# deemoe404/rmcv

Measured on AMD Instinct MI355X. Metric: frames/sec (1280x1024 BGR) armour detect, higher is better.
Workload: dtype u8

## Files before the change

include/rmcv_abi.h:

```cpp
#ifndef RMCV_ABI_H
#define RMCV_ABI_H

#include <stdint.h>

#ifdef __cplusplus
extern "C" {
#endif

#define RMCV_ABI_VERSION 1

#define RMCV_OK 0
#define RMCV_ERR_BAD_ARG (-1)
#define RMCV_ERR_CAPACITY (-2)
#define RMCV_ERR_NOMEM (-3)
#define RMCV_ERR_HIP (-4)
#define RMCV_ERR_NO_DEVICE (-5)
#define RMCV_ERR_RCCL (-6)
#define RMCV_ERR_TIMEOUT (-7)

#define RMCV_CAMP_RED 0
#define RMCV_CAMP_BLUE 1
#define RMCV_CAMP_GUIDELIGHT 2
#define RMCV_CAMP_NEUTRAL (-1)

// ... 19 lines not shown
    int32_t blob_i, blob_j;
} rmcv_armour;

typedef struct {
    int32_t camp;
    int32_t lower_bound;
    int32_t morph;
    float   tilt_max;
    float   ratio_lo, ratio_hi;
    double  area_lo, area_hi;
    float   angle_diff_max;
    float   shear_max;
    float   length_ratio_max;
    int32_t _pad;
} rmcv_params;

typedef struct {
    int32_t max_frames;
    int32_t max_width;
    int32_t max_height;
    int32_t max_contours;
    int32_t max_points;
    int32_t max_blobs;
    int32_t max_armours;
    int32_t _pad;
} rmcv_limits;

#define RMCV_STAGE_BINARY 1
#define RMCV_STAGE_CONTOURS 2
#define RMCV_STAGE_BLOBS 4
#define RMCV_STAGE_ARMOURS 8
#define RMCV_STAGE_ALL 15
#define RMCV_STAGE_POSE 32
#define RMCV_STAGE_NO_IMAGE 64
#define RMCV_STAGE_IDENTITY 16

#define RMCV_FRAME_OVF_CONTOURS 1
#define RMCV_FRAME_OVF_POINTS 2
#define RMCV_FRAME_OVF_BLOBS 4
#define RMCV_FRAME_OVF_ARMOURS 8
#define RMCV_FRAME_SLOW_PATH 16
#define RMCV_FRAME_MID_PATH 64
#define RMCV_FRAME_HULL 32

typedef struct rmcv_ctx rmcv_ctx;

int  rmcv_abi_version(void);
void rmcv_default_params(rmcv_params* p);
void rmcv_default_limits(rmcv_limits* l);

int  rmcv_ctx_create(int device, const rmcv_limits* limits , rmcv_ctx** out);
void rmcv_ctx_destroy(rmcv_ctx* ctx);
const char* rmcv_last_error(const rmcv_ctx* ctx);
#define RMCV_OPT_SPARSE_WAVES 1
#define RMCV_OPT_PIXEL_GROUPS 2
#define RMCV_OPT_FRAME_UPLOAD 3
#define RMCV_OPT_RUN_AHEAD 4
#define RMCV_OPT_CONTOUR_TIER 5
#define RMCV_OPT_DENSE_DEFER 7
#define RMCV_OPT_PIXEL_HALO_NT 11
#define RMCV_OPT_OVERLOADS 13
#define RMCV_OPT_PIXEL_SHAPE 14
#define RMCV_OPT_WAIT_TIMEOUT_MS 15
#define RMCV_OPT_IMAGE_EXPORT 17
#define RMCV_OPT_TEST_SLOW_US 18
#define RMCV_OPT_TEST_DELAY_US 16
#define RMCV_OPT_INPUT_FORMAT 19
#define RMCV_INPUT_BGR 0
#define RMCV_BAYER_RG 1
#define RMCV_BAYER_GB 2
#define RMCV_BAYER_GR 3
#define RMCV_BAYER_BG 4
#define RMCV_OPT_INPUT_SAMPLE_BITS 20
#define RMCV_OPT_INPUT_VALID_BIT 21
#define RMCV_OPT_INPUT_ORIENT 22
#define RMCV_ORIENT_MIRROR 1
#define RMCV_ORIENT_FLIP 2
#define RMCV_OPT_ENHANCE 23
int  rmcv_ctx_set_option(rmcv_ctx* ctx, int option, int value);
int  rmcv_ctx_set_enhance_gains(rmcv_ctx* ctx, float max_gain, float min_gain);
int  rmcv_ctx_get_enhance(const rmcv_ctx* ctx, int32_t* on, float* max_gain, float* min_gain);
int64_t rmcv_pixel_ws_launches(void);
int64_t rmcv_pixel_image_delta_launches(void);
int  rmcv_ctx_check_guards(rmcv_ctx* ctx, int32_t* n_damaged);
int  rmcv_ctx_frame_timing(const rmcv_ctx* ctx, double* us, int cap);
int  rmcv_ctx_forget_frame_buffer(rmcv_ctx* ctx, const void* frame);


int rmcv_extract_color(rmcv_ctx* ctx, const uint8_t* bgr, int w, int h, int stride, int camp, int lower_bound,
                       int morph, uint8_t* binary_out, rmcv_point* pts_out, int pts_cap, int32_t* offs_out,
                       int contours_cap, int32_t* n_contours, int32_t* n_points);

int rmcv_filter_lightblobs(rmcv_ctx* ctx, const rmcv_point* pts, const int32_t* offs, int n_contours,
                           float tilt_max, float ratio_lo, float ratio_hi, double area_lo, double area_hi,
                           int enemy, rmcv_lightblob* blobs_out, int blobs_cap, int32_t* n_blobs,
                           int32_t* blob_src, int32_t* neg_idx_out, int32_t* n_neg);

int rmcv_filter_armours(rmcv_ctx* ctx, const rmcv_lightblob* blobs, int n_blobs, float angle_diff_max,
                        float shear_max, float length_ratio_max, int enemy, rmcv_armour* armours_out,
                        int armours_cap, int32_t* n_armours);

int rmcv_fit_ellipse(rmcv_ctx* ctx, const rmcv_point* pts, int n, rmcv_rrect* out);

int rmcv_demosaic(rmcv_ctx* ctx, const uint8_t* raw, int w, int h, int stride, int pattern, uint8_t* bgr_out, int out_stride);
int rmcv_demosaic_raw(rmcv_ctx* ctx, const void* raw, int w, int h, int stride, int pattern, int sample_bits, int valid_bit, int orient,
                      uint8_t* bgr_out, int out_stride);

int rmcv_gamma_lut(float gamma, uint8_t lut[256]);
int rmcv_enhance_gamma(const uint64_t sums_bgr[3], int64_t n_pixels, float max_gain, float min_gain, float* gamma);
int rmcv_calc_gamma(rmcv_ctx* ctx, const uint8_t* src, int row_bytes, int rows, int src_stride, float gamma, uint8_t* dst, int dst_stride);
int rmcv_auto_enhance(rmcv_ctx* ctx, const uint8_t* bgr, int w, int h, int stride, float max_gain, float min_gain, uint8_t* out, int out_stride,
                      float* gamma_out);


int rmcv_batch_upload(rmcv_ctx* ctx, const uint8_t* frames, int n_frames, int w, int h, int stride,
                      int64_t frame_pitch);
int rmcv_batch_set_device_frames(rmcv_ctx* ctx, const void* d_frames, int n_frames, int w, int h, int stride,
                                 int64_t frame_pitch);
int rmcv_batch_run(rmcv_ctx* ctx, const rmcv_params* p, int stages, void* hip_stream);
int rmcv_batch_sync(rmcv_ctx* ctx);
int rmcv_batch_run_timed(rmcv_ctx* ctx, const rmcv_params* p, int stages, void* hip_stream, float stage_ms[5]);

int rmcv_batch_counts(rmcv_ctx* ctx, int32_t* n_contours, int32_t* n_points, int32_t* n_blobs,
                      int32_t* n_armours, int32_t* status);
int rmcv_batch_get_binary(rmcv_ctx* ctx, int frame, uint8_t* binary_out);
int rmcv_batch_get_contours(rmcv_ctx* ctx, int frame, rmcv_point* pts_out, int pts_cap, int32_t* offs_out,
                            int contours_cap, int32_t* n_contours, int32_t* n_points);
int rmcv_batch_get_blobs(rmcv_ctx* ctx, int frame, rmcv_lightblob* blobs_out, int cap, int32_t* n_blobs,
                         int32_t* blob_src);
int rmcv_batch_get_gammas(rmcv_ctx* ctx, float* gamma_out, int cap);
int rmcv_batch_get_armours(rmcv_ctx* ctx, rmcv_armour* armours_out, int cap, int32_t* frame_offs,
                           int32_t* n_total);
int rmcv_batch_device_views(rmcv_ctx* ctx, void** d_armours, void** d_counts, int32_t* per_frame_cap,
                            int32_t* n_frames);

int rmcv_batch_set_windows(rmcv_ctx* ctx, const rmcv_point* origins, int win_w, int win_h);
int rmcv_batch_set_device_windows(rmcv_ctx* ctx, const void* d_origins, int win_w, int win_h);
int rmcv_batch_get_windows(rmcv_ctx* ctx, rmcv_point* eff_out, int cap, int32_t* win_w, int32_t* win_h);
int rmcv_batch_device_windows(rmcv_ctx* ctx, void** d_eff, int32_t* win_w, int32_t* win_h);
int rmcv_get_roi(const float* points, int n, float scale_w, float scale_h, int frame_w, int frame_h, const int32_t previous[4], int32_t out[4]);
int rmcv_window_origin(const int32_t rect[4], int win_w, int win_h, int32_t out_xy[2]);
int rmcv_armours_to_frame(rmcv_armour* armours, int n, int x, int y);

int rmcv_frame_key(int32_t camp, int32_t lower_bound, int32_t out[4]);
int rmcv_batch_set_frame_camps(rmcv_ctx* ctx, const int32_t* camps, const int32_t* lower_bounds);
int rmcv_batch_set_device_frame_camps(rmcv_ctx* ctx, const void* d_camps, const void* d_lower_bounds);
int rmcv_batch_get_frame_keys(rmcv_ctx* ctx, int32_t* keys_out , int cap);

#define RMCV_SVM_FEATURES 1200
int rmcv_svm_load(rmcv_ctx* ctx, const float* weights , const double* rho,
                  const int32_t* labels, int n_class);
int rmcv_classify_armours(rmcv_ctx* ctx, const uint8_t* bgr, int w, int h, int stride, rmcv_armour* armours, int n,
                          int32_t* identity_out, uint8_t* icons_out);
int rmcv_batch_get_identities(rmcv_ctx* ctx, int32_t* identity_out, int cap, int32_t* n_total);
int rmcv_batch_get_icons(rmcv_ctx* ctx, int frame, uint8_t* icons_out, int cap_armours, int32_t* n_armours);

#define RMCV_SVM_MAX_GRID 16
#define RMCV_SVM_MAX_DF 28
#define RMCV_SVM_MAX_FOLDS 64
#define RMCV_SVM_MAX_SAMPLES 8192
#define RMCV_SVM_MAX_PAIR_SAMPLES 2048
typedef struct {
    double  eps;
    int32_t max_iter;
    int32_t k_fold;
    int32_t n_c;
// ... 457 lines not shown
```

rmcv_amd/abi.py:

```python
import ctypes as C
import os

import numpy as np

_HERE = os.path.dirname(os.path.abspath(__file__))
LIB_PATH = os.environ.get("RMCV_LIB_PATH") or os.path.join(_HERE, "lib", "librmcv_hip.so")

POINT = np.dtype([("x", "<i4"), ("y", "<i4")])
RRECT = np.dtype([("cx", "<f4"), ("cy", "<f4"), ("w", "<f4"), ("h", "<f4"), ("angle", "<f4")])
LIGHTBLOB = np.dtype([("angle", "<f4"), ("target", "<i4"), ("center", "<f4", (2,)),
                      ("vertices", "<f4", (4, 2)), ("size", "<f4", (2,))])
ARMOUR = np.dtype([("icon", "<f4", (4, 2)), ("vertices", "<f4", (4, 2)), ("bbox", "<f4", (4,)),
                   ("blob_i", "<i4"), ("blob_j", "<i4")])
TRACK_IDS = 32
TRACK = np.dtype([("armour", ARMOUR), ("timestamp", "<i8"), ("lost_count", "<i4"), ("identity", "<i4"), ("position", "<f8", (3,)),
                  ("initialized", "<i4"), ("n_ids", "<i4"), ("ids", "<i4", (TRACK_IDS,)), ("counts", "<i4", (TRACK_IDS,)),
                  ("measurement", "<f8", (6,)), ("state_pre", "<f8", (6,)), ("state_post", "<f8", (6,)),
                  ("transition", "<f8", (6, 6)), ("measurement_matrix", "<f8", (6, 6)), ("process_noise_cov", "<f8", (6, 6)),
                  ("measurement_noise_cov", "<f8", (6, 6)), ("error_cov_pre", "<f8", (6, 6)), ("error_cov_post", "<f8", (6, 6)),
                  ("gain", "<f8", (6, 6))])
assert POINT.itemsize == 8 and LIGHTBLOB.itemsize == 56 and ARMOUR.itemsize == 88 and TRACK.itemsize == 2552
AIM = np.dtype([("track", "<i4"), ("identity", "<i4"), ("lost_count", "<i4"), ("status", "<i4"), ("pitch", "<f8"), ("yaw", "<f8"),
                ("flight_time", "<f8"), ("distance", "<f8"), ("point", "<f8", (3,))])
AIM_INPUT = np.dtype([("world2camera", "<f8", (4, 4)), ("motor_angle", "<f8")])
assert AIM.itemsize == 72 and AIM_INPUT.itemsize == 136
ATTITUDE = np.dtype([("roll", "<f8"), ("pitch", "<f8"), ("yaw", "<f8")])
ATTITUDE_CONFIG = np.dtype([("gripper2camera", "<f8", (4, 4)), ("motor_angle_mode", "<i4"), ("reserved", "<i4")])
assert ATTITUDE.itemsize == 24 and ATTITUDE_CONFIG.itemsize == 136
SERIAL_PACKET_BYTES = 24
ATT_MOTOR_KEEP, ATT_MOTOR_PITCH = 0, 1

OK, ERR_BAD_ARG, ERR_CAPACITY, ERR_NOMEM, ERR_HIP, ERR_NO_DEVICE, ERR_RCCL, ERR_TIMEOUT = 0, -1, -2, -3, -4, -5, -6, -7
COMM_ID_BYTES = 128
CAMP_RED, CAMP_BLUE, CAMP_GUIDELIGHT, CAMP_NEUTRAL = 0, 1, 2, -1
MORPH_NONE, MORPH_DILATE, MORPH_CLOSE = 0, 1, 2
OPT_SPARSE_WAVES = 1
OPT_PIXEL_GROUPS = 2
OPT_FRAME_UPLOAD = 3
OPT_RUN_AHEAD = 4
OPT_CONTOUR_TIER = 5
OPT_DENSE_DEFER = 7
OPT_PIXEL_HALO_NT = 11
OPT_OVERLOADS = 13
OPT_PIXEL_SHAPE = 14
OPT_WAIT_TIMEOUT_MS = 15
OPT_TEST_DELAY_US = 16
OPT_IMAGE_EXPORT = 17
OPT_TEST_SLOW_US = 18
OPT_INPUT_FORMAT = 19
INPUT_BGR, BAYER_RG, BAYER_GB, BAYER_GR, BAYER_BG = 0, 1, 2, 3, 4
BAYER_PATTERNS = (BAYER_RG, BAYER_GB, BAYER_GR, BAYER_BG)
OPT_INPUT_SAMPLE_BITS = 20
OPT_INPUT_VALID_BIT = 21
OPT_INPUT_ORIENT = 22
ORIENT_MIRROR, ORIENT_FLIP = 1, 2
OPT_ENHANCE = 23
ENHANCE_MAX_GAIN, ENHANCE_MIN_GAIN = 100.0, 50.0
STAGE_BINARY, STAGE_CONTOURS, STAGE_BLOBS, STAGE_ARMOURS, STAGE_ALL, STAGE_IDENTITY, STAGE_POSE, STAGE_NO_IMAGE = 1, 2, 4, 8, 15, 16, 32, 64
SVM_FEATURES = 1200
COMPENSATE_NONE, COMPENSATE_CLASSIC, COMPENSATE_NI = 0, 1, 2
AIM_NO_TARGET, AIM_NO_SOLUTION = 1, 2
AIM_HEIGHT_FIXED, AIM_HEIGHT_DELTA = 0, 1
AIM_SRC_FILTER, AIM_SRC_MEASUREMENT = 0, 1
AIM_PICK_WINDOW, AIM_PICK_NEAREST = 0, 1
VIEW_BLOBS, VIEW_NEGATIVES, VIEW_ARMOURS, VIEW_ALL = 1, 2, 4, 7
FRAME_OVF_CONTOURS, FRAME_OVF_POINTS, FRAME_OVF_BLOBS, FRAME_OVF_ARMOURS, FRAME_SLOW_PATH, FRAME_MID_PATH = 1, 2, 4, 8, 16, 64
HARVEST_SKIP, HARVEST_MISSES = -2**31, 1
HARVEST_META = np.dtype([("tag", "<u8"), ("frame", "<i4"), ("armour", "<i4"), ("label", "<i4"), ("identity", "<i4"), ("win_x", "<i4"), ("win_y", "<i4"),
                         ("icon", "<f4", (4, 2))])

EXPORTS = [
    "rmcv_abi_version", "rmcv_default_params", "rmcv_default_limits", "rmcv_ctx_create", "rmcv_ctx_destroy",
    "rmcv_last_error", "rmcv_ctx_set_option", "rmcv_ctx_forget_frame_buffer", "rmcv_ctx_check_guards", "rmcv_ctx_frame_timing", "rmcv_extract_color", "rmcv_filter_lightblobs", "rmcv_filter_armours", "rmcv_fit_ellipse", "rmcv_demosaic", "rmcv_demosaic_raw",
    "rmcv_batch_upload", "rmcv_batch_set_device_frames", "rmcv_batch_run", "rmcv_batch_sync", "rmcv_batch_run_timed",
    "rmcv_batch_counts", "rmcv_batch_get_binary", "rmcv_batch_get_contours", "rmcv_batch_get_blobs",
    "rmcv_batch_get_armours", "rmcv_batch_device_views", "rmcv_batch_compact_armours", "rmcv_synth_frame", "rmcv_synth_checksum",
    "rmcv_svm_load", "rmcv_classify_armours", "rmcv_batch_get_identities", "rmcv_batch_get_icons",
    "rmcv_default_pnp_config", "rmcv_pnp_load", "rmcv_locate_armours", "rmcv_batch_set_base2gripper", "rmcv_batch_get_poses",
    "rmcv_max_iou", "rmcv_identity_max", "rmcv_comm_unique_id", "rmcv_comm_create", "rmcv_comm_destroy", "rmcv_comm_info", "rmcv_comm_last_error", "rmcv_gather",
    "rmcv_default_pipeline_config", "rmcv_pipeline_create", "rmcv_pipeline_destroy", "rmcv_pipeline_last_error", "rmcv_pipeline_get_info", "rmcv_pipeline_context", "rmcv_pipeline_context_of", "rmcv_pipeline_set_hot_contexts", "rmcv_pipeline_set_wait_timeout", "rmcv_pipeline_reset_stats", "rmcv_hw_queues_hint", "rmcv_pixel_ws_launches", "rmcv_pixel_image_delta_launches",
    "rmcv_pipeline_submit", "rmcv_pipeline_submit_legacy", "rmcv_pipeline_wait", "rmcv_pipeline_collect", "rmcv_pipeline_drain", "rmcv_pipeline_record",
    "rmcv_pipeline_set_hook", "rmcv_pipeline_set_gather", "rmcv_pipeline_gathered", "rmcv_device_alloc", "rmcv_device_free", "rmcv_device_upload", "rmcv_device_download",
    "rmcv_track_init", "rmcv_track_reset", "rmcv_track_update", "rmcv_track_predict", "rmcv_track_step", "rmcv_min_area_rect", "rmcv_match_lightblob", "rmcv_find_lightblobs", "rmcv_lightblob_overlap", "rmcv_batch_run_legacy",
    "rmcv_ctx_set_enhance_gains", "rmcv_ctx_get_enhance", "rmcv_gamma_lut", "rmcv_enhance_gamma", "rmcv_calc_gamma", "rmcv_auto_enhance", "rmcv_batch_get_gammas",
    "rmcv_batch_set_windows", "rmcv_batch_set_device_windows", "rmcv_batch_get_windows", "rmcv_batch_device_windows", "rmcv_pipeline_submit_windows",
    "rmcv_get_roi", "rmcv_window_origin", "rmcv_armours_to_frame",
    "rmcv_default_tracker_config", "rmcv_tracker_create", "rmcv_tracker_destroy", "rmcv_tracker_last_error", "rmcv_tracker_reset", "rmcv_tracker_set_origins",
    "rmcv_tracker_device_origins", "rmcv_batch_track", "rmcv_tracker_counts", "rmcv_tracker_get", "rmcv_tracker_step_host", "rmcv_pipeline_submit_tracked",
    "rmcv_projectile_angle", "rmcv_solve_gea", "rmcv_delta_height", "rmcv_distance", "rmcv_rigid_inverse", "rmcv_default_aim_config", "rmcv_tracker_set_aim",
    "rmcv_tracker_set_aim_inputs", "rmcv_tracker_device_aim_inputs", "rmcv_tracker_aim", "rmcv_tracker_get_aims", "rmcv_tracker_device_aims", "rmcv_tracker_put",
    "rmcv_aim_step_host",
    "rmcv_frame_key", "rmcv_batch_set_frame_camps", "rmcv_batch_set_device_frame_camps", "rmcv_batch_get_frame_keys", "rmcv_pipeline_submit_camps",
    "rmcv_tracker_set_camps", "rmcv_tracker_device_camps",
    "rmcv_euler_to_matrix", "rmcv_homogeneous", "rmcv_crc8", "rmcv_serial_decode", "rmcv_serial_encode", "rmcv_attitude_step_host", "rmcv_default_attitude_config",
    "rmcv_tracker_set_attitude", "rmcv_tracker_set_attitudes", "rmcv_tracker_get_attitudes", "rmcv_tracker_device_attitudes", "rmcv_tracker_get_aim_inputs",
    "rmcv_batch_get_base2gripper", "rmcv_batch_attitude", "rmcv_pipeline_submit_tracked_serial",
    "rmcv_frame_camera", "rmcv_pnp_load_cameras", "rmcv_batch_set_frame_cameras", "rmcv_batch_set_device_frame_cameras", "rmcv_batch_get_frame_cameras",
    "rmcv_pipeline_set_frame_cameras", "rmcv_tracker_set_stream_cameras", "rmcv_tracker_set_aim_configs",
    "rmcv_batch_debug_views", "rmcv_batch_get_debug_view", "rmcv_debug_view", "rmcv_debug_view_host", "rmcv_pipeline_set_views", "rmcv_pipeline_views",
    "rmcv_pack_bound", "rmcv_pack_host", "rmcv_unpack_host", "rmcv_pack_frames", "rmcv_unpack_frames",
    "rmcv_default_recorder_config", "rmcv_recorder_create", "rmcv_recorder_destroy", "rmcv_recorder_last_error", "rmcv_recorder_set_user", "rmcv_recorder_record",
    "rmcv_recorder_freeze", "rmcv_recorder_resume", "rmcv_recorder_count", "rmcv_recorder_entry", "rmcv_recorder_frame", "rmcv_recorder_device_frame",
    "rmcv_recorder_save", "rmcv_session_append", "rmcv_session_open", "rmcv_session_count", "rmcv_session_entry", "rmcv_session_frame", "rmcv_session_close",
    "rmcv_pipeline_set_recorder",
    "rmcv_loop_bound", "rmcv_loop_trigger_host", "rmcv_recorder_set_trigger", "rmcv_recorder_trigger", "rmcv_recorder_loop", "rmcv_session_loop", "rmcv_session_append_loop",
    "rmcv_tracker_restore", "rmcv_tracker_config_from_loop", "rmcv_tracker_aim_config_from_loop", "rmcv_tracker_attitude_config_from_loop",
    "rmcv_svm_train_defaults", "rmcv_svm_train", "rmcv_svm_train_host", "rmcv_svm_gram", "rmcv_svm_gram_host", "rmcv_svm_predict", "rmcv_svm_predict_host",
    "rmcv_dataset_create", "rmcv_dataset_destroy", "rmcv_dataset_clear", "rmcv_dataset_last_error", "rmcv_dataset_count", "rmcv_dataset_get", "rmcv_dataset_device",
    "rmcv_batch_harvest", "rmcv_batch_harvest_device", "rmcv_harvest_plan_host", "rmcv_pipeline_set_harvest", "rmcv_svm_train_dataset", "rmcv_svm_predict_dataset",
]


class Params(C.Structure):
    _fields_ = [("camp", C.c_int32), ("lower_bound", C.c_int32), ("morph", C.c_int32), ("tilt_max", C.c_float),
                ("ratio_lo", C.c_float), ("ratio_hi", C.c_float), ("area_lo", C.c_double), ("area_hi", C.c_double),
                ("angle_diff_max", C.c_float), ("shear_max", C.c_float), ("length_ratio_max", C.c_float),
                ("_pad", C.c_int32)]


class LegacyParams(C.Structure):
    _fields_ = [("min_ratio", C.c_float), ("max_ratio", C.c_float), ("tilt_angle", C.c_float), ("min_area", C.c_float),
                ("max_area", C.c_float), ("fit_ellipse", C.c_int32)]


class PnpConfig(C.Structure):
    _fields_ = [("camera_matrix", C.c_double * 9), ("dist", C.c_double * 5), ("gripper2camera", C.c_double * 16),
                ("square_w", C.c_float), ("square_h", C.c_float)]


class Limits(C.Structure):
    _fields_ = [("max_frames", C.c_int32), ("max_width", C.c_int32), ("max_height", C.c_int32),
                ("max_contours", C.c_int32), ("max_points", C.c_int32), ("max_blobs", C.c_int32),
                ("max_armours", C.c_int32), ("_pad", C.c_int32)]


class PipelineConfig(C.Structure):
    _fields_ = [("depth", C.c_int32), ("pixel_streams", C.c_int32), ("sparse_streams", C.c_int32), ("armour_cap", C.c_int32),
                ("sparse_waves", C.c_int32), ("pixel_groups", C.c_int32), ("host_results", C.c_int32), ("dense_streams", C.c_int32),
                ("hot_contexts", C.c_int32), ("_reserved", C.c_int32)]


class PipelineInfo(C.Structure):
    _fields_ = [("depth", C.c_int32), ("pixel_streams", C.c_int32), ("sparse_streams", C.c_int32), ("armour_cap", C.c_int32),
                ("sparse_waves", C.c_int32), ("pixel_groups", C.c_int32), ("host_results", C.c_int32), ("dense_streams", C.c_int32),
                ("max_frames", C.c_int32), ("hw_queues_env", C.c_int32), ("hw_queues_wanted", C.c_int32), ("_pad", C.c_int32),
                ("record_bytes", C.c_int64), ("armours_offset", C.c_int64), ("submitted", C.c_uint64), ("collected", C.c_uint64),
                ("dense_split", C.c_uint64), ("hot_batches", C.c_uint64), ("hot_contexts", C.c_int32), ("_pad2", C.c_int32), ("latency_batches", C.c_uint64),
                ("host_blocking_calls", C.c_uint64), ("wait_timeout_ms", C.c_int32), ("_pad3", C.c_int32), ("max_submit_us", C.c_double), ("heavy_batches", C.c_uint64), ("held_back", C.c_uint64)]


SVM_MAX_GRID, SVM_MAX_DF, SVM_MAX_FOLDS, SVM_MAX_SAMPLES, SVM_MAX_PAIR_SAMPLES = 16, 28, 64, 8192, 2048


class SvmTrainParams(C.Structure):
    _fields_ = [("eps", C.c_double), ("max_iter", C.c_int32), ("k_fold", C.c_int32), ("n_c", C.c_int32), ("reserved", C.c_int32),
                ("c_grid", C.c_double * SVM_MAX_GRID)]


class SvmTrainReport(C.Structure):
    _fields_ = [("best_c", C.c_double), ("best_index", C.c_int32), ("n_df", C.c_int32), ("cv_errors", C.c_int32 * SVM_MAX_GRID),
                ("iterations", C.c_int32 * SVM_MAX_DF), ("converged", C.c_int32 * SVM_MAX_DF), ("objective", C.c_double * SVM_MAX_DF),
                ("phase_ms", C.c_double * 6), ("alpha_out", C.c_void_p), ("message", C.c_char * 128)]

# ... 35 lines not shown
    _fields_ = [("world2camera", C.c_double * 16), ("motor_angle", C.c_double)]


class _Attitude(C.Structure):
    _fields_ = [("roll", C.c_double), ("pitch", C.c_double), ("yaw", C.c_double)]


class _TrackerConfig(C.Structure):
    _fields_ = [("n_streams", C.c_int32), ("track_cap", C.c_int32), ("process_noise", C.c_double), ("measurement_noise", C.c_double),
                ("error", C.c_double), ("tick_frequency", C.c_double), ("roi_scale_w", C.c_float), ("roi_scale_h", C.c_float),
                ("frame_w", C.c_int32), ("frame_h", C.c_int32), ("win_w", C.c_int32), ("win_h", C.c_int32)]


class _AimConfig(C.Structure):
    _fields_ = [("g", C.c_double), ("v0", C.c_double), ("height", C.c_double), ("offset_x", C.c_float), ("offset_y", C.c_float),
                ("angle_offset", C.c_double), ("latency_s", C.c_double), ("mode", C.c_int32), ("height_mode", C.c_int32), ("source", C.c_int32),
                ("pick", C.c_int32), ("lead_iterations", C.c_int32), ("max_lost", C.c_int32), ("overloads", C.c_int32), ("identity_mask", C.c_uint32)]


class _AttitudeConfig(C.Structure):
    _fields_ = [("gripper2camera", C.c_double * 16), ("motor_angle_mode", C.c_int32), ("reserved", C.c_int32)]


class LoopState(C.Structure):
    _fields_ = [("stream", C.c_int32), ("n_tracking", C.c_int32), ("status", C.c_int32), ("n_armours", C.c_int32),
                ("origin_next", C.c_int32 * 2), ("origin_eff", C.c_int32 * 2), ("frame_status", C.c_int32), ("has_camps", C.c_int32),
                ("camp", C.c_int32), ("lower_bound", C.c_int32), ("has_key", C.c_int32), ("key", C.c_int32 * 4), ("has_cameras", C.c_int32),
                ("cam_eff", C.c_int32), ("has_aim", C.c_int32), ("has_attitude", C.c_int32), ("has_packet", C.c_int32), ("packet_errors", C.c_int32),
                ("n_tracks", C.c_int32), ("flags", C.c_int32), ("fired", C.c_uint32), ("has_prev", C.c_int32), ("trig_frame_status_mask", C.c_int32),
                ("trig_aim_jump_deg", C.c_double), ("timestamp", C.c_int64), ("sequence", C.c_uint64), ("aim", _Aim), ("aim_input", _AimInput), ("attitude", _Attitude),
                ("packet", C.c_uint8 * 24), ("tracker_config", _TrackerConfig), ("aim_config", _AimConfig), ("attitude_config", _AttitudeConfig),
                ("gripper2camera", C.c_double * 16)]


class TriggerConfig(C.Structure):
    _fields_ = [("mask", C.c_uint32), ("post_batches", C.c_int32), ("frame_status_mask", C.c_int32), ("reserved", C.c_int32), ("aim_jump_deg", C.c_double)]


class TriggerInfo(C.Structure):
    _fields_ = [("fired", C.c_int32), ("mask", C.c_uint32), ("sequence", C.c_uint64), ("k", C.c_int32), ("stream", C.c_int32), ("noticed", C.c_int32),
                ("batches_since", C.c_int32)]


LOOP_SIDE_BYTES = 32
assert C.sizeof(TriggerConfig) == 24 and C.sizeof(TriggerInfo) == 32 and C.sizeof(LoopState) % 8 == 0


PIPELINE_HOOK = C.CFUNCTYPE(C.c_int, C.c_void_p, C.c_uint64, C.c_void_p, C.c_int64, C.c_void_p, C.POINTER(C.c_void_p))


class RmcvError(RuntimeError):
    def __init__(self, code, msg=""):
        super().__init__("rmcv error %d: %s" % (code, msg))
        self.code = code


_lib = None


def load(path):
    if not os.path.exists(path):
        raise ImportError("%s is missing: run `make -C rmcv_amd/csrc` (or __graft_entry__.build())" % path)
    L = C.CDLL(path)
    L.rmcv_last_error.restype = C.c_char_p
    L.rmcv_last_error.argtypes = [C.c_void_p]
    L.rmcv_synth_checksum.restype = C.c_uint64
    L.rmcv_ctx_destroy.restype = None
    L.rmcv_ctx_destroy.argtypes = [C.c_void_p]
    L.rmcv_pipeline_last_error.restype = C.c_char_p
    L.rmcv_pipeline_last_error.argtypes = [C.c_void_p]
    L.rmcv_pipeline_destroy.restype = None
    L.rmcv_pipeline_destroy.argtypes = [C.c_void_p]
    L.rmcv_pipeline_context.restype = C.c_void_p
    L.rmcv_pipeline_context.argtypes = [C.c_void_p, C.c_int]
    L.rmcv_pipeline_set_hot_contexts.restype = C.c_int
    L.rmcv_pipeline_set_hot_contexts.argtypes = [C.c_void_p, C.c_int]
    L.rmcv_pipeline_set_wait_timeout.restype = C.c_int
    L.rmcv_pipeline_set_wait_timeout.argtypes = [C.c_void_p, C.c_int]
    L.rmcv_pixel_ws_launches.restype = C.c_int64
    L.rmcv_pixel_ws_launches.argtypes = []
    if hasattr(L, "rmcv_pixel_image_delta_launches"):
        L.rmcv_pixel_image_delta_launches.restype = C.c_int64
        L.rmcv_pixel_image_delta_launches.argtypes = []
    L.rmcv_pipeline_context_of.restype = C.c_void_p
    L.rmcv_pipeline_context_of.argtypes = [C.c_void_p, C.c_uint64]
    L.rmcv_pipeline_submit.argtypes = [C.c_void_p, C.c_void_p, C.c_int, C.c_int, C.c_int, C.c_int, C.c_int64, C.c_void_p, C.c_int, C.c_void_p]
    L.rmcv_pipeline_submit_legacy.argtypes = [C.c_void_p, C.c_void_p, C.c_int, C.c_int, C.c_int, C.c_int, C.c_int64, C.c_void_p, C.c_void_p, C.c_int, C.c_void_p]
    L.rmcv_pipeline_wait.argtypes = [C.c_void_p, C.c_uint64]
    L.rmcv_pipeline_collect.argtypes = [C.c_void_p, C.c_uint64, C.c_void_p, C.c_int, C.c_void_p, C.c_void_p]
    L.rmcv_pipeline_record.argtypes = [C.c_void_p, C.c_uint64, C.c_void_p, C.c_void_p]
    L.rmcv_pipeline_gathered.argtypes = [C.c_void_p, C.c_uint64, C.c_void_p, C.c_void_p]
    L.rmcv_pipeline_set_gather.argtypes = [C.c_void_p, C.c_void_p, C.c_int]
    if hasattr(L, "rmcv_demosaic"):
        L.rmcv_demosaic.restype = C.c_int
        L.rmcv_demosaic.argtypes = [C.c_void_p, C.c_void_p, C.c_int, C.c_int, C.c_int, C.c_int, C.c_void_p, C.c_int]
    if hasattr(L, "rmcv_demosaic_raw"):
        L.rmcv_demosaic_raw.restype = C.c_int
        L.rmcv_demosaic_raw.argtypes = [C.c_void_p, C.c_void_p, C.c_int, C.c_int, C.c_int, C.c_int, C.c_int, C.c_int, C.c_int, C.c_void_p, C.c_int]
    if hasattr(L, "rmcv_auto_enhance"):
        L.rmcv_ctx_set_enhance_gains.argtypes = [C.c_void_p, C.c_float, C.c_float]
        L.rmcv_ctx_get_enhance.argtypes = [C.c_void_p, C.c_void_p, C.c_void_p, C.c_void_p]
        L.rmcv_gamma_lut.argtypes = [C.c_float, C.c_void_p]
        L.rmcv_enhance_gamma.argtypes = [C.c_void_p, C.c_int64, C.c_float, C.c_float, C.c_void_p]
        L.rmcv_calc_gamma.argtypes = [C.c_void_p, C.c_void_p, C.c_int, C.c_int, C.c_int, C.c_float, C.c_void_p, C.c_int]
        L.rmcv_auto_enhance.argtypes = [C.c_void_p, C.c_void_p, C.c_int, C.c_int, C.c_int, C.c_float, C.c_float, C.c_void_p, C.c_int, C.c_void_p]
        L.rmcv_batch_get_gammas.argtypes = [C.c_void_p, C.c_void_p, C.c_int]
    if hasattr(L, "rmcv_get_roi"):
        L.rmcv_batch_set_windows.argtypes = [C.c_void_p, C.c_void_p, C.c_int, C.c_int]
        L.rmcv_batch_set_device_windows.argtypes = [C.c_void_p, C.c_void_p, C.c_int, C.c_int]
        L.rmcv_batch_get_windows.argtypes = [C.c_void_p, C.c_void_p, C.c_int, C.c_void_p, C.c_void_p]
        L.rmcv_batch_device_windows.argtypes = [C.c_void_p, C.c_void_p, C.c_void_p, C.c_void_p]
        L.rmcv_pipeline_submit_windows.argtypes = [C.c_void_p, C.c_void_p, C.c_int, C.c_int, C.c_int, C.c_int, C.c_int64, C.c_void_p, C.c_int, C.c_int,
                                                   C.c_void_p, C.c_int, C.c_void_p]
        L.rmcv_get_roi.argtypes = [C.c_void_p, C.c_int, C.c_float, C.c_float, C.c_int, C.c_int, C.c_void_p, C.c_void_p]
        L.rmcv_window_origin.argtypes = [C.c_void_p, C.c_int, C.c_int, C.c_void_p]
        L.rmcv_armours_to_frame.argtypes = [C.c_void_p, C.c_int, C.c_int, C.c_int]
    if hasattr(L, "rmcv_tracker_create"):
        L.rmcv_default_tracker_config.restype = None
        L.rmcv_default_tracker_config.argtypes = [C.c_void_p]
        L.rmcv_tracker_create.argtypes = [C.c_int, C.c_void_p, C.c_void_p]
        L.rmcv_tracker_destroy.restype = None
        L.rmcv_tracker_destroy.argtypes = [C.c_void_p]
        L.rmcv_tracker_last_error.restype = C.c_char_p
        L.rmcv_tracker_last_error.argtypes = [C.c_void_p]
        L.rmcv_tracker_reset.argtypes = [C.c_void_p]
        L.rmcv_tracker_set_origins.argtypes = [C.c_void_p, C.c_void_p]
        L.rmcv_tracker_device_origins.argtypes = [C.c_void_p, C.c_void_p]
        L.rmcv_batch_track.argtypes = [C.c_void_p, C.c_void_p, C.c_int64, C.c_void_p]
        L.rmcv_tracker_counts.argtypes = [C.c_void_p, C.c_void_p, C.c_void_p, C.c_int]
        L.rmcv_tracker_get.argtypes = [C.c_void_p, C.c_int, C.c_void_p, C.c_int, C.c_void_p, C.c_void_p, C.c_void_p]
        L.rmcv_tracker_step_host.argtypes = [C.c_void_p, C.c_void_p, C.c_void_p, C.c_void_p, C.c_void_p, C.c_void_p, C.c_void_p, C.c_int, C.c_void_p, C.c_void_p,
                                             C.c_int, C.c_int, C.c_int64]
        L.rmcv_pipeline_submit_tracked.argtypes = [C.c_void_p, C.c_void_p, C.c_void_p, C.c_int, C.c_int, C.c_int, C.c_int, C.c_int64, C.c_void_p, C.c_int, C.c_int64, C.c_void_p]
    if hasattr(L, "rmcv_aim_step_host"):
        L.rmcv_projectile_angle.restype = C.c_double
        L.rmcv_projectile_angle.argtypes = [C.c_double, C.c_double, C.c_double, C.c_double]
        L.rmcv_solve_gea.restype = C.c_double
        L.rmcv_solve_gea.argtypes = [C.c_void_p, C.c_double, C.c_double, C.c_double, C.c_float, C.c_float, C.c_double, C.c_int, C.c_void_p]
        L.rmcv_delta_height.restype = C.c_double
        L.rmcv_delta_height.argtypes = [C.c_void_p, C.c_double, C.c_float, C.c_double]
        L.rmcv_distance.restype = C.c_double
        L.rmcv_distance.argtypes = [C.c_void_p]
        L.rmcv_rigid_inverse.argtypes = [C.c_void_p, C.c_void_p]
        L.rmcv_default_aim_config.restype = None
        L.rmcv_default_aim_config.argtypes = [C.c_void_p]
        L.rmcv_tracker_set_aim.argtypes = [C.c_void_p, C.c_void_p]
        L.rmcv_tracker_set_aim_inputs.argtypes = [C.c_void_p, C.c_void_p]
        L.rmcv_tracker_device_aim_inputs.argtypes = [C.c_void_p, C.c_void_p]
        L.rmcv_tracker_aim.argtypes = [C.c_void_p, C.c_int64, C.c_void_p]
        L.rmcv_tracker_get_aims.argtypes = [C.c_void_p, C.c_void_p, C.c_int]
        L.rmcv_tracker_device_aims.argtypes = [C.c_void_p, C.c_void_p]
        L.rmcv_tracker_put.argtypes = [C.c_void_p, C.c_int, C.c_void_p, C.c_int, C.c_void_p]
        L.rmcv_aim_step_host.argtypes = [C.c_void_p, C.c_double, C.c_void_p, C.c_int, C.c_void_p, C.c_int64, C.c_void_p]
    if hasattr(L, "rmcv_frame_key"):
        L.rmcv_frame_key.argtypes = [C.c_int32, C.c_int32, C.c_void_p]
        L.rmcv_batch_set_frame_camps.argtypes = [C.c_void_p, C.c_void_p, C.c_void_p]
        L.rmcv_batch_set_device_frame_camps.argtypes = [C.c_void_p, C.c_void_p, C.c_void_p]
        L.rmcv_batch_get_frame_keys.argtypes = [C.c_void_p, C.c_void_p, C.c_int]
        L.rmcv_pipeline_submit_camps.argtypes = [C.c_void_p, C.c_void_p, C.c_int, C.c_int, C.c_int, C.c_int, C.c_int64, C.c_void_p, C.c_void_p, C.c_void_p,
                                                 C.c_int, C.c_int, C.c_void_p, C.c_int, C.c_void_p]
        L.rmcv_tracker_set_camps.argtypes = [C.c_void_p, C.c_void_p, C.c_void_p]
        L.rmcv_tracker_device_camps.argtypes = [C.c_void_p, C.c_void_p, C.c_void_p]
    if hasattr(L, "rmcv_attitude_step_host"):
        L.rmcv_euler_to_matrix.argtypes = [C.c_void_p, C.c_void_p]
        L.rmcv_homogeneous.argtypes = [C.c_void_p, C.c_void_p, C.c_void_p]
        L.rmcv_crc8.restype = C.c_uint8
# ... 315 lines not shown
```

rmcv_amd/csrc/image_plan.h:

```cpp
#pragma once

namespace rmcv {

enum ImageTrack { IMAGE_UNKNOWN = 0, IMAGE_TRACKED };
struct ImageState {
    ImageTrack track;
    int w, h;
    int frames;
};
constexpr ImageState IMAGE_STATE_UNKNOWN = {IMAGE_UNKNOWN, 0, 0, 0};

enum ImageKernel { IMAGE_KERNEL_WS = 0, IMAGE_KERNEL_OTHER };
struct ImageLaunch {
    ImageKernel kernel;
    bool image;
    int w, h, ww, frames;
};
enum ImageMode { IMAGE_FULL = 0, IMAGE_DELTA };
struct ImageStep { ImageMode mode; ImageState next; };

inline ImageStep image_step(const ImageState& st, const ImageLaunch& l, bool ok)
{
    ImageStep r = {IMAGE_FULL, st};
    if (!l.image) {
        if (!ok) r.next = IMAGE_STATE_UNKNOWN;
        return r;
    }
    const bool same = st.track == IMAGE_TRACKED && st.w == l.w && st.h == l.h;
    if (l.kernel == IMAGE_KERNEL_WS && same && l.frames <= st.frames && l.ww <= 32) r.mode = IMAGE_DELTA;
    if (!ok || l.kernel != IMAGE_KERNEL_WS) {
        r.next = IMAGE_STATE_UNKNOWN;
        return r;
    }
    r.next = {IMAGE_TRACKED, l.w, l.h, same && st.frames > l.frames ? st.frames : l.frames};
    return r;
}

}
```

rmcv_amd/csrc/k_binary.hip:

```cpp
#include <stdlib.h>

#include <algorithm>
#include <atomic>
#include <type_traits>

#include "k_binary_device.h"

namespace rmcv {

#define K1_ENH 0
#define K1_KERNEL k_binary
#define K1_THRESH(d) thresh16<CA, CB>(d, lb)
#define K1_PASS(a, b) ((a) - (b) >= lb)
#include "k_binary_kernel.inc"

#include "k_binary_ws.inc"

static std::atomic<int64_t> g_ws_launches{0};
int64_t pixel_ws_launches() { return g_ws_launches.load(std::memory_order_relaxed); }
static std::atomic<int64_t> g_image_delta_launches{0};
int64_t pixel_image_delta_launches() { return g_image_delta_launches.load(std::memory_order_relaxed); }
#define K1_LAUNCH_T launch_binary_t
#define K1_EXTRA
#include "k_binary_launch.inc"

hipError_t launch_binary(const Geom& g, const Bufs& b, int camp, int lower_bound, int morph, bool image, const RunPlan& plan, hipStream_t s,
                         ImageState* img)
{
    const PixelVariant v = pixel_variant(g.input_format, g.enhance, g.win, g.keys);
    if (v == PIXEL_BGR)
        return with_channel_pair(frame_key_eff(camp, lower_bound), [&](auto ca, auto cb) { return launch_binary_t<ca, cb>(g, b, lower_bound, morph, image, plan, s, img); });
    const ImageLaunch l = {IMAGE_KERNEL_OTHER, image, g.w, g.h, g.ww, g.n_frames};
    const ImageState before = img ? *img : IMAGE_STATE_UNKNOWN;
    if (img) *img = image_step(before, l, false).next;
    hipError_t e = hipSuccess;
    switch (v) {
    case PIXEL_BGR: break;
    case PIXEL_BAYER: e = launch_binary_bayer(g, b, camp, lower_bound, morph, image, s); break;
    case PIXEL_ENH: e = launch_binary_enh(g, b, camp, lower_bound, morph, image, plan, s); break;
    case PIXEL_WIN: e = launch_binary_win(g, b, camp, lower_bound, morph, image, plan, s); break;
    case PIXEL_CAMP: e = launch_binary_camp(g, b, morph, image, plan, s); break;
    case PIXEL_CAMP_WIN: e = launch_binary_camp_win(g, b, morph, image, plan, s); break;
    }
    if (img && e == hipSuccess) *img = image_step(before, l, true).next;
    return e;
}

__global__ void k_pack_bits(const uint8_t* __restrict__ binary, int w, int h, int ww, uint64_t* __restrict__ bits, int prow,
                            int64_t plane_pitch, uint32_t* __restrict__ rowmask)
{
    const int f = blockIdx.y;
    const int item = blockIdx.x * blockDim.x + threadIdx.x;
    if (item >= h * ww) return;
    const int y = item / ww, k = item % ww;
    const uint8_t* row = binary + (int64_t)f * w * h + (int64_t)y * w;
    uint64_t word = 0;
    for (int bqt = 0; bqt < 64; bqt++) {
        int x = k * 64 + bqt;
        if (x < w && row[x]) word |= 1ull << bqt;
    }
    bits[(int64_t)f * plane_pitch + (int64_t)(y + 1) * prow + 1 + k] = word;
    if (word && k < 32) atomicOr(&rowmask[(int64_t)f * h + y], 1u << k);
}

hipError_t launch_pack_bits(const Geom& g, const Bufs& b, hipStream_t s)
{
    const int items = g.h * g.ww;
    hipError_t e = hipMemsetAsync(b.rowmask, 0, (size_t)g.n_frames * g.h * sizeof(uint32_t), s);
    if (e != hipSuccess) return e;
    return launch(k_pack_bits, dim3((items + 255) / 256, g.n_frames), dim3(256), 0, s, b.binary, g.w, g.h, g.ww, b.bits,
                       g.prow, g.plane_pitch, b.rowmask);
}

}
```

rmcv_amd/csrc/k_binary_launch.inc:

```
#ifndef K1_WIN
#define K1_WIN 0
#endif
#ifndef K1_CAMP
#define K1_CAMP 0
#endif
#if K1_CAMP
#define K1_INST(F) K1_KERNEL<F>
#else
#define K1_INST(F) K1_KERNEL<CA, CB, F>
template <int CA, int CB>
#endif
static hipError_t K1_LAUNCH_T(const Geom& g, const Bufs& b, int lower_bound, int morph, bool image, const RunPlan& plan,
                                  hipStream_t s, ImageState* img = nullptr)
{
    constexpr PixelVariant variant = K1_CAMP ? (K1_WIN ? PIXEL_CAMP_WIN : PIXEL_CAMP) : K1_WIN ? PIXEL_WIN : K1_ENH ? PIXEL_ENH : PIXEL_BGR;
    const PixelShape ps = pixel_shape(pixel_batch(g, b, variant, lower_bound, plan));
    const int strips = ps.strips, lb = ps.lb, all_pass = ps.all_pass, mode = ps.mode;
    const size_t planes = ps.planes;
#if !K1_ENH && !K1_WIN && !K1_CAMP
    const ImageState img_before = img ? *img : IMAGE_STATE_UNKNOWN;
    const ImageLaunch img_launch = {IMAGE_KERNEL_WS, image, g.w, g.h, g.ww, g.n_frames};
    const ImageMode img_mode = image_step(img_before, img_launch, true).mode;
    bool all_ws = true;
    if (img) *img = image_step(img_before, img_launch, false).next;
#endif
    for (int f0 = 0; f0 < g.n_frames; f0 += ps.chunk) {
        const int nf = std::min(ps.chunk, g.n_frames - f0);
        const PixelChunk pc = pixel_chunk(ps, nf);
        const int n_blocks = pc.n_blocks, grid = pc.grid, taper_head = pc.taper_head, taper_tail = pc.taper_tail;
        const uint8_t* frames = b.frames + (int64_t)f0 * g.frame_pitch;
        uint8_t* binary = image ? b.binary + (int64_t)f0 * g.w * g.h : nullptr;
        uint64_t* bits = b.bits + (int64_t)f0 * g.plane_pitch;
        uint32_t* rowmask = b.rowmask + (int64_t)f0 * g.h;
        static size_t lds_set[MAX_DEVICES][3] = {};
        if (planes > 60 * 1024 && planes > lds_set[g.device][mode]) {
#if K1_WIN
            const void* fn = mode == 1 ? reinterpret_cast<const void*>(K1_INST(1)) : reinterpret_cast<const void*>(K1_INST(0));
#else
            const void* fn = mode == 2 ? reinterpret_cast<const void*>(K1_INST(2)) : mode == 1 ? reinterpret_cast<const void*>(K1_INST(1)) : reinterpret_cast<const void*>(K1_INST(0));
#endif
            const hipError_t ea = hipFuncSetAttribute(fn, hipFuncAttributeMaxDynamicSharedMemorySize, (int)planes);
            if (ea != hipSuccess) return ea;
            lds_set[g.device][mode] = planes;
        }
#if !K1_ENH && !K1_WIN && !K1_CAMP
        constexpr int WS_NL = 8, WS_NS = 8, WS_RING = 2, WS_AUX = 2 ;
        if (pc.ws) {
            K1Args ka;
            ka.frames = frames; ka.frame_pitch = g.frame_pitch; ka.stride = g.stride; ka.n_frames = nf; ka.w = g.w; ka.h = g.h; ka.ww = g.ww;
            ka.lb = lb; ka.morph = morph; ka.binary = binary; ka.bits = bits; ka.prow = g.prow; ka.plane_pitch = g.plane_pitch;
            ka.strips = strips; ka.n_blocks = n_blocks; ka.rowmask = rowmask; ka.strip_ctr = b.strip_ctr;
            ka.imgmask = b.imgmask + (int64_t)f0 * g.h; ka.delta = img_mode == IMAGE_DELTA;
            g_ws_launches.fetch_add(1, std::memory_order_relaxed);
            if (ka.delta && binary) g_image_delta_launches.fetch_add(1, std::memory_order_relaxed);
            const hipError_t e = launch(k_binary_ws<CA, CB, WS_NL, WS_NS, WS_RING, WS_AUX, 3, 3>, dim3(pc.grid_ws), dim3((WS_NL + WS_NS) * 64), ps.planes_ws, s, ka);
            if (e != hipSuccess) return e;
            continue;
        }
        all_ws = false;
#endif
#define RMCV_K1_LAUNCH(F)                                                                                                             \
    launch(K1_INST(F), dim3(grid), dim3(256), planes, s, frames, g.frame_pitch, g.stride, nf, g.w, g.h, g.ww, lb, all_pass, \
           morph, binary, bits, g.prow, g.plane_pitch, strips, n_blocks, rowmask, b.strip_ctr, taper_head, taper_tail,               \
           g.pixel_halo_nt K1_EXTRA)
#if K1_WIN
        const hipError_t e = mode == 1 ? RMCV_K1_LAUNCH(1) : RMCV_K1_LAUNCH(0);
#else
        const hipError_t e = mode == 2 ? RMCV_K1_LAUNCH(2) : mode == 1 ? RMCV_K1_LAUNCH(1) : RMCV_K1_LAUNCH(0);
#endif
#undef RMCV_K1_LAUNCH
        if (e != hipSuccess) return e;
    }
#if !K1_ENH && !K1_WIN && !K1_CAMP
    if (img) *img = image_step(img_before, {all_ws ? IMAGE_KERNEL_WS : IMAGE_KERNEL_OTHER, image, g.w, g.h, g.ww, g.n_frames}, true).next;
#endif
    return hipSuccess;
}
#undef K1_INST
```

rmcv_amd/csrc/k_binary_ws.inc:

```

struct K1Args {
    const uint8_t* frames;
    int64_t frame_pitch;
    int stride, n_frames, w, h, ww, lb, morph;
    uint8_t* binary;
    uint64_t* bits;
    int prow;
    int64_t plane_pitch;
    int strips, n_blocks;
    uint32_t* rowmask;
    int* strip_ctr;
    uint32_t* imgmask;
    int delta;
};

template <int NS>
__device__ __forceinline__ uint32_t ws_image_mask(const K1Args& a, const int L, const int sw, const int lane)
{
    constexpr int RPW = SR / NS;
    if (!(a.delta && a.binary && a.ww <= 32) || L < 0) return 0u;
    const int f = L / a.strips, y = (L - f * a.strips) * SR + sw * RPW + lane;
    return (lane < RPW && y < a.h) ? a.imgmask[(int64_t)f * a.h + y] : 0u;
}

template <int NS>
__device__ __forceinline__ uint32_t ws_store_strip(const K1Args& a, const int L, const uint64_t* __restrict__ T, uint64_t* __restrict__ Ew,
                                               const uint64_t* __restrict__ lut, const int sw, const int lane,
                                               const __amdgpu_buffer_rsrc_t r_bin, const __amdgpu_buffer_rsrc_t r_plane, const uint32_t m_old,
                                                   const int L_next)
{
    constexpr int RPW = SR / NS;
    static_assert(RPW >= 2 && RPW % 2 == 0, "a lane produces a pair of rows");
    const int halo = a.morph, ww = a.ww, w = a.w, h = a.h;
    const int f = L / a.strips, strip = L - f * a.strips;
    const int y0 = strip * SR;
    const int s0 = sw * RPW;
    if (y0 + s0 >= h) return ws_image_mask<NS>(a, L_next, sw, lane);
    const uint32_t plane_base = (uint32_t)((int64_t)f * a.plane_pitch);
    const int n_task = (RPW / 2) * ww;
    const uint32_t r_ww = (uint32_t)((0x100000000ull + ww - 1) / ww);
    const bool masked = a.binary && ww <= 32, delta = masked && a.delta;
    const bool my_row = lane < RPW && y0 + s0 + lane < h;
    uint32_t* const im = a.imgmask + ((int64_t)f * h + y0 + s0 + lane);
    uint32_t m_new = 0;
    for (int t0 = 0; t0 < n_task; t0 += 64) {
        const int t = t0 + lane;
        const bool on = t < n_task;
        const int p = on ? div_r(t, r_ww) : 0, k = on ? t - p * ww : 0;
        const int s = s0 + 2 * p;
        const uint64_t* base = T + __umul24(s, ww) + k;
        uint64_t e0, e1;
        if (halo == 0) {
            e0 = base[0];
            e1 = base[ww];
        } else {
            const int nr = 2 + 2 * halo;
            uint64_t ta[6], tb[6], tc[6];
#pragma unroll
            for (int i = 0; i < 6; i++) {
                if (i < nr) {
                    tb[i] = base[i * ww];
                    ta[i] = k > 0 ? base[i * ww - 1] : 0ull;
                    tc[i] = k < ww - 1 ? base[i * ww + 1] : 0ull;
                } else {
                    ta[i] = tb[i] = tc[i] = 0ull;
                }
            }
            uint64_t Db[4];
            uint32_t DL[4], DR[4];
#pragma unroll
            for (int i = 1; i <= 4; i++) {
                if (i <= nr - 2) {
                    const uint64_t ca = ta[i - 1] | ta[i] | ta[i + 1], cb = tb[i - 1] | tb[i] | tb[i + 1], cc = tc[i - 1] | tc[i] | tc[i + 1];
                    uint64_t d = cb | (cb << 1) | (cb >> 1) | (ca >> 63) | ((cc & 1ull) << 63);
                    uint32_t dl = (uint32_t)((ca >> 62) != 0) | (uint32_t)(cb & 1ull);
                    uint32_t dr = (uint32_t)((cc & 3ull) != 0) | (uint32_t)(cb >> 63);
                    const int y = y0 - halo + s + i;
                    if (y < 0 || y >= h) { d = ~0ull; dl = 1; dr = 1; }
                    if (k == 0) dl = 1;
                    if (k == ww - 1) dr = 1;
                    Db[i - 1] = d; DL[i - 1] = dl; DR[i - 1] = dr;
                } else {
                    Db[i - 1] = 0; DL[i - 1] = 0; DR[i - 1] = 0;
                }
            }
            if (halo == 1) {
                e0 = Db[0];
                e1 = Db[1];
            } else {
                uint64_t e[2];
#pragma unroll
                for (int j = 0; j < 2; j++) {
                    const uint64_t c = Db[j] & Db[j + 1] & Db[j + 2];
                    const uint64_t l = (uint64_t)(DL[j] & DL[j + 1] & DL[j + 2]), r = (uint64_t)(DR[j] & DR[j + 1] & DR[j + 2]);
                    e[j] = c & ((c << 1) | l) & ((c >> 1) | (r << 63));
                }
                e0 = e[0];
                e1 = e[1];
            }
        }
        const int y = y0 + s;
        if (on) {
            Ew[__umul24(2 * p, ww) + k] = e0;
            Ew[__umul24(2 * p + 1, ww) + k] = e1;
        }
#ifdef RMCV_K1_NOBITS
        const uint32_t po0 = OOB, po1 = OOB;
#else
        const uint32_t po0 = (on && y < h) ? (plane_base + __umul24(y + 1, a.prow) + 1u + (uint32_t)k) * 8u : OOB;
        const uint32_t po1 = (on && y + 1 < h) ? (plane_base + __umul24(y + 2, a.prow) + 1u + (uint32_t)k) * 8u : OOB;
#endif
        __builtin_amdgcn_raw_buffer_store_b64(__builtin_bit_cast(u32x2v, e0), r_plane, po0, 0, RMCV_K1_PLAIN_PLAUX);
        __builtin_amdgcn_raw_buffer_store_b64(__builtin_bit_cast(u32x2v, e1), r_plane, po1, 0, RMCV_K1_PLAIN_PLAUX);
        {
            const bool last = on && k == ww - 1;
            const u32x4v z = {0u, 0u, 0u, 0u};
            __builtin_amdgcn_raw_buffer_store_b128(z, r_plane, last && po0 != OOB ? po0 + 8u : OOB, 0, RMCV_K1_PLAIN_PLAUX);
            __builtin_amdgcn_raw_buffer_store_b128(z, r_plane, last && po1 != OOB ? po1 + 8u : OOB, 0, RMCV_K1_PLAIN_PLAUX);
        }
        if (ww <= 32 && n_task <= 64) {
            const uint64_t b0 = __builtin_amdgcn_ballot_w64(on && e0 != 0), b1 = __builtin_amdgcn_ballot_w64(on && e1 != 0);
            if (lane < RPW) {
                const int pr = lane >> 1;
                const uint64_t b = (lane & 1) ? b1 : b0;
                const uint32_t m = (uint32_t)(b >> __umul24(pr, ww)) & (ww == 32 ? 0xFFFFFFFFu : ((1u << ww) - 1u));
                m_new = m;
#ifndef RMCV_K1_NOROWMASK
                if (y0 + s0 + lane < h) a.rowmask[(int64_t)f * h + y0 + s0 + lane] = m;
#endif
            }
        }
    }
    __builtin_amdgcn_fence(__ATOMIC_RELEASE, "wavefront");
    __builtin_amdgcn_wave_barrier();
    __builtin_amdgcn_fence(__ATOMIC_ACQUIRE, "wavefront");
    if (ww <= 32 && n_task > 64) {
        if (lane < RPW && y0 + s0 + lane < h) {
            uint32_t m = 0;
            for (int k = 0; k < ww; k++) m |= (uint32_t)(Ew[__umul24(lane, ww) + k] != 0) << k;
            a.rowmask[(int64_t)f * h + y0 + s0 + lane] = m;
            m_new = m;
        }
    }
    const uint32_t m_ahead = ws_image_mask<NS>(a, L_next, sw, lane);
    if (a.binary) {
        const uint32_t keep = delta ? (m_old | m_new) : 0xFFFFFFFFu;
        if (masked && my_row && (!delta || m_new != m_old)) *im = m_new;
        if (delta && __builtin_amdgcn_ballot_w64(my_row && keep != 0) == 0) return m_ahead;
        const int n_valid = min(RPW, h - (y0 + s0)) * ww * 4;
        const uint16_t* R16 = reinterpret_cast<const uint16_t*>(Ew);
        const uint32_t out0 = (uint32_t)((int64_t)f * w * h) + (uint32_t)(y0 + s0) * (uint32_t)w;
        for (int b = 0; b < n_valid; b += 64) {
            const int it = b + lane;
            bool ok = it < n_valid;
            if (delta) {
                const int wd = ok ? it >> 2 : 0, r = div_r(wd, r_ww), k = wd - r * ww;
                const uint32_t kr = (uint32_t)__shfl((int)keep, r);
                ok = ok && ((kr >> k) & 1u);
                if (__builtin_amdgcn_ballot_w64(ok) == 0) continue;
            }
            const uint32_t m = R16[it < n_valid ? it : 0];
            const uint64_t lo = lut[m & 0xFF], hi = lut[m >> 8];
            const u32x4v o = {(uint32_t)lo, (uint32_t)(lo >> 32), (uint32_t)hi, (uint32_t)(hi >> 32)};
#ifdef RMCV_K1_NOSTORE
            const uint32_t off = OOB;
#else
            const uint32_t off = ok ? out0 + (uint32_t)it * 16u : OOB;
#endif
            __builtin_amdgcn_raw_buffer_store_b128(o, r_bin, off, 0, RMCV_K1_STAUX);
        }
    }
    return m_ahead;
}

template <int CA, int CB, int NL, int NS, int R, int AUX, int PRIO_L, int PRIO_S>
__global__ __launch_bounds__((NL + NS) * 64, 6) void k_binary_ws(const K1Args a)
{
    extern __shared__ uint64_t smem[];
    constexpr int RPW = SR / NS;
    const int tid = threadIdx.x;
    const int lane = tid & 63;
    const int wave = __builtin_amdgcn_readfirstlane(tid >> 6);
    const int ww = a.ww;
    const int PL = (SR + 4) * ww;
    uint64_t* const T0 = smem;
    uint64_t* const T1 = smem + PL;
    uint64_t* const Ew = smem + 2 * PL + (wave >= NL ? (wave - NL) * RPW * ww : 0);
    __shared__ uint64_t s_lut[256];
    __shared__ uint16_t s_spare[NL * 64];
    __shared__ int s_L[4];
    asm volatile("v_mov_b32 v71, 0" ::: "v71");
    if (tid < 256) s_lut[tid] = (uint64_t)expand4(tid) | ((uint64_t)expand4(tid >> 4) << 32);
    const int xcd = blockIdx.x & 7;
    const int per_xcd = (a.n_blocks + 7) >> 3;
    int* const head = a.strip_ctr + xcd * CTR_STRIDE;
    if (tid == 0) {
        const int j0 = atomicAdd(head, 2);
        s_L[0] = j0;
        s_L[1] = j0 + 1;
    }
    const __amdgpu_buffer_rsrc_t r_in = __builtin_amdgcn_make_buffer_rsrc(
        const_cast<uint8_t*>(a.frames), 0, (int)((int64_t)(a.n_frames - 1) * a.frame_pitch + (int64_t)(a.h - 1) * a.stride + 3 * a.w), RSRC3);
    const __amdgpu_buffer_rsrc_t r_bin = __builtin_amdgcn_make_buffer_rsrc(a.binary, 0, a.binary ? (int)((int64_t)a.n_frames * a.w * a.h) : 0, RSRC3);
    const __amdgpu_buffer_rsrc_t r_plane = __builtin_amdgcn_make_buffer_rsrc(a.bits, 0, (int)((int64_t)a.n_frames * a.plane_pitch * 8), RSRC3);
    __syncthreads();
    auto strip_of = [&](int j) -> int {
        const int L = xcd * per_xcd + j;
        return ((uint32_t)j < (uint32_t)per_xcd && L < a.n_blocks) ? L : -1;
    };

    if (wave < NL) {
        if (PRIO_L > 0) __builtin_amdgcn_s_setprio(PRIO_L);
        const int halo = a.morph, w = a.w, h = a.h;
        const int srh = SR + 2 * halo;
        const uint32_t lane_off = (uint32_t)lane * 12u;
        const uint32_t M1 = (lane & 1) ? 0xF0F0u : 0x0F0Fu, S1 = (lane & 1) ? 12u : 4u;
        const uint32_t P2 = (lane & 2) ? 0x0c0c0105u : 0x0c0c0400u;
        constexpr uint32_t OOB_S = 0xFFFFFC00u;
        const uint32_t px_total = (uint32_t)__umul24(srh, w);
        const int n_blk = (int)((px_total + 255u) >> 8);
        const int n_itl = (n_blk + 3) >> 2;
        const int nbw = (n_itl + NL - 1) / NL;
        const int nbp = ((nbw + R - 1) / R) * R;
// ... 96 lines not shown
```

rmcv_amd/csrc/rmcv_ctx.h:

```cpp
#pragma once
#include <stdio.h>
#include <time.h>

#include <vector>

#include "rmcv_internal.h"
#include "frame_plan.h"

struct FrameChain {
    int frame_upload = 3;
    int run_ahead = 1;
    struct Reg { const void* p; size_t bytes; };
    std::vector<Reg> registered;
    uint8_t* h_frame = nullptr;
    size_t h_frame_bytes = 0;
    int32_t* h_hdr = nullptr;
    int32_t *hd_hdr = nullptr, *hd_offs = nullptr, *hd_blob_src = nullptr, *hd_neg = nullptr;
    rmcv_point* hd_pts = nullptr;
    rmcv_lightblob* hd_blobs = nullptr;
    rmcv_armour* hd_armours = nullptr;
    rmcv_point* h_pts = nullptr;
    int32_t* h_offs = nullptr;
    rmcv_lightblob* h_blobs = nullptr;
    int32_t* h_blob_src = nullptr;
    int32_t* h_neg = nullptr;
    rmcv_armour* h_armours = nullptr;
    int32_t* d_hdr = nullptr;
    int res_nc = -1, res_total = 0;
    int res_nb = -1;
    rmcv::LbParams last_lb{};
    rmcv::ArParams last_ar{};
    bool last_lb_valid = false, last_ar_valid = false;
    bool ahead_lb = false, ahead_ar = false;
    hipStream_t side = nullptr;
    hipEvent_t ev_fork = nullptr;
    uint8_t *h_image = nullptr, *hd_image = nullptr;
    size_t h_image_bytes = 0;
    uint32_t *h_iflags = nullptr, *hd_iflags = nullptr;
    uint32_t img_seq = 0;
    int image_export = 2;
    int upload_now = 0, image_now = 0;
    rmcv::CopyPathState copy_up{}, copy_img{};
    int test_slow_us = 0;
    uint32_t* d_iarrived = nullptr;
    double marks[9] = {};

    hipError_t init();
    void release();
};

struct rmcv_ctx {
    int device = 0;
    rmcv::Limits lim{};
    rmcv::Geom geom{};
    rmcv::Bufs bufs{};
    hipStream_t stream = nullptr;
    hipEvent_t ev[6] = {};
    uint8_t* own_frames = nullptr;
    size_t own_frames_bytes = 0;
    rmcv_point* pack_pts = nullptr;
    int32_t* pack_offs = nullptr;
    hipStream_t last_stream = nullptr;
    int geom_w = -1, geom_h = -1;
    rmcv::ImageState image = rmcv::IMAGE_STATE_UNKNOWN;
    int order_n = -1, order_h = -1;
    hipEvent_t ev_order = nullptr;
    bool order_pending = false;
    bool external_order = false;
    hipEvent_t ext_done = nullptr;
    FrameChain chain;
    int mid_frames = 0;
    bool mid_failed = false;
    int sparse_waves = 8;
    int pixel_groups = 3;
    int pixel_shape = 1;
    int dense_defer = 0;
    rmcv::InputOptions input;
    int wait_timeout_ms = 5000;
    const char* last_what = "nothing";
    bool timed_out = false;
    int test_delay_us = 0;
    uint64_t blocking_calls = 0;
    int32_t* order_scratch = nullptr;
    int last_stages = 0;
    rmcv_point* win_own = nullptr;
    int32_t* key_own = nullptr;
    int32_t* cam_own = nullptr;
    int last_camp = RMCV_CAMP_BLUE, last_lower_bound = 80;
    uint64_t* view_overlay = nullptr;
    int view_cap = 0;
    int32_t* view_frames = nullptr;
    uint8_t* view_out = nullptr;
    char err[256] = {0};
    std::vector<void*> allocs;
    struct Guarded { uint8_t* base; size_t bytes; const char* name; size_t rear = 0; };
    std::vector<Guarded> guarded;
};

static int fail(rmcv_ctx* c, int code, const char* what, hipError_t e = hipSuccess)
{
    if (c) {
        if (e != hipSuccess) snprintf(c->err, sizeof(c->err), "%s: %s", what, hipGetErrorString(e));
        else snprintf(c->err, sizeof(c->err), "%s", what);
    }
    if (e != hipSuccess) (void)hipGetLastError();
    return code;
}

static int refuse(rmcv_ctx* c, const char* why) { return why ? fail(c, RMCV_ERR_BAD_ARG, why) : RMCV_OK; }
static int refuse(rmcv_ctx* c, const rmcv::Refusal& r) { return r ? fail(c, r.code, r.why) : RMCV_OK; }

#define HIPCHK(c, call, what)                                        \
    do {                                                                \
        (c)->last_what = what;                                          \
        hipError_t e__ = (call);                                        \
        if (e__ != hipSuccess) return fail((c), RMCV_ERR_HIP, what, e__); \
    } while (0)

namespace rmcv {
static inline double now_us()
{
    timespec ts;
    clock_gettime(CLOCK_MONOTONIC, &ts);
    return ts.tv_sec * 1e6 + ts.tv_nsec * 1e-3;
}
}

static int wait_failed(rmcv_ctx* c, int rcw, const char* what, hipError_t e)
{
    if (rcw < 0) return fail(c, RMCV_ERR_HIP, what, e);
    c->timed_out = true;
    snprintf(c->err, sizeof(c->err), "%s: not finished after %d ms (RMCV_OPT_WAIT_TIMEOUT_MS); enqueued last: %s", what, c->wait_timeout_ms, c->last_what);
    return RMCV_ERR_TIMEOUT;
}
static int wait_stream(rmcv_ctx* c, hipStream_t s, const char* what)
{
    hipError_t e = hipSuccess;
    const int rcw = rmcv::wait_stream_deadline(s, c->wait_timeout_ms, &e);
    if (rcw) return wait_failed(c, rcw, what, e);
    return RMCV_OK;
}
static int wait_event(rmcv_ctx* c, hipEvent_t ev, const char* what)
{
    hipError_t e = hipSuccess;
    const int rcw = rmcv::wait_event_deadline(ev, c->wait_timeout_ms, &e);
    if (rcw) return wait_failed(c, rcw, what, e);
    return RMCV_OK;
// ... 65 lines not shown
```

rmcv_amd/csrc/rmcv_frame.hip:

```cpp
#include <stdlib.h>
#include <string.h>

#include <algorithm>
#include <cmath>
#include <vector>

#include "rmcv_ctx.h"

using namespace rmcv;

hipError_t FrameChain::init()
{
    hipError_t e = hipEventCreateWithFlags(&ev_fork, hipEventDisableTiming);
    if (e == hipSuccess) e = hipStreamCreateWithPriority(&side, hipStreamNonBlocking, 0);
    if (e != hipSuccess) return e;
    if (getenv("RMCV_IMAGE_EXPORT")) image_export = atoi(getenv("RMCV_IMAGE_EXPORT"));
    if (getenv("RMCV_FRAME_UPLOAD")) frame_upload = atoi(getenv("RMCV_FRAME_UPLOAD"));
    return e;
}

void FrameChain::release()
{
    if (side) hipStreamDestroy(side);
    if (ev_fork) hipEventDestroy(ev_fork);
// ... 237 lines not shown
            hipHostGetDevicePointer((void**)&ch.hd_iflags, ch.h_iflags, 0) != hipSuccess) {
            (void)hipGetLastError();
            if (ch.h_iflags) hipHostFree(ch.h_iflags);
            ch.h_iflags = ch.hd_iflags = nullptr;
            return false;
        }
        memset(ch.h_iflags, 0, IMG_CHUNKS * sizeof(uint32_t));
        if (dalloc(c, &ch.d_iarrived, IMG_CHUNKS) != hipSuccess || hipMemset(ch.d_iarrived, 0, IMG_CHUNKS * sizeof(uint32_t)) != hipSuccess) {
            (void)hipGetLastError();
            hipHostFree(ch.h_iflags);
            ch.h_iflags = ch.hd_iflags = nullptr;
            return false;
        }
    }
    if (bytes > ch.h_image_bytes) {
        if (ch.h_image) hipHostFree(ch.h_image);
        ch.h_image = ch.hd_image = nullptr;
        ch.h_image_bytes = 0;
        size_t cap = (size_t)c->lim.max_width * c->lim.max_height;
        if (cap < bytes) cap = bytes;
        if (hipHostMalloc((void**)&ch.h_image, cap, hipHostMallocMapped) != hipSuccess || hipHostGetDevicePointer((void**)&ch.hd_image, ch.h_image, 0) != hipSuccess) {
            (void)hipGetLastError();
            if (ch.h_image) hipHostFree(ch.h_image);
            ch.h_image = ch.hd_image = nullptr;
            return false;
        }
        ch.h_image_bytes = cap;
    }
    return true;
}

static int extract_color_body(rmcv_ctx* c, const uint8_t* bgr, int w, int h, int stride, int camp, int lower_bound, int morph,
                              uint8_t* binary_out, rmcv_point* pts_out, int pts_cap, int32_t* offs_out, int contours_cap,
                              int32_t* n_contours, int32_t* n_points);

int rmcv_extract_color(rmcv_ctx* c, const uint8_t* bgr, int w, int h, int stride, int camp, int lower_bound, int morph,
                       uint8_t* binary_out, rmcv_point* pts_out, int pts_cap, int32_t* offs_out, int contours_cap,
                       int32_t* n_contours, int32_t* n_points)
{
    const int rc = extract_color_body(c, bgr, w, h, stride, camp, lower_bound, morph, binary_out, pts_out, pts_cap, offs_out,
                                      contours_cap, n_contours, n_points);
    if (rc != RMCV_OK && rc != RMCV_ERR_TIMEOUT && c) {
        hipError_t e = hipSuccess;
        (void)wait_stream_deadline(c->stream, c->wait_timeout_ms, &e);
        if (c->chain.side) (void)wait_stream_deadline(c->chain.side, c->wait_timeout_ms, &e);
    }
    return rc;
}

static int extract_color_body(rmcv_ctx* c, const uint8_t* bgr, int w, int h, int stride, int camp, int lower_bound, int morph,
                              uint8_t* binary_out, rmcv_point* pts_out, int pts_cap, int32_t* offs_out, int contours_cap,
                              int32_t* n_contours, int32_t* n_points)
{
    if (!c || !bgr) return RMCV_ERR_BAD_ARG;
    FrameChain& ch = c->chain;
    if (morph < RMCV_MORPH_NONE || morph > RMCV_MORPH_CLOSE) return fail(c, RMCV_ERR_BAD_ARG, "bad morph");
    hipSetDevice(c->device);
    ch.marks[0] = now_us();
    int rc = rmcv_batch_sync(c);
    if (rc) return rc;
    resident_none(c);
    if ((rc = ensure_staging(c))) return rc;
    if ((rc = check_layout(c)) || (rc = check_sample_ptr(c, bgr))) return rc;
    const int rowb = ctx_pixel_bytes(c) * w;
    const int dstride = (rowb + 15) & ~15;
    if ((rc = set_geom(c, 1, w, h, dstride, (int64_t)dstride * h))) return rc;
    reset_modes(c);
    if (stride < rowb) return fail(c, RMCV_ERR_BAD_ARG, "bad stride");
    if (c->geom.sample_bytes == 2 && (stride & 1)) return fail(c, RMCV_ERR_BAD_ARG, "16-bit samples (RMCV_OPT_INPUT_SAMPLE_BITS): stride is bytes and must be even");
    if ((rc = ensure_own_frames(c, (size_t)dstride * h))) return rc;
    if ((rc = upload_one(c, bgr, rowb, h, stride, dstride))) return rc;
    ch.marks[1] = now_us();
    c->bufs.frames = c->own_frames;
    const Geom& g = c->geom;
    const Bufs& b = c->bufs;
    hipStream_t s = c->stream;
    RunPlan plan = ctx_plan(c);
    plan.sparse_waves = 8;
    if (c->test_delay_us) {
        HIPCHK(c, launch_delay((unsigned long long)c->test_delay_us * 1000ull, s), "k_delay (RMCV_OPT_TEST_DELAY_US)");
        c->test_delay_us = 0;
    }
    if (g.enhance) HIPCHK(c, launch_enhance_tables(g, b, lower_bound, s), "k_frame_sums + k_enhance_table");
    HIPCHK(c, launch_binary(g, b, camp, lower_bound, morph, binary_out != nullptr, plan, s, &c->image), PIXEL_VARIANTS[geom_variant(g)].kernel);
    if (binary_out) HIPCHK(c, hipEventRecord(ch.ev_fork, s), "image download: mark");
    const bool fused_ahead = ch.run_ahead && ch.last_lb_valid && ch.last_ar_valid && ch.last_lb.enemy == ch.last_ar.enemy;
    if (fused_ahead) {
        const rmcv_params p = chain_run_params(&ch.last_lb, &ch.last_ar);
        HIPCHK(c, launch_sparse(g, b, c->lim, p, true, false, plan, s), "k_contours (fused)");
    } else {
        HIPCHK(c, launch_contours(g, b, c->lim, s), "k_contours");
    }
    static const bool use_export = !(getenv("RMCV_EXPORT") && atoi(getenv("RMCV_EXPORT")) == 0);
    const bool exporting = use_export && ch.hd_hdr != nullptr;
    const bool will_lb = ch.last_lb_valid && ch.run_ahead, will_ar = will_lb && ch.last_ar_valid;
    const FrameWindows W = result_windows(c);
    ExportArgs ex;
    memset(&ex, 0, sizeof(ex));
    if (exporting) {
        ex.hdr_dst = ch.hd_hdr;
        ex.hdr_src[0] = ch.d_hdr; ex.hdr_src[1] = ch.d_hdr + 1; ex.hdr_src[2] = ch.d_hdr + 2;
        ex.sec[ex.n_sec++] = {c->pack_offs, ch.hd_offs, ch.d_hdr, 1, 4, W.offs + 1};
        ex.sec[ex.n_sec++] = {c->pack_pts, ch.hd_pts, ch.d_hdr + 1, 0, (int)sizeof(rmcv_point), W.pts};
        if (will_lb) {
            ex.hdr_src[4] = b.n_blobs; ex.hdr_src[5] = b.n_neg; ex.hdr_src[6] = b.status;
            ex.sec[ex.n_sec++] = {b.blobs, ch.hd_blobs, b.n_blobs, 0, (int)sizeof(rmcv_lightblob), W.blobs};
            ex.sec[ex.n_sec++] = {b.blob_src, ch.hd_blob_src, b.n_blobs, 0, 4, W.blobs};
            ex.sec[ex.n_sec++] = {b.neg_idx, ch.hd_neg, b.n_neg, 0, 4, W.neg};
        }
        if (will_ar) {
            ex.hdr_src[8] = b.n_armours; ex.hdr_src[9] = b.status; ex.hdr_src[10] = b.status;
            ex.sec[ex.n_sec++] = {b.armours, ch.hd_armours, b.n_armours, 0, (int)sizeof(rmcv_armour), W.armours};
        }
    }
    const bool export_in_pack = exporting && fused_ahead;
    HIPCHK(c, launch_pack_contours(g, b, c->lim, c->pack_pts, c->pack_offs, ch.d_hdr, s, export_in_pack ? &ex : nullptr), "k_pack_contours");
    if (!exporting) {
        HIPCHK(c, hipMemcpyAsync(ch.h_hdr, ch.d_hdr, 3 * 4, hipMemcpyDeviceToHost, s), "D2H");
        HIPCHK(c, hipMemcpyAsync(ch.h_offs, c->pack_offs, (size_t)(W.offs + 1) * 4, hipMemcpyDeviceToHost, s), "D2H offs");
        HIPCHK(c, hipMemcpyAsync(ch.h_pts, c->pack_pts, (size_t)W.pts * sizeof(rmcv_point), hipMemcpyDeviceToHost, s), "D2H pts");
    }
    bool ahead_lb = false, ahead_ar = false;
    if (will_lb) {
        if ((rc = enqueue_blobs(c, ch.last_lb, !fused_ahead, !exporting))) return rc;
        ahead_lb = true;
        if (will_ar) {
            if ((rc = enqueue_armours(c, ch.last_ar, !fused_ahead, !exporting))) return rc;
            ahead_ar = true;
        }
    }
    if (exporting && !export_in_pack) HIPCHK(c, launch_export(ex, s), "k_export");
    ch.marks[2] = now_us();
    if (binary_out && image_ready(c, (size_t)w * h)) {
        const long long bytes = (long long)w * h;
        if (++ch.img_seq == 0) ch.img_seq = 1;
        HIPCHK(c, hipStreamWaitEvent(ch.side, ch.ev_fork, 0), "image download: fork");
        const int n_chunks = IMG_CHUNKS_DEFAULT;
        HIPCHK(c, launch(k_image_export, dim3(IMG_GROUPS), dim3(256), 0, ch.side, b.binary, ch.hd_image, bytes, ch.hd_iflags, ch.img_seq, ch.d_iarrived, n_chunks), "k_image_export");
        c->last_what = "k_binary, k_image_export";
        const volatile uint32_t* fl = ch.h_iflags;
        const double t0w = now_us();
        for (int gch = 0; gch < n_chunks; gch++) {
            for (unsigned spins = 0; fl[gch] != ch.img_seq; spins++) {
                __builtin_ia32_pause();
                if ((spins & 1023u) == 1023u) {
                    const double dtw = now_us() - t0w;
                    if (c->wait_timeout_ms > 0 && dtw > c->wait_timeout_ms * 1000.0) return wait_failed(c, 1, "rmcv_extract_color: waiting for the byte image", hipSuccess);
                    if (dtw > 20000.0) { timespec nap = {0, 200000}; nanosleep(&nap, nullptr); }
                }
            }
            __atomic_thread_fence(__ATOMIC_ACQUIRE);
            if (gch == 0) ch.marks[3] = now_us();
            const ImageChunk ck = image_chunk(bytes, n_chunks, gch);
            if (ck.hi > ck.lo) memcpy(binary_out + ck.lo, ch.h_image + ck.lo, (size_t)(ck.hi - ck.lo));
        }
        ch.marks[4] = now_us();
        ch.image_now = 1;
    } else if (binary_out) {
        ch.image_now = 0;
        c->last_what = "k_binary";
        WAITCHK(c, wait_event(c, ch.ev_fork, "rmcv_extract_color: waiting for the pixel kernel"));
        ch.marks[3] = now_us();
        HIPCHK(c, hipMemcpyAsync(binary_out, b.binary, (size_t)w * h, hipMemcpyDeviceToHost, ch.side), "D2H binary");
        ch.marks[4] = now_us();
        WAITCHK(c, wait_stream(c, ch.side, "rmcv_extract_color: waiting for the byte image's download"));
    } else ch.marks[3] = ch.marks[4] = ch.marks[2];
    ch.marks[5] = now_us();
// ... 162 lines not shown
```

rmcv_amd/csrc/rmcv_host.hip:

```cpp
#include <sched.h>
#include <time.h>
#include <stdio.h>
#include <stdlib.h>

#include <algorithm>
#include <vector>

#include "rmcv_ctx.h"
#include "device_pack.h"

using namespace rmcv;

namespace rmcv {
template <typename Q>
static int poll_deadline(Q query, int timeout_ms, hipError_t* err)
{
    const double t0 = now_us();
    int rc = 0;
    for (;;) {
        const hipError_t e = query();
        if (e == hipSuccess) break;
        if (e != hipErrorNotReady) { *err = e; rc = -1; break; }
        const double dt = now_us() - t0;
        if (timeout_ms > 0 && dt > timeout_ms * 1000.0) { rc = 1; break; }
        if (dt < 2000.0) __builtin_ia32_pause();
        else if (dt < 20000.0) sched_yield();
        else { timespec nap = {0, 200000}; nanosleep(&nap, nullptr); }
    }
    (void)hipGetLastError();
    return rc;
}
int wait_stream_deadline(hipStream_t s, int timeout_ms, hipError_t* err) { return poll_deadline([s] { return hipStreamQuery(s); }, timeout_ms, err); }
int wait_event_deadline(hipEvent_t ev, int timeout_ms, hipError_t* err) { return poll_deadline([ev] { return hipEventQuery(ev); }, timeout_ms, err); }
}

extern "C" {

int rmcv_abi_version(void) { return RMCV_ABI_VERSION; }
int64_t rmcv_pixel_ws_launches(void) { return pixel_ws_launches(); }
int64_t rmcv_pixel_image_delta_launches(void) { return pixel_image_delta_launches(); }

const char* rmcv_last_error(const rmcv_ctx* ctx) { return ctx ? ctx->err : "null context"; }

void rmcv_ctx_destroy(rmcv_ctx* c)
{
    if (!c) return;
    hipSetDevice(c->device);
    {
        hipError_t e = hipSuccess;
        const int t = c->wait_timeout_ms;
        bool stuck = false;
        if (c->external_order && c->ext_done && c->timed_out) stuck |= wait_event_deadline(c->ext_done, t, &e) != 0;
        if (c->order_pending) stuck |= wait_event_deadline(c->ev_order, t, &e) == 1;
        if (c->stream) stuck |= wait_stream_deadline(c->stream, t, &e) == 1;
        if (c->chain.side) stuck |= wait_stream_deadline(c->chain.side, t, &e) == 1;
        if (stuck) {
            fprintf(stderr, "rmcv_ctx_destroy: work of this context has not finished after %d ms (enqueued last: %s); its buffers are leaked\n", t, c->last_what);
            delete c;
            return;
        }
    }
    c->chain.release();
    for (void* p : c->allocs) hipFree(p);
    if (c->own_frames) hipFree(c->own_frames);
    for (auto& e : c->ev)
        if (e) hipEventDestroy(e);
    if (c->ev_order) hipEventDestroy(c->ev_order);
    if (c->stream) hipStreamDestroy(c->stream);
    delete c;
}

int rmcv_ctx_create(int device, const rmcv_limits* limits, rmcv_ctx** out)
{
    if (!out) return RMCV_ERR_BAD_ARG;
    *out = nullptr;
    int ndev = 0;
    if (hipGetDeviceCount(&ndev) != hipSuccess || ndev <= 0 || device < 0 || device >= ndev) return RMCV_ERR_NO_DEVICE;
    rmcv_limits d;
    rmcv_default_limits(&d);
    if (limits) {
        if (limits->max_frames > 0) d.max_frames = limits->max_frames;
        if (limits->max_width > 0) d.max_width = limits->max_width;
        if (limits->max_height > 0) d.max_height = limits->max_height;
        if (limits->max_contours > 0) d.max_contours = limits->max_contours;
        if (limits->max_points > 0) d.max_points = limits->max_points;
        if (limits->max_blobs > 0) d.max_blobs = limits->max_blobs;
        if (limits->max_armours > 0) d.max_armours = limits->max_armours;
    }
    rmcv_ctx* c = new (std::nothrow) rmcv_ctx();
    if (!c) return RMCV_ERR_NOMEM;
    c->device = device;
    c->lim = Limits{d.max_frames, d.max_width, d.max_height, d.max_contours, d.max_points, d.max_blobs, d.max_armours};
    hipError_t e = hipSetDevice(device);
    if (e == hipSuccess) e = hipStreamCreateWithFlags(&c->stream, hipStreamNonBlocking);
    for (int i = 0; i < 6 && e == hipSuccess; i++) e = hipEventCreate(&c->ev[i]);
    if (e == hipSuccess) e = hipEventCreateWithFlags(&c->ev_order, hipEventDisableTiming);
    if (e == hipSuccess) e = c->chain.init();
    if (e == hipSuccess) {
        hipDeviceProp_t prop;
        c->geom.device = device;
        c->geom.n_cu = (device < MAX_DEVICES && hipGetDeviceProperties(&prop, device) == hipSuccess) ? prop.multiProcessorCount : 0;
        if (device >= MAX_DEVICES) e = hipErrorInvalidDevice;
    }
    const size_t F = (size_t)d.max_frames;
    const size_t plane = (size_t)(d.max_height + 2) * ((d.max_width + 63) / 64 + 2);
    Bufs& b = c->bufs;
    if (e == hipSuccess) e = dalloc(c, &b.binary, F * d.max_width * d.max_height);
    if (e == hipSuccess) e = dalloc(c, &b.bits, F * plane);
    if (e == hipSuccess) e = dalloc(c, &b.rowmask, F * d.max_height);
    if (e == hipSuccess) e = dalloc(c, &b.strip_ctr, 9 * CTR_STRIDE);
    if (e == hipSuccess) e = dalloc(c, &b.lab, F * plane);
    if (e == hipSuccess) e = dalloc(c, &b.neg, F * plane);
    if (e == hipSuccess) e = dalloc(c, &b.points, F * d.max_points);
    if (e == hipSuccess) e = dalloc(c, &c->pack_pts, F * d.max_points);
    if (e == hipSuccess) e = dalloc(c, &c->pack_offs, F * (d.max_contours + 1));
    if (e == hipSuccess) e = dalloc(c, &b.cont_start, F * d.max_contours);
    if (e == hipSuccess) e = dalloc(c, &b.cont_len, F * d.max_contours);
    if (e == hipSuccess) e = dalloc(c, &b.n_contours, F);
    if (e == hipSuccess) e = dalloc(c, &b.n_points, F);
    if (e == hipSuccess) e = dalloc(c, &b.visit_xy, F * VISIT_CAP);
    {
        const int64_t words = (int64_t)((d.max_width + 63) / 64) * d.max_height;
        b.mid_slot_cap = (int)std::min<int64_t>(words, 65535);
        b.mid_stride = (int64_t)((mid_bytes(b.mid_slot_cap) + 255) & ~(size_t)255);
        b.mid = nullptr;
    }
    if (e == hipSuccess) e = dalloc(c, &b.blobs, F * d.max_blobs);
    if (e == hipSuccess) e = dalloc(c, &b.blob_src, F * d.max_blobs);
    if (e == hipSuccess) e = dalloc(c, &b.ellipses, F * d.max_blobs);
    if (e == hipSuccess) e = dalloc(c, &b.neg_idx, F * d.max_contours);
    if (e == hipSuccess) e = dalloc(c, &b.elig, F * d.max_contours);
    if (e == hipSuccess) e = dalloc(c, &b.n_elig, F);
    if (e == hipSuccess) e = dalloc(c, &b.slot_kind, F * d.max_contours);
    if (e == hipSuccess) e = dalloc(c, &b.slot_ell, F * d.max_contours);
    if (e == hipSuccess) e = dalloc(c, &b.n_blobs, F);
    if (e == hipSuccess) e = dalloc(c, &b.n_neg, F);
    if (e == hipSuccess) e = dalloc(c, &b.armours, F * d.max_armours);
    if (e == hipSuccess) e = dalloc(c, &b.n_armours, F);
    if (e == hipSuccess) e = dalloc(c, &b.status, F);
    if (e == hipSuccess) e = dalloc(c, &b.frame_order, F);
    if (e == hipSuccess) e = dalloc(c, &c->order_scratch, 2 * F);
    if (e == hipSuccess) e = dalloc(c, &b.enh_sums, 3 * F);
    if (e == hipSuccess) e = dalloc(c, &b.enh_gamma, F);
    if (e == hipSuccess) e = dalloc(c, &b.enh_lut, 256 * F);
    if (e == hipSuccess) e = dalloc(c, &b.enh_m, 256 * F);
    if (e == hipSuccess) e = dalloc(c, &b.win_eff, F);
    if (e == hipSuccess) e = dalloc(c, &c->win_own, F);
    if (e == hipSuccess) e = dalloc(c, &b.imgmask, F * d.max_height);
    if (e == hipSuccess) e = dalloc(c, &b.key_eff, F);
    if (e == hipSuccess) e = dalloc(c, &b.key_enemy, F);
    if (e == hipSuccess) e = dalloc(c, &c->key_own, 2 * F);
    if (e == hipSuccess) {
        hipMemset(b.strip_ctr, 0, 9 * CTR_STRIDE * sizeof(int));
        hipMemset(b.n_contours, 0, F * 4);
        hipMemset(b.n_points, 0, F * 4);
        hipMemset(b.n_blobs, 0, F * 4);
        hipMemset(b.n_neg, 0, F * 4);
        hipMemset(b.n_armours, 0, F * 4);
        e = hipMemset(b.status, 0, F * 4);
        if (e == hipSuccess) e = hipMemset(b.win_eff, 0, F * sizeof(rmcv_point));
        if (e == hipSuccess) e = hipMemset(c->win_own, 0, F * sizeof(rmcv_point));
        if (e == hipSuccess) e = hipMemset(b.key_eff, 0, F * sizeof(FrameKey));
        if (e == hipSuccess) e = hipMemset(b.key_enemy, 0, F * 4);
    }
    if (e == hipSuccess) {
        const std::vector<float> ones(F, 1.0f);
        e = hipMemcpy(b.enh_gamma, ones.data(), F * sizeof(float), hipMemcpyHostToDevice);
    }
    if (e != hipSuccess) {
        fprintf(stderr, "rmcv_ctx_create: %s\n", hipGetErrorString(e));
        rmcv_ctx_destroy(c);
        return e == hipErrorOutOfMemory ? RMCV_ERR_NOMEM : RMCV_ERR_HIP;
    }
    *out = c;
    return RMCV_OK;
}

}

namespace rmcv {
void ctx_external_order(rmcv_ctx* c, hipEvent_t done)
{
    c->external_order = true;
    c->ext_done = done;
}
const Limits& ctx_limits(const rmcv_ctx* c) { return c->lim; }
uint64_t ctx_blocking_calls(const rmcv_ctx* c) { return c->blocking_calls; }
int ctx_wait_timeout_ms(const rmcv_ctx* c) { return c->wait_timeout_ms; }
bool pixel_ws_full(const rmcv_ctx* c, int lower_bound, const RunPlan& plan)
{
    return pixel_shape(pixel_batch(c->geom, c->bufs, geom_variant(c->geom), lower_bound, plan)).ws_full;
}
RunPlan ctx_plan(const rmcv_ctx* c) { return {c->pixel_shape, c->pixel_groups, c->sparse_waves, c->dense_defer ? SPARSE_SPLIT_BOTH : SPARSE_STANDARD}; }
int ctx_enhance(const rmcv_ctx* c) { return c->input.enhance; }
int ctx_n_cameras(const rmcv_ctx* c) { return c->bufs.pnp_cams ? c->bufs.n_cameras : 0; }
void ctx_set_frame_cameras(rmcv_ctx* c, const void* d_idx) { c->bufs.cam_req = (const int32_t*)d_idx; }
PixelVariant ctx_pixel_variant(const rmcv_ctx* c) { return geom_variant(c->geom); }
int ctx_frame_pixel_bytes(const rmcv_ctx* c) { return ctx_pixel_bytes(c); }
void ctx_record_batch(const rmcv_ctx* c, RecordBatch* b)
{
    const Geom& g = c->geom;
    b->input_format = g.input_format, b->sample_bits = 8 * g.sample_bytes, b->valid_bit = g.valid_bit, b->orient = g.orient;
    b->w_bytes = g.frame_w * geom_pixel_bytes(g);
    b->lag = pack_lag(g.input_format, b->sample_bits);
    b->key_eff = g.keys ? c->bufs.key_eff : nullptr;
    b->key_enemy = g.keys ? c->bufs.key_enemy : nullptr;
    b->win_eff = g.win ? c->bufs.win_eff : nullptr;
}
int ctx_compact(rmcv_ctx* c, void* d_armours_out, int cap, void* d_frame_offs, void* d_status_or, hipStream_t s, void* hd_record, int host_head)
{
    HIPCHK(c, launch_compact_armours(c->geom, c->bufs, c->lim, (rmcv_armour*)d_armours_out, cap, (int32_t*)d_frame_offs, s, (int32_t*)d_status_or, (uint8_t*)hd_record, host_head), "k_compact_armours");
    return RMCV_OK;
}
}

int rmcv::ensure_own_frames(rmcv_ctx* c, size_t need)
{
    if (need <= c->own_frames_bytes) return RMCV_OK;
    if (c->own_frames) hipFree(c->own_frames);
    c->own_frames = nullptr;
    c->own_frames_bytes = 0;
    size_t cap = (size_t)((3 * c->lim.max_width + 15) & ~15) * c->lim.max_height * c->lim.max_frames;
    if (cap < need) cap = need;
    HIPCHK(c, hipMalloc((void**)&c->own_frames, cap), "hipMalloc frames");
    c->own_frames_bytes = cap;
    return RMCV_OK;
}

static int ensure_mid(rmcv_ctx* c, int n_frames)
{
    if (n_frames <= c->mid_frames || c->mid_failed) return RMCV_OK;
    const bool no_mid = getenv("RMCV_NO_MID") && atoi(getenv("RMCV_NO_MID"));
    c->blocking_calls++;
    if (c->bufs.mid) {
        const int rcs = rmcv_batch_sync(c);
        if (rcs) return rcs;
        uint8_t* raw = c->bufs.mid - GUARD;
        for (size_t i = 0; i < c->allocs.size(); i++)
            if (c->allocs[i] == raw) { c->allocs.erase(c->allocs.begin() + i); break; }
        for (size_t i = 0; i < c->guarded.size(); i++)
            if (c->guarded[i].base == raw) { c->guarded.erase(c->guarded.begin() + i); break; }
        (void)hipFree(raw);
        c->bufs.mid = nullptr;
        c->mid_frames = 0;
    }
    const int want = n_frames > 1 ? c->lim.max_frames : 1;
    uint8_t* m = nullptr;
    const hipError_t e = no_mid ? hipErrorOutOfMemory : dalloc_named(c, &m, (size_t)want * (size_t)c->bufs.mid_stride, "b.mid");
    if (e != hipSuccess) {
        (void)hipGetLastError();
        c->mid_failed = true;
        return RMCV_OK;
    }
    c->bufs.mid = m;
    c->mid_frames = want;
    return RMCV_OK;
}

namespace rmcv {
static constexpr int ORDER_LDS = 2048;
__global__ __launch_bounds__(256) void k_frame_order(int32_t* __restrict__ order, int32_t* __restrict__ scratch, int n, int strips)
{
    __shared__ int32_t s_o[ORDER_LDS], s_rest[ORDER_LDS], s_used[ORDER_LDS];
    __shared__ int s_lo[9];
    const bool in_lds = n <= ORDER_LDS;
    int32_t* o = in_lds ? s_o : order;
    int32_t* rest = in_lds ? s_rest : scratch;
    int32_t* used = in_lds ? s_used : scratch + n;
    const int tid = threadIdx.x;
    for (int i = tid; i < n; i += 256) { o[i] = -1; used[i] = 0; }
    __threadfence_block();
    __syncthreads();
    if (tid == 0) {
        const int per_xcd = (n * strips + 7) >> 3;
        int q = 0;
        s_lo[0] = 0;
        for (int f = 0; f < n; f++) {
            int qf = (f * strips + strips - 1) / per_xcd;
            if (qf > 7) qf = 7;
            while (q < qf) s_lo[++q] = f;
        }
        while (q < 8) s_lo[++q] = n;
        int longest = 0;
        for (q = 0; q < 8; q++) longest = max(longest, s_lo[q + 1] - s_lo[q]);
        int nrest = 0;
        for (int t = 0; t < longest; t++)
            for (q = 0; q < 8; q++)
                if (t < s_lo[q + 1] - s_lo[q]) {
                    const int b_ = t * 8 + q, v = s_lo[q] + t;
                    if (b_ < n) o[b_] = v;
                    else rest[nrest++] = v;
                }
        int r = 0;
        for (int b_ = 0; b_ < n; b_++)
            if (o[b_] < 0 && r < nrest) o[b_] = rest[r++];
        for (int b_ = 0; b_ < n; b_++)
            if (o[b_] >= 0) used[o[b_]] = 1;
        int nf = 0;
        for (int b_ = 0; b_ < n; b_++)
            if (o[b_] < 0) {
                while (used[nf]) nf++;
                o[b_] = nf;
                used[nf] = 1;
            }
    }
    __threadfence_block();
    __syncthreads();
    if (in_lds)
        for (int i = tid; i < n; i += 256) order[i] = s_o[i];
}
}

namespace rmcv {
__global__ void k_delay(unsigned long long ns)
{
    const unsigned long long t0 = wall_clock64();
    while ((wall_clock64() - t0) * 10ull < ns) __builtin_amdgcn_s_sleep(32);
}
hipError_t launch_delay(unsigned long long ns, hipStream_t s) { return launch(k_delay, dim3(1), dim3(64), 0, s, ns); }
}

int rmcv::check_layout(rmcv_ctx* c) { return refuse(c, layout_refusal(c->input)); }
int rmcv::check_sample_ptr(rmcv_ctx* c, const void* p)
{
    if (c->input.format && c->input.sample_bits == 16 && ((uintptr_t)p & 1))
        return fail(c, RMCV_ERR_BAD_ARG, "16-bit samples (RMCV_OPT_INPUT_SAMPLE_BITS): the frame pointer must be 2-byte aligned");
    return RMCV_OK;
}

static int check_frame_camps(rmcv_ctx* c, int fmt, int enh) { return refuse(c, pixel_refusal(fmt, enh, false, true, false)); }

static int extent_apply(rmcv_ctx* c, hipStream_t as)
{
    const Geom& g = c->geom;
    const ExtentChange change = extent_change(c->geom_w, c->geom_h, c->order_n, c->order_h, g.w, g.h, g.n_frames);
    if (!change.planes && !change.order) return RMCV_OK;
    hipStream_t s = as ? as : c->stream;
    if (!as) {
        c->blocking_calls++;
        const int rcs = rmcv_batch_sync(c);
        if (rcs) return rcs;
    }
    if (change.planes) {
        const size_t plane = (size_t)(c->lim.max_height + 2) * ((c->lim.max_width + 63) / 64 + 2);
        HIPCHK(c, hipMemsetAsync(c->bufs.bits, 0, (size_t)c->lim.max_frames * plane * 8, s), "memset planes");
        HIPCHK(c, hipMemsetAsync(c->bufs.lab, 0, (size_t)c->lim.max_frames * plane * 8, s), "memset planes");
        HIPCHK(c, hipMemsetAsync(c->bufs.neg, 0, (size_t)c->lim.max_frames * plane * 8, s), "memset planes");
        c->geom_w = g.w;
        c->geom_h = g.h;
        c->image = IMAGE_STATE_UNKNOWN;
    }
    if (change.order) {
        const int strips = (g.h + STRIP_ROWS - 1) / STRIP_ROWS;
        HIPCHK(c, launch(k_frame_order, dim3(1), dim3(256), 0, s, c->bufs.frame_order, c->order_scratch, g.n_frames, strips), "k_frame_order");
        c->order_n = g.n_frames;
        c->order_h = g.h;
    }
    if (!as) WAITCHK(c, wait_stream(c, s, "binding a geometry"));
    return RMCV_OK;
}

int rmcv::set_geom(rmcv_ctx* c, int n_frames, int w, int h, int stride, int64_t frame_pitch, hipStream_t as, int win_w, int win_h)
{
    int rc = refuse(c, binding_refusal(c->lim, c->input, n_frames, w, h, stride, frame_pitch, win_w, win_h));
    if (rc || (rc = ensure_mid(c, n_frames))) return rc;
    bind_geom(c->geom, c->input, n_frames, w, h, stride, frame_pitch, win_w, win_h);
    return extent_apply(c, as);
}

static int bound(rmcv_ctx* c, const void* frames)
{
    c->bufs.frames = (const uint8_t*)frames;
    reset_modes(c);
    c->bufs.pose_base2gripper = c->bufs.base2gripper;
    c->last_stages = 0;
    return RMCV_OK;
}


template <typename T>
static int set_request_table(rmcv_ctx* c, const T** req, T* own, const T* h_vals, const void* d_vals, bool sync, const char* what)
{
    if (h_vals) {
        if (sync) {
            if (const int rc = ctx_ready(c)) return rc;
        }
        HIPCHK(c, hipMemcpy(own, h_vals, (size_t)c->geom.n_frames * sizeof(T), hipMemcpyHostToDevice), what);
    }
    *req = h_vals ? own : (const T*)d_vals;
    return RMCV_OK;
}

template <typename T>
static int get_effective_table(rmcv_ctx* c, T* out, int cap, bool on, const T* d_eff, const T& off, const char* what)
{
    const int n = std::min(cap, c->geom.n_frames);
    if (n <= 0) return RMCV_OK;
    if (!on) std::fill_n(out, n, off);
    else HIPCHK(c, hipMemcpy(out, d_eff, (size_t)n * sizeof(T), hipMemcpyDeviceToHost), what);
    return RMCV_OK;
}

static int armour_counts(rmcv_ctx* c, std::vector<int32_t>& cnt, int64_t* total)
{
    cnt.resize(c->geom.n_frames);
    HIPCHK(c, hipMemcpy(cnt.data(), c->bufs.n_armours, cnt.size() * 4, hipMemcpyDeviceToHost), "D2H");
    *total = 0;
    for (const int32_t n : cnt) *total += n;
    return RMCV_OK;
}
template <typename T>
static int gather_rows(rmcv_ctx* c, const T* d_table, const std::vector<int32_t>& cnt, T* out, const char* what)
{
    const size_t row_cap = (size_t)c->lim.max_armours;
    std::vector<T> all(cnt.size() * row_cap);
    HIPCHK(c, hipMemcpy(all.data(), d_table, all.size() * sizeof(T), hipMemcpyDeviceToHost), what);
    for (size_t f = 0; f < cnt.size(); f++) out = std::copy_n(all.data() + f * row_cap, cnt[f], out);
    return RMCV_OK;
}

static int order_begin(rmcv_ctx* c, hipStream_t s)
{
    if (c->external_order) return RMCV_OK;
    if (c->order_pending && c->last_stream != s) HIPCHK(c, hipStreamWaitEvent(s, c->ev_order, 0), "order: wait for the previous stream");
    return RMCV_OK;
}
static int order_end(rmcv_ctx* c, hipStream_t s)
{
    c->last_stream = s;
    if (c->external_order) return RMCV_OK;
    HIPCHK(c, hipEventRecord(c->ev_order, s), "order: record");
    c->order_pending = true;
    return RMCV_OK;
}

static int run_stages(rmcv_ctx* c, const rmcv_params* p, int stages, hipStream_t s, bool timed, const RunPlan& plan,
                      const rmcv_legacy_params* lp = nullptr, bool* lean = nullptr)
{
    const Geom& g = c->geom;
    const Bufs& b = c->bufs;
    const Limits& lim = c->lim;
    const RunSteps st = run_steps(stages, timed, lp != nullptr, g.input_format, g.enhance, g.win, g.keys);
    int k = 0;
    resident_none(c);
    int rc;
    if ((rc = refuse(c, st.refusal)) || (rc = order_begin(c, s))) return rc;
    if (c->test_delay_us) {
        HIPCHK(c, launch_delay((unsigned long long)c->test_delay_us * 1000ull, s), "k_delay (RMCV_OPT_TEST_DELAY_US)");
        c->test_delay_us = 0;
    }
    if (timed) HIPCHK(c, hipEventRecord(c->ev[k++], s), "event");
    if (st.status_clear) HIPCHK(c, launch_status_clear(g, b, st.status_clear, s), "k_status_clear");
    if (lean) *lean = false;
    if (st.enhance_tables) HIPCHK(c, launch_enhance_tables(g, b, p->lower_bound, s), "k_frame_sums + k_enhance_table");
    if (st.window_origins) HIPCHK(c, launch_window_origins(g, b, s), "k_window_origins");
    if (st.frame_keys) HIPCHK(c, launch_frame_keys(g, b, p->lower_bound, s), "k_frame_keys");
    if (st.binary) {
        c->last_camp = p->camp;
        c->last_lower_bound = p->lower_bound;
        HIPCHK(c, launch_binary(g, b, p->camp, p->lower_bound, p->morph, st.image, plan, s, &c->image), PIXEL_VARIANTS[geom_variant(g)].kernel);
    }
    if (timed) HIPCHK(c, hipEventRecord(c->ev[k++], s), "event");
    if (st.sparse) HIPCHK(c, launch_sparse(g, b, lim, *p, st.sparse_pairs, st.sparse_identity, plan, s, lean), "k_contours (fused)");
    if (st.contours) HIPCHK(c, launch_contours(g, b, lim, s), "k_contours");
    if (timed) HIPCHK(c, hipEventRecord(c->ev[k++], s), "event");
    if (st.match) HIPCHK(c, launch_match(g, b, lim, *p, *lp, 0, b.frames != nullptr, st.match_pairs, s), "k_match");
    if (st.blobs_armours) HIPCHK(c, launch_blobs_armours(g, b, lim, *p, s), "k_fit");
    if (st.blobs) HIPCHK(c, launch_blobs(g, b, lim, *p, s), "k_fit");
    if (timed) HIPCHK(c, hipEventRecord(c->ev[k++], s), "event");
    if (st.armours) HIPCHK(c, launch_armours(g, b, lim, *p, s), "k_armours");
    if (st.classify) HIPCHK(c, launch_classify(g, b, lim, s), "k_classify");
    if (st.pnp) HIPCHK(c, launch_pnp(g, b, lim, s), "k_pnp");
    if (timed) HIPCHK(c, hipEventRecord(c->ev[k++], s), "event");
    c->last_stages = next_last_stages(c->last_stages, stages);
    return order_end(c, s);
}

int rmcv::ctx_check_stages(rmcv_ctx* c, const rmcv_params* p, int stages)
{
    if (!c) return RMCV_ERR_BAD_ARG;
    return refuse(c, stage_refusal(p, stages, c->bufs.svm_w != nullptr, c->bufs.pnp_cfg != nullptr));
}
static int check_bound(rmcv_ctx* c, const rmcv_params* p, int stages)
{
    if (const int rc = ctx_check_stages(c, p, stages)) return rc;
    if ((c->geom.n_frames <= 0 || !c->bufs.frames) && (stages & RMCV_STAGE_BINARY)) return fail(c, RMCV_ERR_BAD_ARG, "no frames bound");
    return RMCV_OK;
}

extern "C" {

int rmcv_batch_upload(rmcv_ctx* c, const uint8_t* frames, int n_frames, int w, int h, int stride, int64_t frame_pitch)
{
    if (!c || !frames) return RMCV_ERR_BAD_ARG;
    int rc = ctx_ready(c);
    if (rc) return rc;
    resident_none(c);
    if ((rc = check_layout(c)) || (rc = check_sample_ptr(c, frames))) return rc;
    const UploadLayout dev = upload_layout(ctx_pixel_bytes(c), w, h);
    if ((rc = refuse(c, dev.refusal(stride, frame_pitch))) || (rc = set_geom(c, n_frames, w, h, dev.stride, dev.pitch))) return rc;
    const size_t need = (size_t)dev.pitch * n_frames;
    rc = ensure_own_frames(c, need);
    if (rc) return rc;
    if (dev.same(stride, frame_pitch)) {
        HIPCHK(c, hipMemcpyAsync(c->own_frames, frames, need, hipMemcpyHostToDevice, c->stream), "H2D frames");
    } else {
        for (int f = 0; f < n_frames; f++)
            HIPCHK(c, hipMemcpy2DAsync(c->own_frames + (size_t)f * dev.pitch, dev.stride, frames + (size_t)f * frame_pitch, stride,
                                       (size_t)dev.row_bytes, h, hipMemcpyHostToDevice, c->stream),
                   "H2D frames 2D");
    }
    WAITCHK(c, wait_stream(c, c->stream, "H2D frames"));
    return bound(c, c->own_frames);
}

int rmcv_batch_set_device_frames(rmcv_ctx* c, const void* d_frames, int n_frames, int w, int h, int stride,
                                 int64_t frame_pitch)
{
    if (!c || !d_frames) return RMCV_ERR_BAD_ARG;
    hipSetDevice(c->device);
    resident_none(c);
    int rc = check_sample_ptr(c, d_frames);
    if (rc) return rc;
    rc = set_geom(c, n_frames, w, h, stride, frame_pitch);
    if (rc) return rc;
    return bound(c, d_frames);
}

}
namespace rmcv {
int ctx_bind_frames(rmcv_ctx* c, const void* d_frames, int n_frames, int w, int h, int stride, int64_t frame_pitch, hipStream_t s,
                    const void* d_origins, int win_w, int win_h, const void* d_camps, const void* d_lower_bounds)
{
    if (!c || !d_frames || !s) return RMCV_ERR_BAD_ARG;
    resident_none(c);
    int rc = check_sample_ptr(c, d_frames);
    if (rc) return rc;
    if (d_camps && (rc = check_frame_camps(c, c->input.format, c->input.enhance))) return rc;
    if (d_origins && win_w <= 0) return fail(c, RMCV_ERR_BAD_ARG, "window size out of range: win_w and win_h must be at least 1");
    rc = set_geom(c, n_frames, w, h, stride, frame_pitch, s, d_origins ? win_w : 0, win_h);
    if (rc || (rc = bound(c, d_frames))) return rc;
    c->bufs.win_req = (const rmcv_point*)d_origins;
    c->geom.keys = d_camps != nullptr;
    c->bufs.key_camps = (const int32_t*)d_camps;
    c->bufs.key_lbs = d_camps ? (const int32_t*)d_lower_bounds : nullptr;
    return RMCV_OK;
}
int ctx_check_modes(rmcv_ctx* c, bool keys, bool legacy) { return refuse(c, pixel_refusal(c->input.format, c->input.enhance, false, keys, legacy)); }
int ctx_prepare_ring(rmcv_ctx* c) { return ensure_mid(c, c->lim.max_frames); }
int ctx_run(rmcv_ctx* c, const rmcv_params* p, const rmcv_legacy_params* lp, int stages, hipStream_t s, const RunPlan& plan, bool* lean)
{
    const int rc = check_bound(c, p, stages);
    if (rc) return rc;
    return run_stages(c, p, stages, s, false, plan, lp, lean);
}
}
extern "C" {

int rmcv_batch_run(rmcv_ctx* c, const rmcv_params* p, int stages, void* hip_stream)
{
    int rc = check_bound(c, p, stages);
    if (rc) return rc;
    hipSetDevice(c->device);
    return run_stages(c, p, stages, hip_stream ? (hipStream_t)hip_stream : c->stream, false, ctx_plan(c));
}

int rmcv_batch_run_legacy(rmcv_ctx* c, const rmcv_params* p, const rmcv_legacy_params* lp, int stages, void* hip_stream)
{
    int rc = check_bound(c, p, stages);
    if (rc) return rc;
    if (!lp) return fail(c, RMCV_ERR_BAD_ARG, "null legacy params");
    if ((rc = refuse(c, pixel_refusal(c->input.format | c->geom.input_format, c->input.enhance | c->geom.enhance, false, false, true)))) return rc;
    hipSetDevice(c->device);
    return run_stages(c, p, stages, hip_stream ? (hipStream_t)hip_stream : c->stream, false, ctx_plan(c), lp);
}

int rmcv_ctx_set_option(rmcv_ctx* c, int option, int value)
{
    if (!c) return RMCV_ERR_BAD_ARG;
    const OptionRule* rule = option_rule(option);
    if (!rule || !rule->accepts(value)) return fail(c, RMCV_ERR_BAD_ARG, "unknown option or value");
    switch (option) {
    case RMCV_OPT_SPARSE_WAVES: c->sparse_waves = value; break;
    case RMCV_OPT_RUN_AHEAD: c->chain.run_ahead = value; break;
    case RMCV_OPT_FRAME_UPLOAD: c->chain.frame_upload = value, c->chain.copy_up = {}; break;
    case RMCV_OPT_TEST_SLOW_US: c->chain.test_slow_us = value; break;
    case RMCV_OPT_PIXEL_HALO_NT: c->geom.pixel_halo_nt = value; break;
    case OPT_PIXEL_ROWQUAD: c->geom.pixel_rowquad = value; break;
    case RMCV_OPT_PIXEL_SHAPE: c->pixel_shape = value; break;
    case RMCV_OPT_OVERLOADS: c->geom.overloads = value, resident_none(c); break;
    case RMCV_OPT_DENSE_DEFER: c->dense_defer = value; break;
    case RMCV_OPT_CONTOUR_TIER: c->geom.contour_tier = value; break;
    case RMCV_OPT_IMAGE_EXPORT: c->chain.image_export = value, c->chain.copy_img = {}; break;
    case RMCV_OPT_WAIT_TIMEOUT_MS: c->wait_timeout_ms = value; break;
    case RMCV_OPT_TEST_DELAY_US: c->test_delay_us = value; break;
    case RMCV_OPT_INPUT_FORMAT: c->input.format = value; break;
    case RMCV_OPT_INPUT_SAMPLE_BITS: c->input.sample_bits = value; break;
    case RMCV_OPT_INPUT_VALID_BIT: c->input.valid_bit = value; break;
    case RMCV_OPT_INPUT_ORIENT: c->input.orient = value; break;
    case RMCV_OPT_ENHANCE: c->input.enhance = value; break;
    case RMCV_OPT_PIXEL_GROUPS: c->pixel_groups = value; break;
    }
    return RMCV_OK;
}

int rmcv_ctx_check_guards(rmcv_ctx* c, int32_t* n_damaged)
{
    if (!c || !n_damaged) return RMCV_ERR_BAD_ARG;
    if (const int rc = ctx_ready(c)) return rc;
    std::vector<uint8_t> h;
    int bad = 0;
    c->err[0] = 0;
    for (const auto& g : c->guarded) {
        for (int side = 0; side < 2; side++) {
            const size_t n = side ? g.rear : GUARD;
            const uint8_t* src = side ? g.base + GUARD + g.bytes : g.base;
            h.resize(n);
            HIPCHK(c, hipMemcpy(h.data(), src, n, hipMemcpyDeviceToHost), "D2H guard zone");
            size_t first = n;
            for (size_t i = 0; i < n; i++)
                if (h[i] != GUARD_BYTE) { first = i; break; }
            if (first < n) {
                if (!bad) snprintf(c->err, sizeof(c->err), "guard zone %s %s damaged at byte %zu (buffer of %zu bytes)", side ? "behind" : "in front of", g.name, first, g.bytes);
                bad++;
            }
        }
    }
    *n_damaged = bad;
    return RMCV_OK;
}

int rmcv_batch_sync(rmcv_ctx* c)
// ... 630 lines not shown
```

rmcv_amd/csrc/rmcv_internal.h:

```cpp
#pragma once
#include <hip/hip_runtime.h>
#include <stdint.h>

#include <tuple>
#include <utility>
#include <vector>

#include "../../include/rmcv_abi.h"
#include "bind_plan.h"
#include "device_harvest.h"
#include "image_plan.h"
#include "pixel_plan.h"
#include "sparse_plan.h"
#include "svm_plan.h"
#include "tracker_plan.h"

namespace rmcv {

static constexpr int CTR_STRIDE = 32;
static constexpr int VISIT_CAP = 4096;
static constexpr int NN_MID = 1 << 17;
static constexpr int CAND_MID = 1 << 15;
inline size_t mid_bytes(int slot_cap)
{
// ... 25 lines not shown
    int32_t* n_elig;
    int32_t* slot_kind;
    rmcv_rrect* slot_ell;
    int32_t* neg_idx;
    int32_t* n_blobs;
    int32_t* n_neg;
    rmcv_armour* armours;
    int32_t* n_armours;
    int32_t* status;
    int32_t* frame_order;
    float* svm_w;
    double* svm_rho;
    int32_t* svm_labels;
    int svm_classes;
    int32_t* identity;
    uint8_t* icons;
    rmcv_pnp_config* pnp_cfg;
    rmcv_pnp_config* cam_table;
    const rmcv_pnp_config* pnp_cams;
    int n_cameras;
    const int32_t* cam_req;
    int32_t* cam_eff;
    double* base2gripper;
    double* att_base2gripper;
    const double* pose_base2gripper;
    double* poses;
    uint64_t* enh_sums;
    float* enh_gamma;
    uint8_t* enh_lut;
    uint16_t* enh_m;
    const rmcv_point* win_req;
    rmcv_point* win_eff;
    const int32_t* key_camps;
    const int32_t* key_lbs;
    FrameKey* key_eff;
    int32_t* key_enemy;
};
inline const int32_t* enemy_table(const Geom& g, const Bufs& b) { return g.keys ? b.key_enemy : nullptr; }

__host__ __device__ inline rmcv_point window_origin_eff(rmcv_point req, int frame_w, int frame_h, int win_w, int win_h)
{
    const int xm = frame_w - win_w, ym = frame_h - win_h;
    rmcv_point e;
    e.x = (req.x < 0 ? 0 : (req.x > xm ? xm : req.x)) & ~15;
    e.y = req.y < 0 ? 0 : (req.y > ym ? ym : req.y);
    return e;
}
__host__ __device__ inline int64_t frame_origin_offset(const rmcv_point* __restrict__ win_eff, int f, int stride)
{
    return win_eff ? (int64_t)win_eff[f].y * stride + 3 * (int64_t)win_eff[f].x : 0;
}

inline PixelBatch pixel_batch(const Geom& g, const Bufs& b, PixelVariant v, int lower_bound, const RunPlan& plan)
{
    return {v, g.n_frames, g.w, g.h, g.ww, g.stride, g.frame_pitch, g.plane_pitch, g.n_cu, g.pixel_rowquad, (uintptr_t)b.frames % 16 == 0,
            lower_bound, plan.pixel_ws, plan.pixel_groups};
}

#define RMCV_FRAME_DEFERRED_ (1 << 30)

struct SparseSched {
    const int32_t* order;
};

static constexpr int MAX_DEVICES = 64;

template <typename... P, size_t... I>
inline hipError_t launch_tuple(void (*kernel)(P...), dim3 grid, dim3 block, size_t lds, hipStream_t s, std::tuple<P...>& vals,
                               std::index_sequence<I...>)
{
    void* ptrs[] = {static_cast<void*>(const_cast<typename std::remove_const<P>::type*>(&std::get<I>(vals)))...};
    return hipLaunchKernel(reinterpret_cast<const void*>(kernel), grid, block, ptrs, lds, s);
}
template <typename... P, typename... A>
inline hipError_t launch(void (*kernel)(P...), dim3 grid, dim3 block, size_t lds, hipStream_t s, A&&... a)
{
    static_assert(sizeof...(P) == sizeof...(A), "argument count differs from the kernel's parameter list");
    std::tuple<P...> vals{static_cast<P>(a)...};
    return launch_tuple(kernel, grid, block, lds, s, vals, std::index_sequence_for<P...>{});
}

int64_t pixel_ws_launches();
int64_t pixel_image_delta_launches();
hipError_t launch_match(const Geom& g, const Bufs& b, const Limits& lim, const rmcv_params& p, const rmcv_legacy_params& lp,
                        int mode, bool with_frames, bool pairs, hipStream_t s);
hipError_t launch_sparse(const Geom& g, const Bufs& b, const Limits& lim, const rmcv_params& p, bool pairs, bool identity, const RunPlan& plan,
                         hipStream_t s, bool* lean = nullptr);
hipError_t launch_pnp(const Geom& g, const Bufs& b, const Limits& lim, hipStream_t s);
hipError_t launch_binary(const Geom& g, const Bufs& b, int camp, int lower_bound, int morph, bool image, const RunPlan& plan, hipStream_t s,
                         ImageState* img);
hipError_t launch_binary_bayer(const Geom& g, const Bufs& b, int camp, int lower_bound, int morph, bool image, hipStream_t s);
hipError_t launch_enhance_tables(const Geom& g, const Bufs& b, int lower_bound, hipStream_t s);
hipError_t launch_binary_enh(const Geom& g, const Bufs& b, int camp, int lower_bound, int morph, bool image, const RunPlan& plan, hipStream_t s);
hipError_t launch_window_origins(const Geom& g, const Bufs& b, hipStream_t s);
hipError_t launch_binary_win(const Geom& g, const Bufs& b, int camp, int lower_bound, int morph, bool image, const RunPlan& plan, hipStream_t s);
hipError_t launch_frame_keys(const Geom& g, const Bufs& b, int run_lower_bound, hipStream_t s);
hipError_t launch_binary_camp(const Geom& g, const Bufs& b, int morph, bool image, const RunPlan& plan, hipStream_t s);
hipError_t launch_binary_camp_win(const Geom& g, const Bufs& b, int morph, bool image, const RunPlan& plan, hipStream_t s);
hipError_t launch_bytemap(const uint8_t* d_src, uint8_t* d_dst, int64_t n16, const uint8_t* d_lut, int n_cu, hipStream_t s);
hipError_t launch_gamma_lut(float gamma, uint8_t* d_lut, hipStream_t s);
hipError_t launch_demosaic(const uint8_t* d_raw, int stride, int w, int h, int pattern, int lay, uint8_t* d_out, int out_stride, hipStream_t s);
inline int geom_pixel_bytes(const Geom& g) { return g.input_format ? g.sample_bytes : 3; }
hipError_t launch_contours(const Geom& g, const Bufs& b, const Limits& lim, hipStream_t s);
hipError_t launch_blobs(const Geom& g, const Bufs& b, const Limits& lim, const rmcv_params& p, hipStream_t s);
hipError_t launch_armours(const Geom& g, const Bufs& b, const Limits& lim, const rmcv_params& p, hipStream_t s);
hipError_t launch_blobs_armours(const Geom& g, const Bufs& b, const Limits& lim, const rmcv_params& p, hipStream_t s);
hipError_t launch_compact_armours(const Geom& g, const Bufs& b, const Limits& lim, rmcv_armour* d_out, int cap,
                                  int32_t* d_frame_offs, hipStream_t s, int32_t* d_status_or = nullptr, uint8_t* hd_record = nullptr, int host_head = 0);
hipError_t launch_status_clear(const Geom& g, const Bufs& b, int mask, hipStream_t s);
hipError_t launch_classify(const Geom& g, const Bufs& b, const Limits& lim, hipStream_t s);
hipError_t launch_pack_bits(const Geom& g, const Bufs& b, hipStream_t s);
struct ExportSec {
    const void* src;
    void* dst;
    const int32_t* count;
    int count_add, elem_bytes, max_elems;
};
struct ExportArgs {
    ExportSec sec[8];
    int n_sec;
    const int32_t* hdr_src[12];
    int32_t* hdr_dst;
};
hipError_t launch_export(const ExportArgs& a, hipStream_t s);
hipError_t launch_pack_contours(const Geom& g, const Bufs& b, const Limits& lim, rmcv_point* d_pts_out, int32_t* d_offs_out,
                                int32_t* d_hdr , hipStream_t s, const ExportArgs* ex = nullptr);
hipError_t launch_gather3(const int32_t* a, const int32_t* b, const int32_t* c, int32_t* d_out, hipStream_t s);

struct ViewLists {
    const rmcv_lightblob* blobs;
    const int32_t* n_blobs;
    const rmcv_armour* armours;
    const int32_t* n_armours;
    const rmcv_point* points;
    const int32_t* cont_start;
    const int32_t* cont_len;
    const int32_t* n_contours;
    const int32_t* neg_idx;
    const int32_t* n_neg;
    const int32_t* neg_offs;
    int max_blobs, max_armours, max_points, max_contours, csr;
};
struct ViewJob {
    int w, h, prow;
    int64_t plane_pitch;
    const uint64_t* bits;
    uint64_t* overlay;
    const int32_t* frames;
    int n, vw, vh, flags;
    uint8_t* out;
    int out_stride;
    int64_t out_pitch;
    ViewLists lists;
};
hipError_t launch_view(const ViewJob& j, hipStream_t s);
inline int view_stages_needed(int flags)
{
    return RMCV_STAGE_BINARY | ((flags & (RMCV_VIEW_BLOBS | RMCV_VIEW_NEGATIVES)) ? RMCV_STAGE_CONTOURS | RMCV_STAGE_BLOBS : 0) |
           ((flags & RMCV_VIEW_ARMOURS) ? RMCV_STAGE_CONTOURS | RMCV_STAGE_BLOBS | RMCV_STAGE_ARMOURS : 0);
}
int ctx_view_prepare(rmcv_ctx* c, int n);
int ctx_view_check(rmcv_ctx* c, const int32_t* frames, int n, int n_frames, int stages, int vw, int vh, int flags, int out_stride, int64_t out_pitch);
int ctx_view_enqueue(rmcv_ctx* c, const int32_t* d_frames, int n, int vw, int vh, int flags, void* d_out, int out_stride, int64_t out_pitch, hipStream_t s);

void ctx_external_order(rmcv_ctx* c, hipEvent_t done);
int ctx_compact(rmcv_ctx* c, void* d_armours_out, int cap, void* d_frame_offs, void* d_status_or, hipStream_t s, void* hd_record = nullptr, int host_head = 0);
const Limits& ctx_limits(const rmcv_ctx* c);
RunPlan ctx_plan(const rmcv_ctx* c);
int ctx_run(rmcv_ctx* c, const rmcv_params* p, const rmcv_legacy_params* lp, int stages, hipStream_t s, const RunPlan& plan, bool* lean = nullptr);
int ctx_bind_frames(rmcv_ctx* c, const void* d_frames, int n_frames, int w, int h, int stride, int64_t frame_pitch, hipStream_t s,
                    const void* d_origins = nullptr, int win_w = 0, int win_h = 0, const void* d_camps = nullptr, const void* d_lower_bounds = nullptr);
int ctx_check_modes(rmcv_ctx* c, bool keys, bool legacy);
int ctx_prepare_ring(rmcv_ctx* c);
uint64_t ctx_blocking_calls(const rmcv_ctx* c);
int ctx_wait_timeout_ms(const rmcv_ctx* c);
bool pixel_ws_full(const rmcv_ctx* c, int lower_bound, const RunPlan& plan);
int wait_stream_deadline(hipStream_t s, int timeout_ms, hipError_t* err);
int wait_event_deadline(hipEvent_t ev, int timeout_ms, hipError_t* err);
hipError_t launch_delay(unsigned long long ns, hipStream_t s);
int ctx_check_stages(rmcv_ctx* c, const rmcv_params* p, int stages);
int ctx_enhance(const rmcv_ctx* c);
int ctx_n_cameras(const rmcv_ctx* c);
void ctx_set_frame_cameras(rmcv_ctx* c, const void* d_idx);
PixelVariant ctx_pixel_variant(const rmcv_ctx* c);


hipError_t launch_track(const rmcv_tracker_config& cfg, const TrackerBufs& tb, const Bufs& b, const Limits& lim, bool identity, bool pose,
                        const rmcv_point* win_eff, int64_t timestamp, hipStream_t s);
struct LoopTicket;
int ctx_track(rmcv_ctx* c, rmcv_tracker* trk, int64_t timestamp, int stages, hipStream_t s, const LoopTicket* loop = nullptr);
const TrackerView& tracker_view(const rmcv_tracker* t);
hipError_t tracker_order_begin(rmcv_tracker* t, hipStream_t s);
hipError_t tracker_order_end(rmcv_tracker* t, hipStream_t s);

hipError_t launch_aim(const TrackerView& v, int64_t now, hipStream_t s);

hipError_t launch_attitude(const TrackerView& v, const void* d_packets, double* d_base2gripper, hipStream_t s);
int ctx_attitude(rmcv_ctx* c, rmcv_tracker* trk, const void* d_packets, hipStream_t s);

static constexpr int PACK_MAX_FRAMES = 64;
struct PackIdx { int32_t f[PACK_MAX_FRAMES]; };
struct PackJob {
    const uint8_t* frames;
    int64_t pitch;
    int stride, w_bytes, h, lag, n;
    uint8_t* out;
    int64_t out_pitch;
    int64_t* sizes;
    int use_idx;
    PackIdx idx;
    const FrameKey* key_eff;
    int32_t* keys_out;
    const int32_t* key_enemy;
    int32_t* camps_out;
    const rmcv_point* win_eff;
    rmcv_point* origins_out;
};
hipError_t launch_pack(const PackJob& j, hipStream_t s);
hipError_t launch_unpack(const uint8_t* packed, int64_t in_pitch, int n, int w_bytes, int h, int lag, uint8_t* frames, int stride, int64_t pitch, hipStream_t s);
const char* pack_job_refusal(const void* frames, int n, int w_bytes, int h, int stride, int64_t pitch, int lag, const void* packed, int64_t packed_pitch);

struct RecordBatch {
    const void* d_frames;
    int w, h, stride;
    int w_bytes, lag;
    int64_t pitch;
    int batch_frames;
    int input_format, sample_bits, valid_bit, orient;
    int stages, win_w, win_h;
    rmcv_params params;
    int64_t timestamp;
    uint64_t ticket;
    const FrameKey* key_eff;
    const int32_t* key_enemy;
    const rmcv_point* win_eff;
    const rmcv_tracker* trk;
};
const char* recorder_refusal(const rmcv_recorder* r, int device, int n, int w_bytes, int h);
int recorder_enqueue(rmcv_recorder* r, const RecordBatch& b, const int32_t* frames, int n, hipStream_t s, LoopTicket* loop = nullptr);
void ctx_record_batch(const rmcv_ctx* c, RecordBatch* b);
int ctx_frame_pixel_bytes(const rmcv_ctx* c);

struct LoopLatch {
    uint32_t fired;
    int32_t k, stream;
    int32_t set;
    uint64_t sequence;
};
struct LoopTicket {
    rmcv_recorder* rec = nullptr;
    int slot = 0;
    uint64_t sequence = 0;
    const void* d_packets = nullptr;
};
struct LoopArgs {
    int n, rec_cap, n_streams, trk_cap;
// ... 61 lines not shown
```

rmcv_amd/csrc/rmcv_pipeline.hip:

```cpp
#include <stdio.h>
#include <stdlib.h>
#include <string.h>
#include <time.h>

#include <new>
#include <vector>

#include "batch_plan.h"
#include "rmcv_internal.h"

using namespace rmcv;

struct Slot {
    hipEvent_t ev_bin = nullptr;
    hipEvent_t ev_done = nullptr;
    hipEvent_t ev_host = nullptr;
    hipEvent_t ev_sp = nullptr;
    hipEvent_t ev_free = nullptr;
    hipEvent_t ev_chg = nullptr;
    void* ev_hook = nullptr;
    uint8_t *d_rec = nullptr, *h_rec = nullptr, *hd_rec = nullptr, *d_recv = nullptr;
    uint64_t ticket = 0;
    hipStream_t stream = nullptr;
    int frames = 0, ctx = 0;
    bool lean = false;
    uint8_t* d_views = nullptr;
    int view_n = 0, view_w = 0, view_h = 0;
};

struct BatchRequest {
    const void* d_frames;
    int n_frames, w, h, stride;
    int64_t frame_pitch;
    const rmcv_params* p;
    int stages;
    const rmcv_legacy_params* lp = nullptr;
    const void* d_origins = nullptr;
    int win_w = 0, win_h = 0;
    const void *d_camps = nullptr, *d_lower_bounds = nullptr;
    rmcv_tracker* trk = nullptr;
    int64_t timestamp = 0;
    const void* d_packets = nullptr;
};

struct rmcv_pipeline {
    int device = 0;
    rmcv_pipeline_config cfg{};
    Limits lim{};
    RecordLayout rec{};
    std::vector<rmcv_ctx*> ring;
    std::vector<int> ctx_last;
    std::vector<Slot> slots;
    std::vector<hipStream_t> pix, sp, dn;
    uint64_t next_ticket = 0, collected = 0;
    int hot = 0;
    int hot_cfg = 0;
    Mood mood{};
    bool split_now = false;
    bool was_cold = false;
    uint64_t hot_seq = 0, hot_batches = 0, heavy_batches = 0, split_batches = 0, latency_batches = 0;
    struct Pending {
        bool valid = false;
        uint64_t t = 0;
        BatchRequest req{};
        rmcv_params p{};
        rmcv_legacy_params lp{};
        size_t k = 0;
        rmcv_ctx* c = nullptr;
        bool used = false;
        RunPlan plan{};
        int sparse = 0;
        hipStream_t B = nullptr;
        bool views = false;
        LoopTicket loop{};
        bool harvest = false;
    } pend;
    rmcv_pipeline_hook hook = nullptr;
    void* hook_user = nullptr;
    rmcv_comm* comm = nullptr;
    int root = 0, n_ranks = 0, rank = 0;
    hipEvent_t ev_gather = nullptr;
    bool gather_pending = false;
    uint64_t own_blocking = 0, held_back = 0;
    int wait_timeout_ms = 5000;
    const char* last_what = "nothing";
    const void* cam_idx = nullptr;
    int cam_frames = 0;
    double max_submit_us = 0;
    struct Views {
        int n = 0, vw = 0, vh = 0, flags = 0, max_index = 0, need = 0;
        int32_t* d_frames = nullptr;
    } views;
    struct Recording {
        rmcv_recorder* rec = nullptr;
        int n = 0, max_index = 0;
        int32_t frames[RMCV_RECORDER_MAX_FRAMES] = {};
    } recd;
    struct Harvest {
        rmcv_dataset* ds = nullptr;
        int32_t* d_labels = nullptr;
        int n_labels = 0, flags = 0;
    } harv;
    char err[256] = {0};
};

static int finish_back(rmcv_pipeline* pl, bool latency);

static int pfail(rmcv_pipeline* pl, int code, const char* what, hipError_t e = hipSuccess)
{
    if (pl) {
        if (e != hipSuccess) snprintf(pl->err, sizeof(pl->err), "%s: %s", what, hipGetErrorString(e));
        else snprintf(pl->err, sizeof(pl->err), "%s", what);
    }
    if (e != hipSuccess) (void)hipGetLastError();
    return code;
}
#define PCHK(pl, call, what)                                               \
    do {                                                                   \
        (pl)->last_what = what;                                            \
        hipError_t e__ = (call);                                           \
        if (e__ != hipSuccess) return pfail((pl), RMCV_ERR_HIP, what, e__); \
    } while (0)
static int cfail(rmcv_pipeline* pl, rmcv_ctx* c, int rc)
{
    snprintf(pl->err, sizeof(pl->err), "%s", rmcv_last_error(c));
    return rc;
}

template <class Wait, class What> static int pwait(rmcv_pipeline* pl, Wait wait, What on, const char* what)
{
    hipError_t e = hipSuccess;
    const int rcw = wait(on, pl->wait_timeout_ms, &e);
    if (rcw < 0) return pfail(pl, RMCV_ERR_HIP, what, e);
    if (rcw == 0) return RMCV_OK;
    snprintf(pl->err, sizeof(pl->err), "%s: not finished after %d ms (rmcv_pipeline_set_wait_timeout); enqueued last: %s", what, pl->wait_timeout_ms, pl->last_what);
    return RMCV_ERR_TIMEOUT;
}
static int pwait_event(rmcv_pipeline* pl, hipEvent_t ev, const char* what) { return pwait(pl, wait_event_deadline, ev, what); }
static int pwait_stream(rmcv_pipeline* pl, hipStream_t st, const char* what) { return pwait(pl, wait_stream_deadline, st, what); }
static uint64_t ring_blocking(const rmcv_pipeline* pl)
{
    uint64_t n = 0;
    for (auto c : pl->ring) n += ctx_blocking_calls(c);
    return n;
}

static hipError_t slot_create(Slot& s, size_t record_bytes, bool host_mirror)
{
    hipError_t e = hipSuccess;
    for (hipEvent_t* ev : {&s.ev_sp, &s.ev_free, &s.ev_chg, &s.ev_bin, &s.ev_done, &s.ev_host})
        if (e == hipSuccess) e = hipEventCreateWithFlags(ev, hipEventDisableTiming);
    if (e == hipSuccess) e = hipMalloc((void**)&s.d_rec, record_bytes);
    if (e == hipSuccess) e = hipMemset(s.d_rec, 0, record_bytes);
    if (e == hipSuccess && host_mirror) {
        e = hipHostMalloc((void**)&s.h_rec, record_bytes, hipHostMallocMapped);
        if (e == hipSuccess) memset(s.h_rec, 0, record_bytes);
        if (e == hipSuccess) e = hipHostGetDevicePointer((void**)&s.hd_rec, s.h_rec, 0);
    }
    return e;
}
static void slot_destroy(Slot& s)
{
    for (hipEvent_t ev : {s.ev_bin, s.ev_done, s.ev_host, s.ev_sp, s.ev_free, s.ev_chg}) if (ev) hipEventDestroy(ev);
    if (s.d_rec) hipFree(s.d_rec);
    if (s.d_recv) hipFree(s.d_recv);
    if (s.h_rec) hipHostFree(s.h_rec);
    if (s.d_views) hipFree(s.d_views);
}
static RecordReport slot_report(const rmcv_pipeline* pl, const Slot& s) { return record_report(reinterpret_cast<const uint32_t*>(s.h_rec)[pl->rec.report_word]); }
static Slot* live_slot(rmcv_pipeline* pl, uint64_t ticket)
{
    Slot* s = ticket < pl->next_ticket ? &pl->slots[ticket_place(ticket, pl->cfg).slot] : nullptr;
    if (s && s->ticket == ticket + 1) return s;
    pfail(pl, RMCV_ERR_BAD_ARG, "no such ticket in flight (never issued, or its slot has been reused)");
    return nullptr;
}
static constexpr uint64_t NO_TICKET = ~0ull;
static int finish_newest(rmcv_pipeline* pl, uint64_t ticket)
{
    if (!pl->pend.valid) return RMCV_OK;
    hipSetDevice(pl->device);
    return finish_back(pl, pl->pend.t == ticket);
}

extern "C" {

void rmcv_default_pipeline_config(rmcv_pipeline_config* c) { if (c) *c = default_batch_config(); }

void rmcv_pipeline_destroy(rmcv_pipeline* pl)
{
    if (!pl) return;
    hipSetDevice(pl->device);
    if (!pl->ring.empty()) (void)finish_back(pl, true);
    {
        bool stuck = false;
        for (auto streams : {&pl->pix, &pl->sp, &pl->dn})
            for (auto s : *streams) if (s) stuck |= pwait_stream(pl, s, "destroy") == RMCV_ERR_TIMEOUT;
        if (stuck) {
            fprintf(stderr, "rmcv_pipeline_destroy: %s; the pipeline's buffers are leaked\n", pl->err);
            return;
        }
    }
    for (auto c : pl->ring) rmcv_ctx_destroy(c);
    for (auto& s : pl->slots) slot_destroy(s);
    if (pl->views.d_frames) hipFree(pl->views.d_frames);
    if (pl->harv.d_labels) hipFree(pl->harv.d_labels);
    if (pl->ev_gather) hipEventDestroy(pl->ev_gather);
    for (auto streams : {&pl->pix, &pl->sp, &pl->dn})
        for (auto s : *streams) if (s) hipStreamDestroy(s);
    delete pl;
}

int rmcv_pipeline_create(int device, const rmcv_limits* limits, const rmcv_pipeline_config* cfg, rmcv_pipeline** out)
{
    if (!out) return RMCV_ERR_BAD_ARG;
    *out = nullptr;
    const BatchConfig bc = resolve_config(cfg);
    if (bc.rc != RMCV_OK) return bc.rc;
    const rmcv_pipeline_config& d = bc.cfg;
    rmcv_pipeline* pl = new (std::nothrow) rmcv_pipeline();
    if (!pl) return RMCV_ERR_NOMEM;
    pl->device = device;
    pl->cfg = d, pl->hot_cfg = bc.hot_cfg;
    int rc = RMCV_OK;
    for (int k = 0; k < d.depth && rc == RMCV_OK; k++) {
        rmcv_ctx* c = nullptr;
        rc = rmcv_ctx_create(device, limits, &c);
        if (rc == RMCV_OK) {
            pl->ring.push_back(c);
            rc = rmcv_ctx_set_option(c, RMCV_OPT_SPARSE_WAVES, d.sparse_waves);
            if (rc == RMCV_OK) rc = rmcv_ctx_set_option(c, RMCV_OPT_PIXEL_GROUPS, d.pixel_groups);
            if (rc == RMCV_OK) rc = ctx_prepare_ring(c);
        }
    }
    if (rc != RMCV_OK) {
        rmcv_pipeline_destroy(pl);
        return rc;
    }
    pl->lim = ctx_limits(pl->ring[0]);
    pl->rec = record_layout(pl->lim.max_frames, pl->cfg.armour_cap);
    pl->cfg.armour_cap = pl->rec.armour_cap;
    hipError_t e = hipSetDevice(device);
    int lo = 0, hi = 0;
    if (e == hipSuccess) e = hipDeviceGetStreamPriorityRange(&lo, &hi);
    const auto streams = [&e](std::vector<hipStream_t>& v, int n, int priority) {
        for (int i = 0; i < n && e == hipSuccess; i++) {
            v.push_back(nullptr);
            e = hipStreamCreateWithPriority(&v.back(), hipStreamNonBlocking, priority);
        }
    };
    streams(pl->pix, d.pixel_streams, 0);
    streams(pl->sp, d.sparse_streams, hi);
    streams(pl->dn, d.dense_streams, 0);
    for (int k = 0; k < d.depth && e == hipSuccess; k++) {
        pl->slots.emplace_back();
        e = slot_create(pl->slots.back(), (size_t)pl->rec.record_bytes, d.host_results == 1);
        if (e == hipSuccess) ctx_external_order(pl->ring[(size_t)k], pl->slots.back().ev_done);
    }
    if (e == hipSuccess) e = hipEventCreateWithFlags(&pl->ev_gather, hipEventDisableTiming);
    pl->ctx_last.assign((size_t)d.depth, -1);
    pl->hot = hot_for(pl->hot_cfg, d.depth, pl->lim.max_frames, pl->lim.max_width, pl->lim.max_height);
    pl->wait_timeout_ms = ctx_wait_timeout_ms(pl->ring[0]);
    if (e != hipSuccess) {
        fprintf(stderr, "rmcv_pipeline_create: %s\n", hipGetErrorString(e));
        (void)hipGetLastError();
        rmcv_pipeline_destroy(pl);
        return e == hipErrorOutOfMemory ? RMCV_ERR_NOMEM : RMCV_ERR_HIP;
    }
    *out = pl;
    return RMCV_OK;
}

int rmcv_hw_queues_hint(void)
{
    setenv("GPU_MAX_HW_QUEUES", "12", 0);
    const char* q = getenv("GPU_MAX_HW_QUEUES");
    return q ? atoi(q) : 0;
}

const char* rmcv_pipeline_last_error(const rmcv_pipeline* pl) { return pl ? pl->err : "null pipeline"; }

int rmcv_pipeline_get_info(const rmcv_pipeline* pl, rmcv_pipeline_info* o)
{
    if (!pl || !o) return RMCV_ERR_BAD_ARG;
    memset(o, 0, sizeof(*o));
    const rmcv_pipeline_config& c = pl->cfg;
    o->depth = c.depth, o->pixel_streams = c.pixel_streams, o->sparse_streams = c.sparse_streams, o->armour_cap = c.armour_cap;
    o->sparse_waves = c.sparse_waves, o->pixel_groups = c.pixel_groups, o->host_results = c.host_results, o->dense_streams = c.dense_streams;
    const char* q = getenv("GPU_MAX_HW_QUEUES");
    o->hw_queues_env = q ? atoi(q) : 0;
    o->hw_queues_wanted = 1 + pl->cfg.pixel_streams + pl->cfg.sparse_streams + pl->cfg.dense_streams + (pl->comm ? 1 : 0);
    o->record_bytes = pl->rec.record_bytes, o->armours_offset = pl->rec.head_bytes;
    o->submitted = pl->next_ticket, o->collected = pl->collected;
    o->dense_split = pl->split_batches, o->hot_batches = pl->hot_batches, o->latency_batches = pl->latency_batches;
    o->hot_contexts = pl->hot, o->max_frames = pl->lim.max_frames;
    o->host_blocking_calls = pl->own_blocking, o->max_submit_us = pl->max_submit_us, o->wait_timeout_ms = pl->wait_timeout_ms;
    o->held_back = pl->held_back, o->heavy_batches = pl->heavy_batches;
    return RMCV_OK;
}

rmcv_ctx* rmcv_pipeline_context(rmcv_pipeline* pl, int slot)
{
    if (!pl || slot < 0 || slot >= pl->cfg.depth) return nullptr;
    return pl->ring[(size_t)slot];
}

int rmcv_pipeline_set_hot_contexts(rmcv_pipeline* pl, int n)
{
    if (!pl) return RMCV_ERR_BAD_ARG;
    if (n <= 0) { pl->hot = 0; pl->hot_cfg = -1; return RMCV_OK; }
    if (const char* no = hot_contexts_refusal(n, pl->cfg)) return pfail(pl, RMCV_ERR_BAD_ARG, no);
    pl->hot = pl->hot_cfg = n;
    return RMCV_OK;
}

int rmcv_pipeline_set_wait_timeout(rmcv_pipeline* pl, int ms)
{
    if (!pl || ms < 0) return RMCV_ERR_BAD_ARG;
    pl->wait_timeout_ms = ms;
    for (auto c : pl->ring) rmcv_ctx_set_option(c, RMCV_OPT_WAIT_TIMEOUT_MS, ms);
    return RMCV_OK;
}

rmcv_ctx* rmcv_pipeline_context_of(rmcv_pipeline* pl, uint64_t ticket)
{
    if (!pl || finish_newest(pl, ticket)) return nullptr;
    const Slot* s = live_slot(pl, ticket);
    if (!s) return nullptr;
    if (pl->ctx_last[(size_t)s->ctx] != (int)(s - pl->slots.data())) { pfail(pl, RMCV_ERR_BAD_ARG, "the ticket's context has been reused by a later batch (its record is still there: rmcv_pipeline_collect)"); return nullptr; }
    return pl->ring[(size_t)s->ctx];
}

int rmcv_pipeline_set_hook(rmcv_pipeline* pl, rmcv_pipeline_hook fn, void* user)
{
    if (!pl) return RMCV_ERR_BAD_ARG;
    if (const int rcb = finish_newest(pl, NO_TICKET)) return rcb;
    if (pl->comm && fn) return pfail(pl, RMCV_ERR_BAD_ARG, "the pipeline already gathers with rmcv_gather (rmcv_pipeline_set_gather): one hook at a time");
    pl->hook = fn, pl->hook_user = user;
    return RMCV_OK;
}

int rmcv_pipeline_set_gather(rmcv_pipeline* pl, rmcv_comm* comm, int root)
{
    if (!pl) return RMCV_ERR_BAD_ARG;
    if (const int rcb = finish_newest(pl, NO_TICKET)) return rcb;
    if (pl->hook && comm) return pfail(pl, RMCV_ERR_BAD_ARG, "the pipeline already has a hook (rmcv_pipeline_set_hook): one at a time");
    int rc = rmcv_pipeline_drain(pl);
    if (rc) return rc;
    hipSetDevice(pl->device);
    for (auto& s : pl->slots) if (s.d_recv) { hipFree(s.d_recv); s.d_recv = nullptr; }
    pl->comm = nullptr, pl->gather_pending = false;
    if (!comm) return RMCV_OK;
    int32_t n = 0, r = 0;
    if ((rc = rmcv_comm_info(comm, &n, &r))) return pfail(pl, rc, "rmcv_comm_info");
    if (root < 0 || root >= n) return pfail(pl, RMCV_ERR_BAD_ARG, "root out of range");
    if (r == root)
        for (auto& s : pl->slots) PCHK(pl, hipMalloc((void**)&s.d_recv, (size_t)pl->rec.record_bytes * (size_t)n), "hipMalloc (gather receive buffer)");
    pl->comm = comm;
    pl->root = root, pl->n_ranks = n, pl->rank = r;
    return RMCV_OK;
}

static int finish_back(rmcv_pipeline* pl, bool latency)
{
    if (!pl->pend.valid) return RMCV_OK;
    pl->pend.valid = false;
    const rmcv_pipeline::Pending& P = pl->pend;
    const BatchRequest& q = P.req;
    Slot& S = pl->slots[P.k];
    hipStream_t B = P.B;
    int rc = RMCV_OK;
    if (P.used && !pl->dn.empty() && hipEventQuery(S.ev_done) == hipSuccess) pl->split_now = split_rule(slot_report(pl, S), S.frames);
    (void)hipGetLastError();
    const BackPlan bp = back_plan(latency, pl->cfg, q.lp != nullptr, P.plan, pl->split_now, (int)pl->dn.size(), P.sparse, P.k);
    RunPlan plan = {P.plan.pixel_ws, P.plan.pixel_groups, bp.sparse_waves, bp.first};
    if (bp.w8) pl->latency_batches++;
    if (bp.split) pl->split_batches++;
    hipStream_t T = bp.dense_stream >= 0 ? pl->dn[(size_t)bp.dense_stream] : B;
    if (P.used && S.stream && S.stream != T) {
        PCHK(pl, hipEventRecord(S.ev_chg, S.stream), "pipeline: change of the slot's stream (mark)");
        PCHK(pl, hipStreamWaitEvent(T, S.ev_chg, 0), "pipeline: change of the slot's stream (wait)");
    }
    bool lean = false;
    if (P.sparse) {
        if (bp.split) {
            rc = ctx_run(P.c, q.p, nullptr, P.sparse & ~RMCV_STAGE_POSE, B, plan);
            if (rc == RMCV_OK) {
                PCHK(pl, hipEventRecord(S.ev_sp, B), "pipeline: mark the first sparse launch");
                PCHK(pl, hipStreamWaitEvent(T, S.ev_sp, 0), "pipeline: chain the dense frames");
                plan.form = bp.second;
                rc = ctx_run(P.c, q.p, nullptr, P.sparse, T, plan);
            }
        } else {
            rc = ctx_run(P.c, q.p, q.lp, P.sparse, B, plan, &lean);
        }
        if (rc) return cfail(pl, P.c, rc);
    }
    S.view_n = 0;
    if (P.views) {
        const rmcv_pipeline::Views& V = pl->views;
        rc = ctx_view_enqueue(P.c, V.d_frames, V.n, V.vw, V.vh, V.flags, S.d_views, 3 * V.vw, (int64_t)3 * V.vw * V.vh, T);
        if (rc) return cfail(pl, P.c, rc);
        pl->last_what = "k_view_resize";
        S.view_n = V.n, S.view_w = V.vw, S.view_h = V.vh;
    }
    if (P.harvest) {
        const rmcv_pipeline::Harvest& Hv = pl->harv;
        rc = ctx_harvest(P.c, Hv.ds, nullptr, Hv.d_labels, Hv.n_labels, Hv.flags, P.t, q.stages, T);
        if (rc) return cfail(pl, P.c, rc);
        pl->last_what = "k_harvest_rows";
    }
    PCHK(pl, hipEventRecord(S.ev_free, T), "pipeline: mark the pixel outputs' last reader");
    if (S.ev_hook) {
        PCHK(pl, hipStreamWaitEvent(T, (hipEvent_t)S.ev_hook, 0), "pipeline: wait for the record's reader");
        S.ev_hook = nullptr;
    }
    int32_t* offs = reinterpret_cast<int32_t*>(S.d_rec);
    rc = ctx_compact(P.c, S.d_rec + pl->rec.head_bytes, pl->cfg.armour_cap, offs, offs + pl->rec.status_word, T, S.hd_rec, (int)pl->rec.head_bytes);
    if (rc) return cfail(pl, P.c, rc);
    if (q.trk) {
        rc = ctx_track(P.c, q.trk, q.timestamp, q.stages, T, &P.loop);
        if (rc) return cfail(pl, P.c, rc);
        pl->last_what = P.loop.rec ? "k_loop_record" : "k_track";
    }
    PCHK(pl, hipEventRecord(S.ev_done, T), "pipeline: mark the slot");
    S.ticket = P.t + 1;
    S.frames = q.n_frames;
    S.lean = lean;
    S.stream = T;
    if (pl->comm) {
        if (pl->gather_pending) PCHK(pl, hipStreamWaitEvent(T, pl->ev_gather, 0), "pipeline: order the gathers");
        rc = rmcv_gather(pl->comm, S.d_rec, pl->rec.record_bytes, pl->rank == pl->root ? S.d_recv : nullptr, pl->root, T);
        if (rc) return pfail(pl, rc, rmcv_comm_last_error(pl->comm));
        PCHK(pl, hipEventRecord(pl->ev_gather, T), "pipeline: mark the gather");
        pl->gather_pending = true;
        PCHK(pl, hipEventRecord(S.ev_host, T), "pipeline: mark the gather");
    } else if (pl->hook) {
        void* done = nullptr;
        rc = pl->hook(pl->hook_user, P.t, S.d_rec, pl->rec.record_bytes, T, &done);
        if (rc) return pfail(pl, rc, "the pipeline hook failed");
        S.ev_hook = done;
    }
    return RMCV_OK;
}

static int submit(rmcv_pipeline* pl, const BatchRequest& q, uint64_t* ticket)
{
    if (!pl || !q.d_frames || !q.p) return RMCV_ERR_BAD_ARG;
    const rmcv_legacy_params* lp = q.lp;
    const int stages = q.stages;
    if (!(stages & RMCV_STAGE_BINARY)) return pfail(pl, RMCV_ERR_BAD_ARG, "a pipelined batch starts at RMCV_STAGE_BINARY");
    bool attitude = false;
    if (q.trk) {
        const TrackerView& v = tracker_view(q.trk);
        attitude = v.att_on;
        if (const char* no = tracked_refusal(v.device, pl->device, v.cfg, q.n_frames, q.w, q.h, stages, q.d_packets != nullptr, attitude))
            return pfail(pl, RMCV_ERR_BAD_ARG, no);
    }
    if (pl->views.n) {
        if (q.n_frames <= pl->views.max_index) return pfail(pl, RMCV_ERR_BAD_ARG, "the batch has fewer frames than the debug views name (rmcv_pipeline_set_views)");
        if ((stages & pl->views.need) != pl->views.need) return pfail(pl, RMCV_ERR_BAD_ARG, "the batch's stages lack what the debug views' flags need (rmcv_pipeline_set_views)");
    }
    if (pl->recd.n) {
        if (q.n_frames <= pl->recd.max_index) return pfail(pl, RMCV_ERR_BAD_ARG, "the batch has fewer frames than the recorder's frame list names (rmcv_pipeline_set_recorder)");
        if (const char* no = recorder_refusal(pl->recd.rec, pl->device, pl->recd.n, q.w * ctx_frame_pixel_bytes(pl->ring[0]), q.h)) return pfail(pl, RMCV_ERR_BAD_ARG, no);
        if (const char* no = recorder_trigger_refusal(pl->recd.rec, pl->cfg.depth)) return pfail(pl, RMCV_ERR_BAD_ARG, no);
    }
    if (pl->harv.ds)
        if (const char* no = ctx_harvest_refusal(pl->device, q.n_frames, true, pl->harv.ds, pl->harv.n_labels, pl->harv.flags, stages)) return pfail(pl, RMCV_ERR_BAD_ARG, no);
    hipSetDevice(pl->device);
    int rc = finish_back(pl, false);
    if (rc) return rc;
    const uint64_t t = pl->next_ticket;
    const TicketPlace at = ticket_place(t, pl->cfg);
    const size_t k = at.slot;
    Slot& S = pl->slots[k];
    const bool used = S.ticket != 0;
    pl->hot = hot_for(pl->hot_cfg, pl->cfg.depth, q.n_frames, q.d_origins ? q.win_w : q.w, q.d_origins ? q.win_h : q.h);
    if (pl->cfg.host_results == 1) {
        for (uint64_t d = 1; d <= (uint64_t)pl->cfg.depth && d <= t; d++) {
            const Slot& s = pl->slots[ticket_place(t - d, pl->cfg).slot];
            if (s.ticket != t - d + 1 || !s.h_rec) break;
            if (hipEventQuery(s.ev_done) != hipSuccess) continue;
            pl->mood = stream_mood(slot_report(pl, s), s.lean, s.frames);
            break;
        }
        (void)hipGetLastError();
    }
    const bool ws_variant = PIXEL_VARIANTS[pixel_variant(RMCV_INPUT_BGR, ctx_enhance(pl->ring[k]), q.d_origins != nullptr, q.d_camps != nullptr)].ws;
    const FrontPlan fp = front_plan(pl->hot, pl->mood.calm, pl->mood.heavy, pl->cfg, stages, lp != nullptr, ws_variant, q.trk != nullptr, pl->hot_seq, k);
    rmcv_ctx* c = pl->ring[fp.j];
    for (size_t i = 1; i < pl->ring.size(); i++)
        if (ctx_enhance(pl->ring[i]) != ctx_enhance(pl->ring[0]))
            return pfail(pl, RMCV_ERR_BAD_ARG, "RMCV_OPT_ENHANCE differs between the pipeline's contexts: set it on EVERY slot (rmcv_pipeline_context)");
    const bool cameras = pl->cam_idx && (stages & RMCV_STAGE_POSE);
    if (cameras) {
        bool agree = true;
        char msg[200];
        for (size_t i = 1; i < pl->ring.size(); i++) agree &= ctx_n_cameras(pl->ring[i]) == ctx_n_cameras(pl->ring[0]);
        if (const char* no = cameras_refusal(q.n_frames, pl->cam_frames, agree, msg)) return pfail(pl, RMCV_ERR_BAD_ARG, no);
    }
    if ((lp || q.d_camps) && (rc = ctx_check_modes(c, q.d_camps != nullptr, lp != nullptr))) return cfail(pl, c, rc);
    if ((rc = ctx_check_stages(c, q.p, stages))) return cfail(pl, c, rc);
    const RunPlan plan = fp.plan(ctx_plan(c));
    hipStream_t A = pl->pix[at.pixel], B = pl->sp[at.sparse];
    if (used) PCHK(pl, hipStreamWaitEvent(A, S.ev_done, 0), "pipeline: wait for the slot");
    if (pl->ctx_last[fp.j] >= 0 && pl->ctx_last[fp.j] != (int)k) {
        const Slot& last = pl->slots[(size_t)pl->ctx_last[fp.j]];
        PCHK(pl, hipStreamWaitEvent(A, waits_for_free(last.stream, B) ? last.ev_free : last.ev_done, 0), "pipeline: wait for the context");
    }
    rc = ctx_bind_frames(c, q.d_frames, q.n_frames, q.w, q.h, q.stride, q.frame_pitch, A, q.d_origins, q.win_w, q.win_h, q.d_camps, q.d_lower_bounds);
    if (rc) return cfail(pl, c, rc);
    if (cameras) ctx_set_frame_cameras(c, pl->cam_idx);
    const int pixel = stages & (RMCV_STAGE_BINARY | RMCV_STAGE_NO_IMAGE), sparse = stages & ~(RMCV_STAGE_BINARY | RMCV_STAGE_NO_IMAGE);
    ctx_external_order(c, S.ev_done);
    bool prev_live = false, prev_done = false;
    if (fp.fast && t > 0) {
        const Slot& prev = pl->slots[ticket_place(t - 1, pl->cfg).slot];
        prev_live = prev.ticket == t;
        prev_done = prev_live && hipEventQuery(prev.ev_done) == hipSuccess;
        (void)hipGetLastError();
    }
    const bool ws_full = prev_live && !prev_done && pl->was_cold && pixel_ws_full(c, q.p->lower_bound, plan);
    const HoldBack hb = hold_back(fp.fast, t, pl->was_cold, prev_live, prev_done, ws_full, q.n_frames, q.w, q.h);
    if (hb.hold_us > 0) {
        PCHK(pl, launch_delay((unsigned long long)hb.hold_us * 1000ull, A), "pipeline: k_delay");
        pl->held_back++;
    }
    if (q.trk && q.d_origins && !attitude) PCHK(pl, tracker_order_begin(q.trk, A), "pipeline: wait for the tracker's last step");
    if (attitude) {
        rc = ctx_attitude(c, q.trk, q.d_packets, A);
        if (rc) return cfail(pl, c, rc);
    }
    rc = ctx_run(c, q.p, nullptr, pixel, A, plan);
    if (rc) return cfail(pl, c, rc);
    pl->last_what = PIXEL_VARIANTS[ctx_pixel_variant(c)].step;
    pl->was_cold = hb.cold;
    if (fp.fast) { pl->hot_seq++; pl->hot_batches++; }
    if (fp.heavy) pl->heavy_batches++;
    pl->ctx_last[fp.j] = (int)k;
    S.ctx = (int)fp.j;
    PCHK(pl, hipEventRecord(S.ev_bin, A), "pipeline: mark the pixel kernel");
    PCHK(pl, hipStreamWaitEvent(B, S.ev_bin, 0), "pipeline: chain the sparse stages");
    LoopTicket loop{};
    if (pl->recd.n) {
        RecordBatch rb{};
        rb.d_frames = q.d_frames, rb.w = q.w, rb.h = q.h, rb.stride = q.stride, rb.pitch = q.frame_pitch, rb.batch_frames = q.n_frames;
        rb.stages = stages, rb.win_w = q.d_origins ? q.win_w : 0, rb.win_h = q.d_origins ? q.win_h : 0;
        rb.params = *q.p, rb.timestamp = q.timestamp, rb.ticket = t;
        ctx_record_batch(c, &rb);
        rb.trk = q.trk;
        if ((rc = recorder_enqueue(pl->recd.rec, rb, pl->recd.frames, pl->recd.n, B, &loop))) return pfail(pl, rc, rmcv_recorder_last_error(pl->recd.rec));
        loop.d_packets = q.d_packets;
        pl->last_what = "k_pack_emit";
    }
    pl->next_ticket = t + 1;
    if (ticket) *ticket = t;
    pl->pend = {true, t, q, *q.p, lp ? *lp : rmcv_legacy_params{}, k, c, used, plan, sparse, B, pl->views.n > 0, loop, pl->harv.ds != nullptr};
    pl->pend.req.p = &pl->pend.p;
    pl->pend.req.lp = lp ? &pl->pend.lp : nullptr;
    if (pl->hook || pl->comm) return finish_back(pl, false);
    return RMCV_OK;
}

static int submit_counted(rmcv_pipeline* pl, const BatchRequest& q, uint64_t* ticket)
{
    if (!pl) return RMCV_ERR_BAD_ARG;
    timespec t0, t1;
    clock_gettime(CLOCK_MONOTONIC, &t0);
    const uint64_t b0 = ring_blocking(pl);
    const int rc = submit(pl, q, ticket);
    pl->own_blocking += ring_blocking(pl) - b0;
    clock_gettime(CLOCK_MONOTONIC, &t1);
    const double us = (t1.tv_sec - t0.tv_sec) * 1e6 + (t1.tv_nsec - t0.tv_nsec) * 1e-3;
    if (us > pl->max_submit_us) pl->max_submit_us = us;
    return rc;
}

int rmcv_pipeline_set_frame_cameras(rmcv_pipeline* pl, const void* d_idx, int n_frames)
{
    if (!pl) return RMCV_ERR_BAD_ARG;
    if (d_idx && (n_frames < 1 || n_frames > pl->lim.max_frames)) return pfail(pl, RMCV_ERR_BAD_ARG, "rmcv_pipeline_set_frame_cameras: n_frames out of range");
    pl->cam_idx = d_idx;
    pl->cam_frames = d_idx ? n_frames : 0;
    return RMCV_OK;
}

int rmcv_pipeline_reset_stats(rmcv_pipeline* pl)
{
    if (!pl) return RMCV_ERR_BAD_ARG;
    pl->max_submit_us = 0;
    return RMCV_OK;
}

int rmcv_pipeline_submit(rmcv_pipeline* pl, const void* d_frames, int n_frames, int w, int h, int stride, int64_t frame_pitch,
                         const rmcv_params* p, int stages, uint64_t* ticket)
{
    return submit_counted(pl, {d_frames, n_frames, w, h, stride, frame_pitch, p, stages}, ticket);
}

int rmcv_pipeline_submit_legacy(rmcv_pipeline* pl, const void* d_frames, int n_frames, int w, int h, int stride, int64_t frame_pitch,
                                const rmcv_params* p, const rmcv_legacy_params* lp, int stages, uint64_t* ticket)
{
    if (!lp) return RMCV_ERR_BAD_ARG;
    BatchRequest q{d_frames, n_frames, w, h, stride, frame_pitch, p, stages};
    q.lp = lp;
    return submit_counted(pl, q, ticket);
}

int rmcv_pipeline_submit_windows(rmcv_pipeline* pl, const void* d_frames, int n_frames, int frame_w, int frame_h, int stride, int64_t frame_pitch,
                                 const void* d_origins, int win_w, int win_h, const rmcv_params* p, int stages, uint64_t* ticket)
{
    if (!pl) return RMCV_ERR_BAD_ARG;
    if (!d_origins) return pfail(pl, RMCV_ERR_BAD_ARG, "rmcv_pipeline_submit_windows: null origins (device memory: one rmcv_point per frame)");
    if (win_w < 1 || win_h < 1) return pfail(pl, RMCV_ERR_BAD_ARG, "rmcv_pipeline_submit_windows: window size out of range");
    BatchRequest q{d_frames, n_frames, frame_w, frame_h, stride, frame_pitch, p, stages};
    q.d_origins = d_origins, q.win_w = win_w, q.win_h = win_h;
    return submit_counted(pl, q, ticket);
}

int rmcv_pipeline_submit_tracked(rmcv_pipeline* pl, rmcv_tracker* trk, const void* d_frames, int n_frames, int frame_w, int frame_h, int stride,
                                 int64_t frame_pitch, const rmcv_params* p, int stages, int64_t timestamp, uint64_t* ticket)
{
    return rmcv_pipeline_submit_tracked_serial(pl, trk, d_frames, n_frames, frame_w, frame_h, stride, frame_pitch, nullptr, p, stages, timestamp, ticket);
// ... 239 lines not shown
```

Measured before the change: 1.230 million.

## Double-buffer pixel outputs per hot context and skip unchanged plane writes

Adds a second set of pixel-output buffers (binary, bit planes, row and image masks) to each hot context and alternates between them. The next batch's pixel kernel then waits only on the earlier use of the same set, not on the whole previous batch, so it can overlap the sparse stages still reading the other set. It also adds a plane-delta mode to the workspace binary kernel, which skips bit-plane stores, padding clears and rowmask writes for words that were empty before and are still empty. This costs extra device memory, more events and stream waits, and a more intricate state machine that must keep planes consistent across set swaps.

New measurement: 1.305 million, median of 6. 1.06x the previous value.

```diff
diff --git a/include/rmcv_abi.h b/include/rmcv_abi.h
--- a/include/rmcv_abi.h
+++ b/include/rmcv_abi.h
@@ -125,6 +125,7 @@
 int  rmcv_ctx_get_enhance(const rmcv_ctx* ctx, int32_t* on, float* max_gain, float* min_gain);
 int64_t rmcv_pixel_ws_launches(void);
 int64_t rmcv_pixel_image_delta_launches(void);
+int64_t rmcv_pixel_plane_delta_launches(void);
 int  rmcv_ctx_check_guards(rmcv_ctx* ctx, int32_t* n_damaged);
 int  rmcv_ctx_frame_timing(const rmcv_ctx* ctx, double* us, int cap);
 int  rmcv_ctx_forget_frame_buffer(rmcv_ctx* ctx, const void* frame);
diff --git a/rmcv_amd/abi.py b/rmcv_amd/abi.py
--- a/rmcv_amd/abi.py
+++ b/rmcv_amd/abi.py
@@ -78,7 +78,7 @@
     "rmcv_svm_load", "rmcv_classify_armours", "rmcv_batch_get_identities", "rmcv_batch_get_icons",
     "rmcv_default_pnp_config", "rmcv_pnp_load", "rmcv_locate_armours", "rmcv_batch_set_base2gripper", "rmcv_batch_get_poses",
     "rmcv_max_iou", "rmcv_identity_max", "rmcv_comm_unique_id", "rmcv_comm_create", "rmcv_comm_destroy", "rmcv_comm_info", "rmcv_comm_last_error", "rmcv_gather",
-    "rmcv_default_pipeline_config", "rmcv_pipeline_create", "rmcv_pipeline_destroy", "rmcv_pipeline_last_error", "rmcv_pipeline_get_info", "rmcv_pipeline_context", "rmcv_pipeline_context_of", "rmcv_pipeline_set_hot_contexts", "rmcv_pipeline_set_wait_timeout", "rmcv_pipeline_reset_stats", "rmcv_hw_queues_hint", "rmcv_pixel_ws_launches", "rmcv_pixel_image_delta_launches",
+    "rmcv_default_pipeline_config", "rmcv_pipeline_create", "rmcv_pipeline_destroy", "rmcv_pipeline_last_error", "rmcv_pipeline_get_info", "rmcv_pipeline_context", "rmcv_pipeline_context_of", "rmcv_pipeline_set_hot_contexts", "rmcv_pipeline_set_wait_timeout", "rmcv_pipeline_reset_stats", "rmcv_hw_queues_hint", "rmcv_pixel_ws_launches", "rmcv_pixel_image_delta_launches", "rmcv_pixel_plane_delta_launches",
     "rmcv_pipeline_submit", "rmcv_pipeline_submit_legacy", "rmcv_pipeline_wait", "rmcv_pipeline_collect", "rmcv_pipeline_drain", "rmcv_pipeline_record",
     "rmcv_pipeline_set_hook", "rmcv_pipeline_set_gather", "rmcv_pipeline_gathered", "rmcv_device_alloc", "rmcv_device_free", "rmcv_device_upload", "rmcv_device_download",
     "rmcv_track_init", "rmcv_track_reset", "rmcv_track_update", "rmcv_track_predict", "rmcv_track_step", "rmcv_min_area_rect", "rmcv_match_lightblob", "rmcv_find_lightblobs", "rmcv_lightblob_overlap", "rmcv_batch_run_legacy",
@@ -280,6 +280,9 @@
     if hasattr(L, "rmcv_pixel_image_delta_launches"):
         L.rmcv_pixel_image_delta_launches.restype = C.c_int64
         L.rmcv_pixel_image_delta_launches.argtypes = []
+    if hasattr(L, "rmcv_pixel_plane_delta_launches"):
+        L.rmcv_pixel_plane_delta_launches.restype = C.c_int64
+        L.rmcv_pixel_plane_delta_launches.argtypes = []
     L.rmcv_pipeline_context_of.restype = C.c_void_p
     L.rmcv_pipeline_context_of.argtypes = [C.c_void_p, C.c_uint64]
     L.rmcv_pipeline_submit.argtypes = [C.c_void_p, C.c_void_p, C.c_int, C.c_int, C.c_int, C.c_int, C.c_int64, C.c_void_p, C.c_int, C.c_void_p]
diff --git a/rmcv_amd/csrc/image_plan.h b/rmcv_amd/csrc/image_plan.h
--- a/rmcv_amd/csrc/image_plan.h
+++ b/rmcv_amd/csrc/image_plan.h
@@ -36,4 +36,14 @@
     return r;
 }
 
+struct PlaneStep { bool delta; int next; };
+inline PlaneStep plane_step(int sync, ImageMode mode, const ImageLaunch& l, bool ok)
+{
+    PlaneStep r = {false, 0};
+    if (!l.image || l.kernel != IMAGE_KERNEL_WS) return r;
+    r.delta = mode == IMAGE_DELTA && l.frames <= sync;
+    if (ok) r.next = r.delta ? sync : l.frames;
+    return r;
 }
+
+}
diff --git a/rmcv_amd/csrc/k_binary.hip b/rmcv_amd/csrc/k_binary.hip
--- a/rmcv_amd/csrc/k_binary.hip
+++ b/rmcv_amd/csrc/k_binary.hip
@@ -20,19 +20,22 @@
 int64_t pixel_ws_launches() { return g_ws_launches.load(std::memory_order_relaxed); }
 static std::atomic<int64_t> g_image_delta_launches{0};
 int64_t pixel_image_delta_launches() { return g_image_delta_launches.load(std::memory_order_relaxed); }
+static std::atomic<int64_t> g_plane_delta_launches{0};
+int64_t pixel_plane_delta_launches() { return g_plane_delta_launches.load(std::memory_order_relaxed); }
 #define K1_LAUNCH_T launch_binary_t
 #define K1_EXTRA
 #include "k_binary_launch.inc"
 
 hipError_t launch_binary(const Geom& g, const Bufs& b, int camp, int lower_bound, int morph, bool image, const RunPlan& plan, hipStream_t s,
-                         ImageState* img)
+                         ImageState* img, int* plane)
 {
     const PixelVariant v = pixel_variant(g.input_format, g.enhance, g.win, g.keys);
     if (v == PIXEL_BGR)
-        return with_channel_pair(frame_key_eff(camp, lower_bound), [&](auto ca, auto cb) { return launch_binary_t<ca, cb>(g, b, lower_bound, morph, image, plan, s, img); });
+        return with_channel_pair(frame_key_eff(camp, lower_bound), [&](auto ca, auto cb) { return launch_binary_t<ca, cb>(g, b, lower_bound, morph, image, plan, s, img, plane); });
     const ImageLaunch l = {IMAGE_KERNEL_OTHER, image, g.w, g.h, g.ww, g.n_frames};
     const ImageState before = img ? *img : IMAGE_STATE_UNKNOWN;
     if (img) *img = image_step(before, l, false).next;
+    if (plane) *plane = 0;
     hipError_t e = hipSuccess;
     switch (v) {
     case PIXEL_BGR: break;
diff --git a/rmcv_amd/csrc/k_binary_launch.inc b/rmcv_amd/csrc/k_binary_launch.inc
--- a/rmcv_amd/csrc/k_binary_launch.inc
+++ b/rmcv_amd/csrc/k_binary_launch.inc
@@ -11,7 +11,7 @@
 template <int CA, int CB>
 #endif
 static hipError_t K1_LAUNCH_T(const Geom& g, const Bufs& b, int lower_bound, int morph, bool image, const RunPlan& plan,
-                                  hipStream_t s, ImageState* img = nullptr)
+                                  hipStream_t s, ImageState* img = nullptr, int* plane = nullptr)
 {
     constexpr PixelVariant variant = K1_CAMP ? (K1_WIN ? PIXEL_CAMP_WIN : PIXEL_CAMP) : K1_WIN ? PIXEL_WIN : K1_ENH ? PIXEL_ENH : PIXEL_BGR;
     const PixelShape ps = pixel_shape(pixel_batch(g, b, variant, lower_bound, plan));
@@ -21,8 +21,11 @@
     const ImageState img_before = img ? *img : IMAGE_STATE_UNKNOWN;
     const ImageLaunch img_launch = {IMAGE_KERNEL_WS, image, g.w, g.h, g.ww, g.n_frames};
     const ImageMode img_mode = image_step(img_before, img_launch, true).mode;
+    const int plane_before = plane ? *plane : 0;
+    const bool plane_delta = plane_step(plane_before, img_mode, img_launch, true).delta;
     bool all_ws = true;
     if (img) *img = image_step(img_before, img_launch, false).next;
+    if (plane) *plane = plane_step(plane_before, img_mode, img_launch, false).next;
 #endif
     for (int f0 = 0; f0 < g.n_frames; f0 += ps.chunk) {
         const int nf = std::min(ps.chunk, g.n_frames - f0);
@@ -51,8 +54,10 @@
             ka.lb = lb; ka.morph = morph; ka.binary = binary; ka.bits = bits; ka.prow = g.prow; ka.plane_pitch = g.plane_pitch;
             ka.strips = strips; ka.n_blocks = n_blocks; ka.rowmask = rowmask; ka.strip_ctr = b.strip_ctr;
             ka.imgmask = b.imgmask + (int64_t)f0 * g.h; ka.delta = img_mode == IMAGE_DELTA;
+            ka.plane_delta = plane_delta;
             g_ws_launches.fetch_add(1, std::memory_order_relaxed);
             if (ka.delta && binary) g_image_delta_launches.fetch_add(1, std::memory_order_relaxed);
+            if (ka.delta && binary && plane_delta) g_plane_delta_launches.fetch_add(1, std::memory_order_relaxed);
             const hipError_t e = launch(k_binary_ws<CA, CB, WS_NL, WS_NS, WS_RING, WS_AUX, 3, 3>, dim3(pc.grid_ws), dim3((WS_NL + WS_NS) * 64), ps.planes_ws, s, ka);
             if (e != hipSuccess) return e;
             continue;
@@ -72,7 +77,9 @@
         if (e != hipSuccess) return e;
     }
 #if !K1_ENH && !K1_WIN && !K1_CAMP
-    if (img) *img = image_step(img_before, {all_ws ? IMAGE_KERNEL_WS : IMAGE_KERNEL_OTHER, image, g.w, g.h, g.ww, g.n_frames}, true).next;
+    const ImageLaunch img_ran = {all_ws ? IMAGE_KERNEL_WS : IMAGE_KERNEL_OTHER, image, g.w, g.h, g.ww, g.n_frames};
+    if (img) *img = image_step(img_before, img_ran, true).next;
+    if (plane) *plane = plane_step(plane_before, img_mode, img_ran, true).next;
 #endif
     return hipSuccess;
 }
diff --git a/rmcv_amd/csrc/k_binary_ws.inc b/rmcv_amd/csrc/k_binary_ws.inc
--- a/rmcv_amd/csrc/k_binary_ws.inc
+++ b/rmcv_amd/csrc/k_binary_ws.inc
@@ -12,6 +12,7 @@
     int* strip_ctr;
     uint32_t* imgmask;
     int delta;
+    int plane_delta;
 };
 
 template <int NS>
@@ -39,7 +40,7 @@
     const uint32_t plane_base = (uint32_t)((int64_t)f * a.plane_pitch);
     const int n_task = (RPW / 2) * ww;
     const uint32_t r_ww = (uint32_t)((0x100000000ull + ww - 1) / ww);
-    const bool masked = a.binary && ww <= 32, delta = masked && a.delta;
+    const bool masked = a.binary && ww <= 32, delta = masked && a.delta, pdelta = delta && a.plane_delta;
     const bool my_row = lane < RPW && y0 + s0 + lane < h;
     uint32_t* const im = a.imgmask + ((int64_t)f * h + y0 + s0 + lane);
     uint32_t m_new = 0;
@@ -100,6 +101,19 @@
             }
         }
         const int y = y0 + s;
+        bool k0 = true, k1 = true;
+        if (pdelta) {
+            static_assert(RPW / 2 * 32 <= 64, "a delta launch's tasks fit one pass");
+            uint64_t mo0 = 0, mo1 = 0;
+#pragma unroll
+            for (int i = 0; i < RPW / 2; i++) {
+                mo0 |= (uint64_t)(uint32_t)__builtin_amdgcn_readlane((int)m_old, 2 * i) << (i * ww);
+                mo1 |= (uint64_t)(uint32_t)__builtin_amdgcn_readlane((int)m_old, 2 * i + 1) << (i * ww);
+            }
+            const uint64_t kb0 = mo0 | __builtin_amdgcn_ballot_w64(on && e0 != 0), kb1 = mo1 | __builtin_amdgcn_ballot_w64(on && e1 != 0);
+            k0 = (kb0 >> lane) & 1ull;
+            k1 = (kb1 >> lane) & 1ull;
+        }
         if (on) {
             Ew[__umul24(2 * p, ww) + k] = e0;
             Ew[__umul24(2 * p + 1, ww) + k] = e1;
@@ -107,13 +121,13 @@
 #ifdef RMCV_K1_NOBITS
         const uint32_t po0 = OOB, po1 = OOB;
 #else
-        const uint32_t po0 = (on && y < h) ? (plane_base + __umul24(y + 1, a.prow) + 1u + (uint32_t)k) * 8u : OOB;
-        const uint32_t po1 = (on && y + 1 < h) ? (plane_base + __umul24(y + 2, a.prow) + 1u + (uint32_t)k) * 8u : OOB;
+        const uint32_t po0 = (on && y < h && k0) ? (plane_base + __umul24(y + 1, a.prow) + 1u + (uint32_t)k) * 8u : OOB;
+        const uint32_t po1 = (on && y + 1 < h && k1) ? (plane_base + __umul24(y + 2, a.prow) + 1u + (uint32_t)k) * 8u : OOB;
 #endif
         __builtin_amdgcn_raw_buffer_store_b64(__builtin_bit_cast(u32x2v, e0), r_plane, po0, 0, RMCV_K1_PLAIN_PLAUX);
         __builtin_amdgcn_raw_buffer_store_b64(__builtin_bit_cast(u32x2v, e1), r_plane, po1, 0, RMCV_K1_PLAIN_PLAUX);
         {
-            const bool last = on && k == ww - 1;
+            const bool last = on && k == ww - 1 && !pdelta;
             const u32x4v z = {0u, 0u, 0u, 0u};
             __builtin_amdgcn_raw_buffer_store_b128(z, r_plane, last && po0 != OOB ? po0 + 8u : OOB, 0, RMCV_K1_PLAIN_PLAUX);
             __builtin_amdgcn_raw_buffer_store_b128(z, r_plane, last && po1 != OOB ? po1 + 8u : OOB, 0, RMCV_K1_PLAIN_PLAUX);
@@ -126,7 +140,7 @@
                 const uint32_t m = (uint32_t)(b >> __umul24(pr, ww)) & (ww == 32 ? 0xFFFFFFFFu : ((1u << ww) - 1u));
                 m_new = m;
 #ifndef RMCV_K1_NOROWMASK
-                if (y0 + s0 + lane < h) a.rowmask[(int64_t)f * h + y0 + s0 + lane] = m;
+                if (y0 + s0 + lane < h && (!pdelta || m != m_old)) a.rowmask[(int64_t)f * h + y0 + s0 + lane] = m;
 #endif
             }
         }
@@ -138,7 +152,7 @@
         if (lane < RPW && y0 + s0 + lane < h) {
             uint32_t m = 0;
             for (int k = 0; k < ww; k++) m |= (uint32_t)(Ew[__umul24(lane, ww) + k] != 0) << k;
-            a.rowmask[(int64_t)f * h + y0 + s0 + lane] = m;
+            if (!pdelta || m != m_old) a.rowmask[(int64_t)f * h + y0 + s0 + lane] = m;
             m_new = m;
         }
     }
diff --git a/rmcv_amd/csrc/pixel_sets_plan.h b/rmcv_amd/csrc/pixel_sets_plan.h
--- /dev/null
+++ b/rmcv_amd/csrc/pixel_sets_plan.h
@@ -0,0 +1,19 @@
+#pragma once
+
+#include <stdint.h>
+
+namespace rmcv {
+
+inline int pixel_set_for(bool fast, uint64_t hot_seq, int hot, int sets)
+{
+    return fast && hot > 0 && sets > 1 ? (int)((hot_seq / (uint64_t)hot) & 1u) : 0;
+}
+
+struct SetWaits { bool pixel_ctx_last, pixel_set_last, pixel_ctx_bin, sparse_ctx_last; };
+inline SetWaits pixel_set_waits(bool fast, int sets, bool bind_enqueues)
+{
+    const bool old = !fast || sets < 2 || bind_enqueues;
+    return {old, !old, !old, true};
+}
+
+}
diff --git a/rmcv_amd/csrc/rmcv_ctx.h b/rmcv_amd/csrc/rmcv_ctx.h
--- a/rmcv_amd/csrc/rmcv_ctx.h
+++ b/rmcv_amd/csrc/rmcv_ctx.h
@@ -63,6 +63,15 @@
     hipStream_t last_stream = nullptr;
     int geom_w = -1, geom_h = -1;
     rmcv::ImageState image = rmcv::IMAGE_STATE_UNKNOWN;
+    int plane_sync = 0;
+    struct PixelSet {
+        uint8_t* binary = nullptr;
+        uint64_t* bits = nullptr;
+        uint32_t *rowmask = nullptr, *imgmask = nullptr;
+        rmcv::ImageState image = rmcv::IMAGE_STATE_UNKNOWN;
+        int plane_sync = 0;
+    } parked;
+    int n_sets = 1, cur_set = 0;
     int order_n = -1, order_h = -1;
     hipEvent_t ev_order = nullptr;
     bool order_pending = false;
diff --git a/rmcv_amd/csrc/rmcv_frame.hip b/rmcv_amd/csrc/rmcv_frame.hip
--- a/rmcv_amd/csrc/rmcv_frame.hip
+++ b/rmcv_amd/csrc/rmcv_frame.hip
@@ -343,7 +343,7 @@
         c->test_delay_us = 0;
     }
     if (g.enhance) HIPCHK(c, launch_enhance_tables(g, b, lower_bound, s), "k_frame_sums + k_enhance_table");
-    HIPCHK(c, launch_binary(g, b, camp, lower_bound, morph, binary_out != nullptr, plan, s, &c->image), PIXEL_VARIANTS[geom_variant(g)].kernel);
+    HIPCHK(c, launch_binary(g, b, camp, lower_bound, morph, binary_out != nullptr, plan, s, &c->image, &c->plane_sync), PIXEL_VARIANTS[geom_variant(g)].kernel);
     if (binary_out) HIPCHK(c, hipEventRecord(ch.ev_fork, s), "image download: mark");
     const bool fused_ahead = ch.run_ahead && ch.last_lb_valid && ch.last_ar_valid && ch.last_lb.enemy == ch.last_ar.enemy;
     if (fused_ahead) {
diff --git a/rmcv_amd/csrc/rmcv_host.hip b/rmcv_amd/csrc/rmcv_host.hip
--- a/rmcv_amd/csrc/rmcv_host.hip
+++ b/rmcv_amd/csrc/rmcv_host.hip
@@ -39,6 +39,7 @@
 int rmcv_abi_version(void) { return RMCV_ABI_VERSION; }
 int64_t rmcv_pixel_ws_launches(void) { return pixel_ws_launches(); }
 int64_t rmcv_pixel_image_delta_launches(void) { return pixel_image_delta_launches(); }
+int64_t rmcv_pixel_plane_delta_launches(void) { return pixel_plane_delta_launches(); }
 
 const char* rmcv_last_error(const rmcv_ctx* ctx) { return ctx ? ctx->err : "null context"; }
 
@@ -190,6 +191,23 @@
 bool pixel_ws_full(const rmcv_ctx* c, int lower_bound, const RunPlan& plan)
 {
     return pixel_shape(pixel_batch(c->geom, c->bufs, geom_variant(c->geom), lower_bound, plan)).ws_full;
+}
+int ctx_pixel_sets(const rmcv_ctx* c) { return c->n_sets; }
+int ctx_pixel_set(const rmcv_ctx* c) { return c->cur_set; }
+void ctx_use_pixel_set(rmcv_ctx* c, int s)
+{
+    if (s == c->cur_set || s < 0 || s >= c->n_sets) return;
+    Bufs& b = c->bufs;
+    const rmcv_ctx::PixelSet mine = {b.binary, b.bits, b.rowmask, b.imgmask, c->image, c->plane_sync};
+    b.binary = c->parked.binary, b.bits = c->parked.bits, b.rowmask = c->parked.rowmask, b.imgmask = c->parked.imgmask;
+    c->image = c->parked.image, c->plane_sync = c->parked.plane_sync;
+    c->parked = mine;
+    c->cur_set = s;
+}
+bool ctx_bind_enqueues(const rmcv_ctx* c, int n_frames, int w, int h)
+{
+    const ExtentChange change = extent_change(c->geom_w, c->geom_h, c->order_n, c->order_h, w, h, n_frames);
+    return change.planes || change.order;
 }
 RunPlan ctx_plan(const rmcv_ctx* c) { return {c->pixel_shape, c->pixel_groups, c->sparse_waves, c->dense_defer ? SPARSE_SPLIT_BOTH : SPARSE_STANDARD}; }
 int ctx_enhance(const rmcv_ctx* c) { return c->input.enhance; }
@@ -344,11 +362,13 @@
     if (change.planes) {
         const size_t plane = (size_t)(c->lim.max_height + 2) * ((c->lim.max_width + 63) / 64 + 2);
         HIPCHK(c, hipMemsetAsync(c->bufs.bits, 0, (size_t)c->lim.max_frames * plane * 8, s), "memset planes");
+        if (c->n_sets > 1) HIPCHK(c, hipMemsetAsync(c->parked.bits, 0, (size_t)c->lim.max_frames * plane * 8, s), "memset planes");
         HIPCHK(c, hipMemsetAsync(c->bufs.lab, 0, (size_t)c->lim.max_frames * plane * 8, s), "memset planes");
         HIPCHK(c, hipMemsetAsync(c->bufs.neg, 0, (size_t)c->lim.max_frames * plane * 8, s), "memset planes");
         c->geom_w = g.w;
         c->geom_h = g.h;
-        c->image = IMAGE_STATE_UNKNOWN;
+        c->image = c->parked.image = IMAGE_STATE_UNKNOWN;
+        c->plane_sync = c->parked.plane_sync = 0;
     }
     if (change.order) {
         const int strips = (g.h + STRIP_ROWS - 1) / STRIP_ROWS;
@@ -458,7 +478,7 @@
     if (st.binary) {
         c->last_camp = p->camp;
         c->last_lower_bound = p->lower_bound;
-        HIPCHK(c, launch_binary(g, b, p->camp, p->lower_bound, p->morph, st.image, plan, s, &c->image), PIXEL_VARIANTS[geom_variant(g)].kernel);
+        HIPCHK(c, launch_binary(g, b, p->camp, p->lower_bound, p->morph, st.image, plan, s, &c->image, &c->plane_sync), PIXEL_VARIANTS[geom_variant(g)].kernel);
     }
     if (timed) HIPCHK(c, hipEventRecord(c->ev[k++], s), "event");
     if (st.sparse) HIPCHK(c, launch_sparse(g, b, lim, *p, st.sparse_pairs, st.sparse_identity, plan, s, lean), "k_contours (fused)");
@@ -548,6 +568,24 @@
 }
 int ctx_check_modes(rmcv_ctx* c, bool keys, bool legacy) { return refuse(c, pixel_refusal(c->input.format, c->input.enhance, false, keys, legacy)); }
 int ctx_prepare_ring(rmcv_ctx* c) { return ensure_mid(c, c->lim.max_frames); }
+int ctx_prepare_pixel_sets(rmcv_ctx* c)
+{
+    if (c->n_sets > 1) return RMCV_OK;
+    hipSetDevice(c->device);
+    c->blocking_calls++;
+    const size_t F = (size_t)c->lim.max_frames;
+    const size_t plane = (size_t)(c->lim.max_height + 2) * ((c->lim.max_width + 63) / 64 + 2);
+    rmcv_ctx::PixelSet& p = c->parked;
+    HIPCHK(c, dalloc(c, &p.binary, F * c->lim.max_width * c->lim.max_height), "hipMalloc (second pixel set)");
+    HIPCHK(c, dalloc(c, &p.bits, F * plane), "hipMalloc (second pixel set)");
+    HIPCHK(c, dalloc(c, &p.rowmask, F * c->lim.max_height), "hipMalloc (second pixel set)");
+    HIPCHK(c, dalloc(c, &p.imgmask, F * c->lim.max_height), "hipMalloc (second pixel set)");
+    HIPCHK(c, hipMemset(p.bits, 0, F * plane * 8), "memset planes");
+    p.image = IMAGE_STATE_UNKNOWN;
+    p.plane_sync = 0;
+    c->n_sets = 2;
+    return RMCV_OK;
+}
 int ctx_run(rmcv_ctx* c, const rmcv_params* p, const rmcv_legacy_params* lp, int stages, hipStream_t s, const RunPlan& plan, bool* lean)
 {
     const int rc = check_bound(c, p, stages);
diff --git a/rmcv_amd/csrc/rmcv_internal.h b/rmcv_amd/csrc/rmcv_internal.h
--- a/rmcv_amd/csrc/rmcv_internal.h
+++ b/rmcv_amd/csrc/rmcv_internal.h
@@ -131,13 +131,14 @@
 
 int64_t pixel_ws_launches();
 int64_t pixel_image_delta_launches();
+int64_t pixel_plane_delta_launches();
 hipError_t launch_match(const Geom& g, const Bufs& b, const Limits& lim, const rmcv_params& p, const rmcv_legacy_params& lp,
                         int mode, bool with_frames, bool pairs, hipStream_t s);
 hipError_t launch_sparse(const Geom& g, const Bufs& b, const Limits& lim, const rmcv_params& p, bool pairs, bool identity, const RunPlan& plan,
                          hipStream_t s, bool* lean = nullptr);
 hipError_t launch_pnp(const Geom& g, const Bufs& b, const Limits& lim, hipStream_t s);
 hipError_t launch_binary(const Geom& g, const Bufs& b, int camp, int lower_bound, int morph, bool image, const RunPlan& plan, hipStream_t s,
-                         ImageState* img);
+                         ImageState* img, int* plane);
 hipError_t launch_binary_bayer(const Geom& g, const Bufs& b, int camp, int lower_bound, int morph, bool image, hipStream_t s);
 hipError_t launch_enhance_tables(const Geom& g, const Bufs& b, int lower_bound, hipStream_t s);
 hipError_t launch_binary_enh(const Geom& g, const Bufs& b, int camp, int lower_bound, int morph, bool image, const RunPlan& plan, hipStream_t s);
@@ -221,6 +222,11 @@
                     const void* d_origins = nullptr, int win_w = 0, int win_h = 0, const void* d_camps = nullptr, const void* d_lower_bounds = nullptr);
 int ctx_check_modes(rmcv_ctx* c, bool keys, bool legacy);
 int ctx_prepare_ring(rmcv_ctx* c);
+int ctx_prepare_pixel_sets(rmcv_ctx* c);
+int ctx_pixel_sets(const rmcv_ctx* c);
+int ctx_pixel_set(const rmcv_ctx* c);
+void ctx_use_pixel_set(rmcv_ctx* c, int s);
+bool ctx_bind_enqueues(const rmcv_ctx* c, int n_frames, int w, int h);
 uint64_t ctx_blocking_calls(const rmcv_ctx* c);
 int ctx_wait_timeout_ms(const rmcv_ctx* c);
 bool pixel_ws_full(const rmcv_ctx* c, int lower_bound, const RunPlan& plan);
diff --git a/rmcv_amd/csrc/rmcv_pipeline.hip b/rmcv_amd/csrc/rmcv_pipeline.hip
--- a/rmcv_amd/csrc/rmcv_pipeline.hip
+++ b/rmcv_amd/csrc/rmcv_pipeline.hip
@@ -7,6 +7,7 @@
 #include <vector>
 
 #include "batch_plan.h"
+#include "pixel_sets_plan.h"
 #include "rmcv_internal.h"
 
 using namespace rmcv;
@@ -23,6 +24,7 @@
     uint64_t ticket = 0;
     hipStream_t stream = nullptr;
     int frames = 0, ctx = 0;
+    int set = 0;
     bool lean = false;
     uint8_t* d_views = nullptr;
     int view_n = 0, view_w = 0, view_h = 0;
@@ -50,6 +52,7 @@
     RecordLayout rec{};
     std::vector<rmcv_ctx*> ring;
     std::vector<int> ctx_last;
+    std::vector<hipEvent_t> ev_set;
     std::vector<Slot> slots;
     std::vector<hipStream_t> pix, sp, dn;
     uint64_t next_ticket = 0, collected = 0;
@@ -127,6 +130,14 @@
     return rc;
 }
 
+static int prepare_pixel_sets(rmcv_pipeline* pl, int n)
+{
+    if (pl->cfg.host_results != 1 || pl->cfg.sparse_waves != 4) return RMCV_OK;
+    for (int j = 0; j < n && j < (int)pl->ring.size(); j++)
+        if (const int rc = ctx_prepare_pixel_sets(pl->ring[(size_t)j])) return cfail(pl, pl->ring[(size_t)j], rc);
+    return RMCV_OK;
+}
+
 template <class Wait, class What> static int pwait(rmcv_pipeline* pl, Wait wait, What on, const char* what)
 {
     hipError_t e = hipSuccess;
@@ -206,6 +217,7 @@
     if (pl->views.d_frames) hipFree(pl->views.d_frames);
     if (pl->harv.d_labels) hipFree(pl->harv.d_labels);
     if (pl->ev_gather) hipEventDestroy(pl->ev_gather);
+    for (hipEvent_t ev : pl->ev_set) if (ev) hipEventDestroy(ev);
     for (auto streams : {&pl->pix, &pl->sp, &pl->dn})
         for (auto s : *streams) if (s) hipStreamDestroy(s);
     delete pl;
@@ -259,7 +271,10 @@
     }
     if (e == hipSuccess) e = hipEventCreateWithFlags(&pl->ev_gather, hipEventDisableTiming);
     pl->ctx_last.assign((size_t)d.depth, -1);
+    pl->ev_set.assign(2 * (size_t)d.depth, nullptr);
+    for (hipEvent_t& ev : pl->ev_set) if (e == hipSuccess) e = hipEventCreateWithFlags(&ev, hipEventDisableTiming);
     pl->hot = hot_for(pl->hot_cfg, d.depth, pl->lim.max_frames, pl->lim.max_width, pl->lim.max_height);
+    if (e == hipSuccess && prepare_pixel_sets(pl, pl->hot) != RMCV_OK) e = hipErrorOutOfMemory;
     pl->wait_timeout_ms = ctx_wait_timeout_ms(pl->ring[0]);
     if (e != hipSuccess) {
         fprintf(stderr, "rmcv_pipeline_create: %s\n", hipGetErrorString(e));
@@ -310,6 +325,8 @@
     if (!pl) return RMCV_ERR_BAD_ARG;
     if (n <= 0) { pl->hot = 0; pl->hot_cfg = -1; return RMCV_OK; }
     if (const char* no = hot_contexts_refusal(n, pl->cfg)) return pfail(pl, RMCV_ERR_BAD_ARG, no);
+    hipSetDevice(pl->device);
+    if (const int rc = prepare_pixel_sets(pl, n)) return rc;
     pl->hot = pl->hot_cfg = n;
     return RMCV_OK;
 }
@@ -424,6 +441,7 @@
         pl->last_what = P.loop.rec ? "k_loop_record" : "k_track";
     }
     PCHK(pl, hipEventRecord(S.ev_done, T), "pipeline: mark the slot");
+    PCHK(pl, hipEventRecord(pl->ev_set[2 * (size_t)S.ctx + (size_t)S.set], T), "pipeline: mark the pixel-output set");
     S.ticket = P.t + 1;
     S.frames = q.n_frames;
     S.lean = lean;
@@ -504,11 +522,17 @@
     if ((rc = ctx_check_stages(c, q.p, stages))) return cfail(pl, c, rc);
     const RunPlan plan = fp.plan(ctx_plan(c));
     hipStream_t A = pl->pix[at.pixel], B = pl->sp[at.sparse];
+    const int set = pixel_set_for(fp.fast, pl->hot_seq, pl->hot, ctx_pixel_sets(c));
+    const SetWaits sw = pixel_set_waits(fp.fast, ctx_pixel_sets(c), ctx_bind_enqueues(c, q.n_frames, q.d_origins ? q.win_w : q.w, q.d_origins ? q.win_h : q.h));
     if (used) PCHK(pl, hipStreamWaitEvent(A, S.ev_done, 0), "pipeline: wait for the slot");
     if (pl->ctx_last[fp.j] >= 0 && pl->ctx_last[fp.j] != (int)k) {
         const Slot& last = pl->slots[(size_t)pl->ctx_last[fp.j]];
-        PCHK(pl, hipStreamWaitEvent(A, waits_for_free(last.stream, B) ? last.ev_free : last.ev_done, 0), "pipeline: wait for the context");
-    }
+        if (sw.pixel_ctx_last) PCHK(pl, hipStreamWaitEvent(A, waits_for_free(last.stream, B) ? last.ev_free : last.ev_done, 0), "pipeline: wait for the context");
+        if (sw.pixel_ctx_bin) PCHK(pl, hipStreamWaitEvent(A, last.ev_bin, 0), "pipeline: wait for the context's pixel kernel");
+    }
+    if (sw.pixel_set_last) PCHK(pl, hipStreamWaitEvent(A, pl->ev_set[2 * fp.j + (size_t)set], 0), "pipeline: wait for the context's pixel-output set");
+    if (sw.sparse_ctx_last && pl->ctx_last[fp.j] >= 0 && pl->ctx_last[fp.j] != (int)k)
+        PCHK(pl, hipStreamWaitEvent(B, pl->slots[(size_t)pl->ctx_last[fp.j]].ev_done, 0), "pipeline: the sparse stream waits for the context");
     rc = ctx_bind_frames(c, q.d_frames, q.n_frames, q.w, q.h, q.stride, q.frame_pitch, A, q.d_origins, q.win_w, q.win_h, q.d_camps, q.d_lower_bounds);
     if (rc) return cfail(pl, c, rc);
     if (cameras) ctx_set_frame_cameras(c, pl->cam_idx);
@@ -532,14 +556,19 @@
         rc = ctx_attitude(c, q.trk, q.d_packets, A);
         if (rc) return cfail(pl, c, rc);
     }
+    const int set_before = ctx_pixel_set(c);
+    ctx_use_pixel_set(c, set);
     rc = ctx_run(c, q.p, nullptr, pixel, A, plan);
-    if (rc) return cfail(pl, c, rc);
+    if (rc) {
+        ctx_use_pixel_set(c, set_before);
+        return cfail(pl, c, rc);
+    }
     pl->last_what = PIXEL_VARIANTS[ctx_pixel_variant(c)].step;
     pl->was_cold = hb.cold;
     if (fp.fast) { pl->hot_seq++; pl->hot_batches++; }
     if (fp.heavy) pl->heavy_batches++;
     pl->ctx_last[fp.j] = (int)k;
-    S.ctx = (int)fp.j;
+    S.ctx = (int)fp.j, S.set = set;
     PCHK(pl, hipEventRecord(S.ev_bin, A), "pipeline: mark the pixel kernel");
     PCHK(pl, hipStreamWaitEvent(B, S.ev_bin, 0), "pipeline: chain the sparse stages");
     LoopTicket loop{};
```
